# shenweichen/DeepCTR

Hardware: NVIDIA H100
Metric: samples/sec fwd+bwd DeepFM Criteo-synth (higher is better)
Workload: dtype f32

## Files before the change

### deepctr_b200/csrc/common.cuh

```cuda
#pragma once
#include <cuda_runtime.h>
#include <cuda_bf16.h>
#include <stdint.h>
#include <stdio.h>
#include <atomic>
#include "../../include/b2ctr.h"

namespace b2ctr {

void set_error(const char* fmt, ...);
extern std::atomic<long long> g_launches;
inline void count_launch(int n = 1) { g_launches.fetch_add(n, std::memory_order_relaxed); }

#define B2_REQUIRE(cond, ...)                         \
  do {                                                \
    if (!(cond)) {                                    \
      b2ctr::set_error(__VA_ARGS__);                  \
      return B2CTR_ERR_INVALID_ARG;                   \
    }                                                 \
  } while (0)

#define B2_CHECK_LAUNCH(name)                                                         \
  do {                                                                                \
    cudaError_t e__ = cudaGetLastError();                                             \
    if (e__ != cudaSuccess) {                                                         \
      b2ctr::set_error("%s: CUDA launch failed: %s", name, cudaGetErrorString(e__));  \
      return B2CTR_ERR_CUDA;                                                          \
    }                                                                                 \
    b2ctr::count_launch();                                                            \
  } while (0)

constexpr int kNumSMs = 132;

unsigned long long* oob_counter();

static inline int64_t ceil_div(int64_t a, int64_t b) { return (a + b - 1) / b; }

static inline int grid_for(int64_t work_items, int items_per_block, int blocks_per_sm) {
  int64_t need = ceil_div(work_items, items_per_block);
  int64_t cap = (int64_t)kNumSMs * blocks_per_sm;
  if (need < 1) need = 1;
  return (int)(need < cap ? need : cap);
}

static inline int64_t planes_rows_pad(int64_t rows) { return (rows + 255) / 256 * 256; }
static inline int64_t planes_cols_pad(int64_t cols) { return cols <= 64 ? 64 : (cols + 127) / 128 * 128; }

#ifdef __CUDACC__
__device__ __forceinline__ uint32_t pack_bf16(__nv_bfloat16 lo, __nv_bfloat16 hi) {
  return (uint32_t)__bfloat16_as_ushort(lo) | ((uint32_t)__bfloat16_as_ushort(hi) << 16);
}

__device__ __forceinline__ float4 ldg_stream_f4(const float* p) {
  float4 r;
  asm volatile("ld.global.nc.L1::no_allocate.v4.f32 {%0,%1,%2,%3}, [%4];"
               : "=f"(r.x), "=f"(r.y), "=f"(r.z), "=f"(r.w)
               : "l"(p));
  return r;
}
__device__ __forceinline__ float ldg_stream_f1(const float* p) {
  float r;
  asm volatile("ld.global.nc.L1::no_allocate.f32 %0, [%1];" : "=f"(r) : "l"(p));
  return r;
}
__device__ __forceinline__ void stg_stream_f4(float* p, float4 v) {
  asm volatile("st.global.L1::no_allocate.v4.f32 [%0], {%1,%2,%3,%4};" ::"l"(p), "f"(v.x),
               "f"(v.y), "f"(v.z), "f"(v.w)
               : "memory");
}
__device__ __forceinline__ void red_add_f4(float* p, float4 v) {
  asm volatile("red.relaxed.gpu.global.add.v4.f32 [%0], {%1,%2,%3,%4};" ::"l"(p), "f"(v.x),
               "f"(v.y), "f"(v.z), "f"(v.w)
               : "memory");
}
__device__ __forceinline__ void red_add_f1(float* p, float v) {
  asm volatile("red.relaxed.gpu.global.add.f32 [%0], %1;" ::"l"(p), "f"(v) : "memory");
}

__device__ __forceinline__ uint64_t l2_policy_evict_last() {
  uint64_t p;
  asm volatile("createpolicy.fractional.L2::evict_last.b64 %0, 1.0;" : "=l"(p));
  return p;
}
__device__ __forceinline__ uint64_t l2_policy_evict_first() {
  uint64_t p;
  asm volatile("createpolicy.fractional.L2::evict_first.b64 %0, 1.0;" : "=l"(p));
  return p;
}
__device__ __forceinline__ float4 ldg_stream_f4_pol(const float* p, uint64_t pol) {
  float4 r;
  asm volatile("ld.global.nc.L1::no_allocate.L2::cache_hint.v4.f32 {%0,%1,%2,%3}, [%4], %5;"
               : "=f"(r.x), "=f"(r.y), "=f"(r.z), "=f"(r.w)
               : "l"(p), "l"(pol));
  return r;
}
__device__ __forceinline__ float ldg_f1_pol(const float* p, uint64_t pol) {
  float r;
  asm volatile("ld.global.nc.L2::cache_hint.f32 %0, [%1], %2;" : "=f"(r) : "l"(p), "l"(pol));
  return r;
}
__device__ __forceinline__ void stg_stream_f4_pol(float* p, float4 v, uint64_t pol) {
  asm volatile("st.global.L1::no_allocate.L2::cache_hint.v4.f32 [%0], {%1,%2,%3,%4}, %5;" ::"l"(p),
               "f"(v.x), "f"(v.y), "f"(v.z), "f"(v.w), "l"(pol)
               : "memory");
}
__device__ __forceinline__ void red_add_f4_pol(float* p, float4 v, uint64_t pol) {
  asm volatile("red.relaxed.gpu.global.add.L2::cache_hint.v4.f32 [%0], {%1,%2,%3,%4}, %5;" ::"l"(p),
               "f"(v.x), "f"(v.y), "f"(v.z), "f"(v.w), "l"(pol)
               : "memory");
}
__device__ __forceinline__ void red_add_f1_pol(float* p, float v, uint64_t pol) {
  asm volatile("red.relaxed.gpu.global.add.L2::cache_hint.f32 [%0], %1, %2;" ::"l"(p), "f"(v), "l"(pol)
               : "memory");
}

__device__ __forceinline__ bool id_in_range(int64_t id, int64_t vocab) { return (uint64_t)id < (uint64_t)vocab; }
__device__ __forceinline__ void note_oob(unsigned long long* counter) {
  if (counter) atomicAdd(counter, 1ull);
}

__device__ __forceinline__ float warp_sum(float v) {
#pragma unroll
  for (int o = 16; o > 0; o >>= 1) v += __shfl_xor_sync(0xffffffffu, v, o);
  return v;
}

__device__ __forceinline__ uint32_t mix32(uint64_t z) {
  z = (z ^ (z >> 30)) * 0xbf58476d1ce4e5b9ULL;
  z = (z ^ (z >> 27)) * 0x94d049bb133111ebULL;
  return (uint32_t)((z ^ (z >> 31)) >> 32);
}

__device__ __forceinline__ int64_t load_idx(const void* p, int64_t off, int dtype) {
  return dtype == B2CTR_IDX_I64 ? reinterpret_cast<const int64_t*>(p)[off]
                                : (int64_t) reinterpret_cast<const int32_t*>(p)[off];
}

__device__ __forceinline__ float act_apply(float x, int act) {
  switch (act) {
    case B2CTR_ACT_RELU: return x > 0.f ? x : 0.f;
    case B2CTR_ACT_SIGMOID: return 1.f / (1.f + expf(-x));
    case B2CTR_ACT_TANH: return tanhf(x);
    default: return x;
  }
}
__device__ __forceinline__ float act_grad_from_out(float y, int act) {
  switch (act) {
    case B2CTR_ACT_RELU: return y > 0.f ? 1.f : 0.f;
    case B2CTR_ACT_SIGMOID: return y * (1.f - y);
    case B2CTR_ACT_TANH: return 1.f - y * y;
    default: return 1.f;
  }
}

#endif
}
```

### deepctr_b200/csrc/gemm_tc.cu

```cuda
#include <cuda.h>
#include <cuda_bf16.h>
#include "common.cuh"

namespace b2ctr {

constexpr int kTM = 128;
constexpr int kTK = 64;
constexpr int kTcThreads = 256;

struct PlaneArgs {
  const __nv_bfloat16* a_hi; const __nv_bfloat16* a_lo;
  const __nv_bfloat16* b_hi; const __nv_bfloat16* b_lo;
  int64_t a_pitch, b_pitch;
  int a_mn, b_mn;
  float* c; const float* bias; float* ws;
  int64_t m, n, k_pad;
  int64_t ldc;
  int64_t k_per_split;
  float alpha;
  int act, accumulate, splits;
  const float* cin_t0; const float* cin_xk;
  int64_t cin_ld0, cin_ldk, cin_rows;
  int cin_m, cin_h, cin_hp, cin_on;
  float* fold_dt0; float* fold_dxk; int64_t fold_ldx;
};

__device__ __forceinline__ uint32_t smem_u32(const void* p) {
  return (uint32_t)__cvta_generic_to_shared(p);
}
__device__ __forceinline__ void mbar_init(uint64_t* bar, uint32_t count) {
  asm volatile("mbarrier.init.shared::cta.b64 [%0], %1;" ::"r"(smem_u32(bar)), "r"(count));
}
__device__ __forceinline__ void mbar_arrive(uint64_t* bar) {
  asm volatile("mbarrier.arrive.shared::cta.b64 _, [%0];" ::"r"(smem_u32(bar)) : "memory");
}
__device__ __forceinline__ void mbar_wait(uint64_t* bar, uint32_t parity) {
  uint32_t done;
  do {
    asm volatile(
        "{\n\t"
        ".reg .pred p;\n\t"
        "mbarrier.try_wait.parity.shared::cta.b64 p, [%1], %2;\n\t"
        "selp.u32 %0, 1, 0, p;\n\t"
        "}\n"
        : "=r"(done)
        : "r"(smem_u32(bar)), "r"(parity)
        : "memory");
  } while (!done);
}
__device__ __forceinline__ uint64_t wgmma_desc(uint32_t saddr, int mn) {
  return (uint64_t)((saddr & 0x3FFFF) >> 4) | ((uint64_t)(mn ? 512 : 1) << 16) | (64ull << 32) | (1ull << 62);
}
__device__ __forceinline__ uint64_t wgmma_desc_k(uint32_t base, int ks, int mn) {
  return wgmma_desc(mn ? base + ks * 2048 : base + ks * 32, mn);
}
__device__ __forceinline__ void wgmma_fence() { asm volatile("wgmma.fence.sync.aligned;" ::: "memory"); }
__device__ __forceinline__ void wgmma_commit() { asm volatile("wgmma.commit_group.sync.aligned;" ::: "memory"); }
template <int N>
__device__ __forceinline__ void wgmma_wait() { asm volatile("wgmma.wait_group.sync.aligned %0;" ::"n"(N) : "memory"); }
template <int R>
__device__ __forceinline__ void fence_acc(float (&d)[R]) {
#pragma unroll
  for (int i = 0; i < R; ++i) asm volatile("" : "+f"(d[i])::"memory");
}

template <int N> struct Wgmma;
template <> struct Wgmma<32> {
  template <int TA, int TB>
  static __device__ __forceinline__ void mma(float (&d)[16], uint64_t da, uint64_t db) {
    asm volatile(
        "{\n\t.reg .pred p;\n\tsetp.ne.b32 p, %18, 0;\n\t"
        "wgmma.mma_async.sync.aligned.m64n32k16.f32.bf16.bf16 "
        "{%0,%1,%2,%3,%4,%5,%6,%7,%8,%9,%10,%11,%12,%13,%14,%15}, %16, %17, p, 1, 1, %19, %20;\n}\n"
        : "+f"(d[0]), "+f"(d[1]), "+f"(d[2]), "+f"(d[3]), "+f"(d[4]), "+f"(d[5]), "+f"(d[6]), "+f"(d[7]), "+f"(d[8]), "+f"(d[9]), "+f"(d[10]), "+f"(d[11]), "+f"(d[12]), "+f"(d[13]), "+f"(d[14]), "+f"(d[15])
        : "l"(da), "l"(db), "r"(1), "n"(TA), "n"(TB));
  }
};
template <> struct Wgmma<64> {
  template <int TA, int TB>
  static __device__ __forceinline__ void mma(float (&d)[32], uint64_t da, uint64_t db) {
    asm volatile(
        "{\n\t.reg .pred p;\n\tsetp.ne.b32 p, %34, 0;\n\t"
        "wgmma.mma_async.sync.aligned.m64n64k16.f32.bf16.bf16 "
        "{%0,%1,%2,%3,%4,%5,%6,%7,%8,%9,%10,%11,%12,%13,%14,%15,%16,%17,%18,%19,%20,%21,%22,%23,%24,%25,%26,%27,%28,%29,%30,%31}, %32, %33, p, 1, 1, %35, %36;\n}\n"
        : "+f"(d[0]), "+f"(d[1]), "+f"(d[2]), "+f"(d[3]), "+f"(d[4]), "+f"(d[5]), "+f"(d[6]), "+f"(d[7]), "+f"(d[8]), "+f"(d[9]), "+f"(d[10]), "+f"(d[11]), "+f"(d[12]), "+f"(d[13]), "+f"(d[14]), "+f"(d[15]), "+f"(d[16]), "+f"(d[17]), "+f"(d[18]), "+f"(d[19]), "+f"(d[20]), "+f"(d[21]), "+f"(d[22]), "+f"(d[23]), "+f"(d[24]), "+f"(d[25]), "+f"(d[26]), "+f"(d[27]), "+f"(d[28]), "+f"(d[29]), "+f"(d[30]), "+f"(d[31])
        : "l"(da), "l"(db), "r"(1), "n"(TA), "n"(TB));
  }
};
template <> struct Wgmma<128> {
  template <int TA, int TB>
  static __device__ __forceinline__ void mma(float (&d)[64], uint64_t da, uint64_t db) {
    asm volatile(
        "{\n\t.reg .pred p;\n\tsetp.ne.b32 p, %66, 0;\n\t"
        "wgmma.mma_async.sync.aligned.m64n128k16.f32.bf16.bf16 "
        "{%0,%1,%2,%3,%4,%5,%6,%7,%8,%9,%10,%11,%12,%13,%14,%15,%16,%17,%18,%19,%20,%21,%22,%23,%24,%25,%26,%27,%28,%29,%30,%31,%32,%33,%34,%35,%36,%37,%38,%39,%40,%41,%42,%43,%44,%45,%46,%47,%48,%49,%50,%51,%52,%53,%54,%55,%56,%57,%58,%59,%60,%61,%62,%63}, %64, %65, p, 1, 1, %67, %68;\n}\n"
        : "+f"(d[0]), "+f"(d[1]), "+f"(d[2]), "+f"(d[3]), "+f"(d[4]), "+f"(d[5]), "+f"(d[6]), "+f"(d[7]), "+f"(d[8]), "+f"(d[9]), "+f"(d[10]), "+f"(d[11]), "+f"(d[12]), "+f"(d[13]), "+f"(d[14]), "+f"(d[15]), "+f"(d[16]), "+f"(d[17]), "+f"(d[18]), "+f"(d[19]), "+f"(d[20]), "+f"(d[21]), "+f"(d[22]), "+f"(d[23]), "+f"(d[24]), "+f"(d[25]), "+f"(d[26]), "+f"(d[27]), "+f"(d[28]), "+f"(d[29]), "+f"(d[30]), "+f"(d[31]), "+f"(d[32]), "+f"(d[33]), "+f"(d[34]), "+f"(d[35]), "+f"(d[36]), "+f"(d[37]), "+f"(d[38]), "+f"(d[39]), "+f"(d[40]), "+f"(d[41]), "+f"(d[42]), "+f"(d[43]), "+f"(d[44]), "+f"(d[45]), "+f"(d[46]), "+f"(d[47]), "+f"(d[48]), "+f"(d[49]), "+f"(d[50]), "+f"(d[51]), "+f"(d[52]), "+f"(d[53]), "+f"(d[54]), "+f"(d[55]), "+f"(d[56]), "+f"(d[57]), "+f"(d[58]), "+f"(d[59]), "+f"(d[60]), "+f"(d[61]), "+f"(d[62]), "+f"(d[63])
        : "l"(da), "l"(db), "r"(1), "n"(TA), "n"(TB));
  }
};
template <> struct Wgmma<256> {
  template <int TA, int TB>
  static __device__ __forceinline__ void mma(float (&d)[128], uint64_t da, uint64_t db) {
    asm volatile(
        "{\n\t.reg .pred p;\n\tsetp.ne.b32 p, %130, 0;\n\t"
        "wgmma.mma_async.sync.aligned.m64n256k16.f32.bf16.bf16 "
        "{%0,%1,%2,%3,%4,%5,%6,%7,%8,%9,%10,%11,%12,%13,%14,%15,%16,%17,%18,%19,%20,%21,%22,%23,%24,%25,%26,%27,%28,%29,%30,%31,%32,%33,%34,%35,%36,%37,%38,%39,%40,%41,%42,%43,%44,%45,%46,%47,%48,%49,%50,%51,%52,%53,%54,%55,%56,%57,%58,%59,%60,%61,%62,%63,%64,%65,%66,%67,%68,%69,%70,%71,%72,%73,%74,%75,%76,%77,%78,%79,%80,%81,%82,%83,%84,%85,%86,%87,%88,%89,%90,%91,%92,%93,%94,%95,%96,%97,%98,%99,%100,%101,%102,%103,%104,%105,%106,%107,%108,%109,%110,%111,%112,%113,%114,%115,%116,%117,%118,%119,%120,%121,%122,%123,%124,%125,%126,%127}, %128, %129, p, 1, 1, %131, %132;\n}\n"
        : "+f"(d[0]), "+f"(d[1]), "+f"(d[2]), "+f"(d[3]), "+f"(d[4]), "+f"(d[5]), "+f"(d[6]), "+f"(d[7]), "+f"(d[8]), "+f"(d[9]), "+f"(d[10]), "+f"(d[11]), "+f"(d[12]), "+f"(d[13]), "+f"(d[14]), "+f"(d[15]), "+f"(d[16]), "+f"(d[17]), "+f"(d[18]), "+f"(d[19]), "+f"(d[20]), "+f"(d[21]), "+f"(d[22]), "+f"(d[23]), "+f"(d[24]), "+f"(d[25]), "+f"(d[26]), "+f"(d[27]), "+f"(d[28]), "+f"(d[29]), "+f"(d[30]), "+f"(d[31]), "+f"(d[32]), "+f"(d[33]), "+f"(d[34]), "+f"(d[35]), "+f"(d[36]), "+f"(d[37]), "+f"(d[38]), "+f"(d[39]), "+f"(d[40]), "+f"(d[41]), "+f"(d[42]), "+f"(d[43]), "+f"(d[44]), "+f"(d[45]), "+f"(d[46]), "+f"(d[47]), "+f"(d[48]), "+f"(d[49]), "+f"(d[50]), "+f"(d[51]), "+f"(d[52]), "+f"(d[53]), "+f"(d[54]), "+f"(d[55]), "+f"(d[56]), "+f"(d[57]), "+f"(d[58]), "+f"(d[59]), "+f"(d[60]), "+f"(d[61]), "+f"(d[62]), "+f"(d[63]), "+f"(d[64]), "+f"(d[65]), "+f"(d[66]), "+f"(d[67]), "+f"(d[68]), "+f"(d[69]), "+f"(d[70]), "+f"(d[71]), "+f"(d[72]), "+f"(d[73]), "+f"(d[74]), "+f"(d[75]), "+f"(d[76]), "+f"(d[77]), "+f"(d[78]), "+f"(d[79]), "+f"(d[80]), "+f"(d[81]), "+f"(d[82]), "+f"(d[83]), "+f"(d[84]), "+f"(d[85]), "+f"(d[86]), "+f"(d[87]), "+f"(d[88]), "+f"(d[89]), "+f"(d[90]), "+f"(d[91]), "+f"(d[92]), "+f"(d[93]), "+f"(d[94]), "+f"(d[95]), "+f"(d[96]), "+f"(d[97]), "+f"(d[98]), "+f"(d[99]), "+f"(d[100]), "+f"(d[101]), "+f"(d[102]), "+f"(d[103]), "+f"(d[104]), "+f"(d[105]), "+f"(d[106]), "+f"(d[107]), "+f"(d[108]), "+f"(d[109]), "+f"(d[110]), "+f"(d[111]), "+f"(d[112]), "+f"(d[113]), "+f"(d[114]), "+f"(d[115]), "+f"(d[116]), "+f"(d[117]), "+f"(d[118]), "+f"(d[119]), "+f"(d[120]), "+f"(d[121]), "+f"(d[122]), "+f"(d[123]), "+f"(d[124]), "+f"(d[125]), "+f"(d[126]), "+f"(d[127])
        : "l"(da), "l"(db), "r"(1), "n"(TA), "n"(TB));
  }
};
template <int BN, int TA, int TB>
__device__ __forceinline__ void wg_kblock(float (&d)[BN / 2], uint32_t st, int wg) {
  constexpr uint32_t A_PLANE = kTM * 128, B_PLANE = BN * 128;
  const uint32_t a_hi = st + wg * 8192, a_lo = a_hi + A_PLANE, b_hi = st + 2 * A_PLANE, b_lo = b_hi + B_PLANE;
  wgmma_fence();
#pragma unroll
  for (int ks = 0; ks < kTK / 16; ++ks) {
    const uint64_t dah = wgmma_desc_k(a_hi, ks, TA), dal = wgmma_desc_k(a_lo, ks, TA);
    const uint64_t dbh = wgmma_desc_k(b_hi, ks, TB), dbl = wgmma_desc_k(b_lo, ks, TB);
    Wgmma<BN>::template mma<TA, TB>(d, dah, dbh);
    Wgmma<BN>::template mma<TA, TB>(d, dah, dbl);
    Wgmma<BN>::template mma<TA, TB>(d, dal, dbh);
  }
  wgmma_commit();
}
template <int BN, int TA, int TB, int KS0>
__device__ __forceinline__ void tile_kblock_half(float (&d0)[BN / 2], float (&d1)[BN / 2], uint32_t st) {
  constexpr uint32_t A_PLANE = kTM * 128, B_PLANE = BN * 128;
  const uint32_t a_hi = st, a_lo = a_hi + A_PLANE, b_hi = st + 2 * A_PLANE, b_lo = b_hi + B_PLANE;
  wgmma_fence();
#pragma unroll
  for (int ks = KS0; ks < KS0 + 2; ++ks) {
    const uint64_t dah0 = wgmma_desc_k(a_hi, ks, TA), dal0 = wgmma_desc_k(a_lo, ks, TA);
    const uint64_t dah1 = wgmma_desc_k(a_hi + 8192, ks, TA), dal1 = wgmma_desc_k(a_lo + 8192, ks, TA);
    const uint64_t dbh = wgmma_desc_k(b_hi, ks, TB), dbl = wgmma_desc_k(b_lo, ks, TB);
    Wgmma<BN>::template mma<TA, TB>(d0, dah0, dbh);
    Wgmma<BN>::template mma<TA, TB>(d1, dah1, dbh);
    Wgmma<BN>::template mma<TA, TB>(d0, dah0, dbl);
    Wgmma<BN>::template mma<TA, TB>(d1, dah1, dbl);
    Wgmma<BN>::template mma<TA, TB>(d0, dal0, dbh);
    Wgmma<BN>::template mma<TA, TB>(d1, dal1, dbh);
  }
  wgmma_commit();
}
template <int V> struct Major { static constexpr int value = V; };
template <class F>
__device__ __forceinline__ void with_majorness(int a_mn, int b_mn, F&& f) {
  if (a_mn) {
    if (b_mn) f(Major<1>{}, Major<1>{});
    else f(Major<1>{}, Major<0>{});
  } else {
    if (b_mn) f(Major<0>{}, Major<1>{});
    else f(Major<0>{}, Major<0>{});
  }
}

template <int BN>
__device__ __forceinline__ void store_acc(const PlaneArgs& g, const float (&d)[BN / 2], int64_t row0, int64_t n0,
                                          int64_t z) {
  const int lane = threadIdx.x & 31, w = (threadIdx.x >> 5) & 3;
  const bool vec = (g.ldc % 2 == 0) && ((reinterpret_cast<uintptr_t>(g.c) & 7) == 0);
  const bool vec_ws = g.n % 2 == 0;
#pragma unroll
  for (int h = 0; h < 2; ++h) {
    const int64_t gm = row0 + w * 16 + (lane >> 2) + 8 * h;
    if (gm >= g.m) continue;
#pragma unroll
    for (int i = 0; i < BN / 8; ++i) {
      const int64_t gn = n0 + 8 * i + 2 * (lane & 3);
      if (gn >= g.n) continue;
      const bool two = gn + 1 < g.n;
      float v0 = g.alpha * d[4 * i + 2 * h], v1 = g.alpha * d[4 * i + 2 * h + 1];
      if (g.splits > 1) {
        float* wp = g.ws + (z * g.m + gm) * g.n + gn;
        if (two && vec_ws) *reinterpret_cast<float2*>(wp) = make_float2(v0, v1);
        else {
          wp[0] = v0;
          if (two) wp[1] = v1;
        }
        continue;
      }
      float* cp = g.c + gm * g.ldc + gn;
      if (two && vec) {
        if (g.accumulate) {
          const float2 o = *reinterpret_cast<const float2*>(cp);
          v0 += o.x; v1 += o.y;
        }
        if (g.bias) { v0 += __ldg(g.bias + gn); v1 += __ldg(g.bias + gn + 1); }
        *reinterpret_cast<float2*>(cp) = make_float2(act_apply(v0, g.act), act_apply(v1, g.act));
      } else {
        if (g.accumulate) v0 += cp[0];
        if (g.bias) v0 += g.bias[gn];
        cp[0] = act_apply(v0, g.act);
        if (two) {
          if (g.accumulate) v1 += cp[1];
          if (g.bias) v1 += g.bias[gn + 1];
          cp[1] = act_apply(v1, g.act);
        }
      }
    }
  }
}

__device__ __forceinline__ unsigned char* align1024(unsigned char* p) {
  return reinterpret_cast<unsigned char*>((reinterpret_cast<uintptr_t>(p) + 1023) & ~(uintptr_t)1023);
}

__global__ void tc_splitk_reduce_kernel(const PlaneArgs g) {
  const int64_t total = g.m * g.n;
  for (int64_t i = (int64_t)blockIdx.x * blockDim.x + threadIdx.x; i < total;
       i += (int64_t)gridDim.x * blockDim.x) {
    const int64_t gm = i / g.n, gn = i - gm * g.n;
    float v = 0.f;
    for (int z = 0; z < g.splits; ++z) v += g.ws[(int64_t)z * total + i];
    if (g.accumulate) v += g.c[gm * g.ldc + gn];
    if (g.bias) v += g.bias[gn];
    g.c[gm * g.ldc + gn] = act_apply(v, g.act);
  }
}
constexpr int kReduceBatch = 16;
__global__ void __launch_bounds__(128) tc_splitk_reduce4_kernel(const PlaneArgs g) {
  const int64_t total4 = g.m * g.n / 4;
  const float4* ws = reinterpret_cast<const float4*>(g.ws);
  const bool vec_c = g.ldc % 4 == 0 && ((reinterpret_cast<uintptr_t>(g.c) & 15) == 0);
  for (int64_t i = (int64_t)blockIdx.x * blockDim.x + threadIdx.x; i < total4;
       i += (int64_t)gridDim.x * blockDim.x) {
    float v[4] = {0.f, 0.f, 0.f, 0.f};
    for (int z0 = 0; z0 < g.splits; z0 += kReduceBatch) {
      float4 p[kReduceBatch];
#pragma unroll
      for (int j = 0; j < kReduceBatch; ++j)
        if (z0 + j < g.splits) p[j] = __ldcs(ws + (int64_t)(z0 + j) * total4 + i);
#pragma unroll
      for (int j = 0; j < kReduceBatch; ++j)
        if (z0 + j < g.splits) {
          v[0] += p[j].x; v[1] += p[j].y; v[2] += p[j].z; v[3] += p[j].w;
        }
    }
    const int64_t gm = (4 * i) / g.n, gn = 4 * i - gm * g.n;
    float* cp = g.c + gm * g.ldc + gn;
    if (g.accumulate) {
#pragma unroll
      for (int e = 0; e < 4; ++e) v[e] += cp[e];
    }
    if (g.bias) {
#pragma unroll
      for (int e = 0; e < 4; ++e) v[e] += __ldg(g.bias + gn + e);
    }
#pragma unroll
    for (int e = 0; e < 4; ++e) v[e] = act_apply(v[e], g.act);
    if (vec_c) *reinterpret_cast<float4*>(cp) = make_float4(v[0], v[1], v[2], v[3]);
    else {
#pragma unroll
      for (int e = 0; e < 4; ++e) cp[e] = v[e];
    }
  }
}
static void splitk_reduce(const PlaneArgs& pa, cudaStream_t st) {
  if (pa.n % 4 != 0 || ((uintptr_t)pa.ws & 15) != 0) {
    tc_splitk_reduce_kernel<<<grid_for(pa.m * pa.n, 256, 4), 256, 0, st>>>(pa);
    return;
  }
  const int64_t total4 = pa.m * pa.n / 4;
  int tpb = 128;
  while (tpb > 32 && ceil_div(total4, tpb) < kNumSMs) tpb /= 2;
  tc_splitk_reduce4_kernel<<<grid_for(total4, tpb, 2048 / tpb), tpb, 0, st>>>(pa);
}

__global__ void __launch_bounds__(256)
    split_planes_kernel(const float* __restrict__ p, int64_t sr, int64_t rows, int64_t k, int64_t rows_pad,
                        int64_t k_pad, __nv_bfloat16* hi, __nv_bfloat16* lo, int vec_ok) {
  const int64_t chunks = k_pad / 8;
  const int64_t total = rows_pad * chunks;
  for (int64_t t = (int64_t)blockIdx.x * blockDim.x + threadIdx.x; t < total;
       t += (int64_t)gridDim.x * blockDim.x) {
    const int64_t r = t / chunks;
    const int64_t k0 = (t - r * chunks) * 8;
    float v[8];
    if (r < rows && vec_ok && k0 + 8 <= k) {
      const float4 a = __ldg(reinterpret_cast<const float4*>(p + r * sr + k0));
      const float4 b = __ldg(reinterpret_cast<const float4*>(p + r * sr + k0) + 1);
      v[0] = a.x; v[1] = a.y; v[2] = a.z; v[3] = a.w; v[4] = b.x; v[5] = b.y; v[6] = b.z; v[7] = b.w;
    } else {
#pragma unroll
      for (int j = 0; j < 8; ++j) v[j] = (r < rows && k0 + j < k) ? __ldg(p + r * sr + k0 + j) : 0.f;
    }
    uint32_t h[4], l[4];
#pragma unroll
    for (int j = 0; j < 4; ++j) {
      const __nv_bfloat16 h0 = __float2bfloat16_rn(v[2 * j]), h1 = __float2bfloat16_rn(v[2 * j + 1]);
      h[j] = pack_bf16(h0, h1);
      l[j] = pack_bf16(__float2bfloat16_rn(v[2 * j] - __bfloat162float(h0)),
                       __float2bfloat16_rn(v[2 * j + 1] - __bfloat162float(h1)));
    }
    *reinterpret_cast<uint4*>(hi + r * k_pad + k0) = make_uint4(h[0], h[1], h[2], h[3]);
    *reinterpret_cast<uint4*>(lo + r * k_pad + k0) = make_uint4(l[0], l[1], l[2], l[3]);
  }
}
__global__ void __launch_bounds__(256)
    split_planes_t_kernel(const float* __restrict__ p, int64_t sk, int64_t rows, int64_t k, int64_t rows_pad,
                          int64_t k_pad, __nv_bfloat16* hi, __nv_bfloat16* lo) {
  __shared__ float tile[64][65];
  const int64_t r0 = (int64_t)blockIdx.x * 64, k0 = (int64_t)blockIdx.y * 64;
  const int tx = threadIdx.x & 63, ty = threadIdx.x >> 6;
#pragma unroll 4
  for (int kk = ty; kk < 64; kk += 4) {
    const int64_t gr = r0 + tx, gk = k0 + kk;
    tile[kk][tx] = (gr < rows && gk < k) ? __ldg(p + gk * sk + gr) : 0.f;
  }
  __syncthreads();
  for (int t = threadIdx.x; t < 64 * 8; t += 256) {
    const int r = t >> 3, c = t & 7;
    const int64_t gr = r0 + r;
    if (gr >= rows_pad) continue;
    uint32_t h[4], l[4];
#pragma unroll
    for (int j = 0; j < 4; ++j) {
      const float v0 = tile[c * 8 + 2 * j][r], v1 = tile[c * 8 + 2 * j + 1][r];
      const __nv_bfloat16 h0 = __float2bfloat16_rn(v0), h1 = __float2bfloat16_rn(v1);
      h[j] = pack_bf16(h0, h1);
      l[j] = pack_bf16(__float2bfloat16_rn(v0 - __bfloat162float(h0)), __float2bfloat16_rn(v1 - __bfloat162float(h1)));
    }
    *reinterpret_cast<uint4*>(hi + gr * k_pad + k0 + c * 8) = make_uint4(h[0], h[1], h[2], h[3]);
    *reinterpret_cast<uint4*>(lo + gr * k_pad + k0 + c * 8) = make_uint4(l[0], l[1], l[2], l[3]);
  }
}

__device__ __forceinline__ void cp_async16(uint32_t dst, const void* src) {
  asm volatile("cp.async.cg.shared.global [%0], [%1], 16;" ::"r"(dst), "l"(src) : "memory");
}

template <int BN, int STAGES>
__global__ void __launch_bounds__(kTcThreads, (STAGES * (2 * kTM * 128 + 2 * BN * 128) + 1024 <= 113 * 1024) ? 2 : 1)
    gemm_planes_kernel(const PlaneArgs g) {
  constexpr int A_PLANE = kTM * 128;
  constexpr int B_PLANE = BN * 128;
  constexpr int STAGE = 2 * A_PLANE + 2 * B_PLANE;
  extern __shared__ unsigned char smem_raw[];
  unsigned char* tiles = align1024(smem_raw);

  const int tid = threadIdx.x, wg = tid >> 7;
  const int64_t m0 = (int64_t)blockIdx.y * kTM, n0 = (int64_t)blockIdx.x * BN;
  const int64_t kbeg = (int64_t)blockIdx.z * g.k_per_split;
  const int64_t kend = kbeg + g.k_per_split < g.k_pad ? kbeg + g.k_per_split : g.k_pad;
  const int nkb = kend > kbeg ? (int)((kend - kbeg) / kTK) : 0;

  auto load = [&](int kb) {
    const uint32_t st = smem_u32(tiles + (size_t)(kb % STAGES) * STAGE);
    const int64_t k0 = kbeg + (int64_t)kb * kTK;
#pragma unroll
    for (int t = tid; t < kTM * 8; t += kTcThreads) {
      uint32_t off;
      int64_t src;
      if (g.a_mn) {
        const int kk = t / (kTM / 8), c = t % (kTM / 8);
        off = (c >> 3) * 8192 + kk * 128 + (((c & 7) ^ (kk & 7)) << 4);
        src = (k0 + kk) * g.a_pitch + m0 + c * 8;
      } else {
        const int r = t >> 3, c = t & 7;
        off = r * 128 + ((c ^ (r & 7)) << 4);
        src = (m0 + r) * g.a_pitch + k0 + c * 8;
      }
      cp_async16(st + off, g.a_hi + src);
      cp_async16(st + A_PLANE + off, g.a_lo + src);
    }
#pragma unroll
    for (int t = tid; t < BN * 8; t += kTcThreads) {
      uint32_t off;
      int64_t src;
      if (g.b_mn) {
        const int kk = t / (BN / 8), c = t % (BN / 8);
        off = (c >> 3) * 8192 + kk * 128 + (((c & 7) ^ (kk & 7)) << 4);
        src = (k0 + kk) * g.b_pitch + n0 + c * 8;
      } else {
        const int r = t >> 3, c = t & 7;
        off = r * 128 + ((c ^ (r & 7)) << 4);
        src = (n0 + r) * g.b_pitch + k0 + c * 8;
      }
      cp_async16(st + 2 * A_PLANE + off, g.b_hi + src);
      cp_async16(st + 2 * A_PLANE + B_PLANE + off, g.b_lo + src);
    }
  };

  float d[BN / 2];
#pragma unroll
  for (int j = 0; j < BN / 2; ++j) d[j] = 0.f;
#pragma unroll
  for (int s = 0; s < STAGES - 1; ++s) {
    if (s < nkb) load(s);
    asm volatile("cp.async.commit_group;" ::: "memory");
  }
  with_majorness(g.a_mn, g.b_mn, [&](auto ta, auto tb) {
    for (int kb = 0; kb < nkb; ++kb) {
      if (kb + STAGES - 1 < nkb) load(kb + STAGES - 1);
      asm volatile("cp.async.commit_group;" ::: "memory");
      asm volatile("cp.async.wait_group %0;" ::"n"(STAGES - 1) : "memory");
      asm volatile("fence.proxy.async.shared::cta;" ::: "memory");
      __syncthreads();
      wg_kblock<BN, decltype(ta)::value, decltype(tb)::value>(d, smem_u32(tiles + (size_t)(kb % STAGES) * STAGE), wg);
      wgmma_wait<0>();
      __syncthreads();
    }
  });
  asm volatile("cp.async.wait_all;" ::: "memory");
  fence_acc(d);
  store_acc<BN>(g, d, m0 + wg * 64, n0, blockIdx.z);
}

template <int BN, int STAGES>
static cudaError_t launch_planes(const PlaneArgs& pa, cudaStream_t st) {
  constexpr size_t smem = (size_t)STAGES * (2 * kTM * 128 + 2 * BN * 128) + 1024;
  dim3 grid((unsigned)ceil_div(pa.n, BN), (unsigned)ceil_div(pa.m, kTM), (unsigned)pa.splits);
  auto kern = gemm_planes_kernel<BN, STAGES>;
  cudaError_t e = cudaFuncSetAttribute(kern, cudaFuncAttributeMaxDynamicSharedMemorySize, (int)smem);
  if (e != cudaSuccess) return e;
  kern<<<grid, kTcThreads, smem, st>>>(pa);
  return cudaGetLastError();
}


constexpr int kWsConsumerWarps = 8;
constexpr int kWsProducers = 4;

struct WsArgs {
  PlaneArgs p;
  int tiles_m, tiles_n;
  int64_t ntiles;
  int c_tma;
  int coop;
};
template <int BN>
__host__ __device__ constexpr int ws_staging_bytes() { return 64 * (BN < 64 ? BN : 64) * 4; }
__device__ __forceinline__ void mbar_expect_tx(uint64_t* bar, uint32_t bytes) {
  asm volatile("mbarrier.arrive.expect_tx.shared::cta.b64 _, [%0], %1;" ::"r"(smem_u32(bar)), "r"(bytes) : "memory");
}
__device__ __forceinline__ void tma_load_2d(uint32_t dst, const CUtensorMap* map, int32_t c0, int32_t c1, uint64_t* bar) {
  asm volatile(
      "cp.async.bulk.tensor.2d.shared::cluster.global.mbarrier::complete_tx::bytes [%0], [%1, {%2, %3}], [%4];" ::"r"(dst),
      "l"(map), "r"(c0), "r"(c1), "r"(smem_u32(bar))
      : "memory");
}
__device__ __forceinline__ void tma_prefetch_desc(const CUtensorMap* map) {
  asm volatile("prefetch.tensormap [%0];" ::"l"(map) : "memory");
}
__device__ __forceinline__ void tma_store_2d(const CUtensorMap* map, uint32_t src, int32_t c0, int32_t c1) {
  asm volatile("cp.async.bulk.tensor.2d.global.shared::cta.bulk_group [%0, {%2, %3}], [%1];" ::"l"(map), "r"(src),
               "r"(c0), "r"(c1)
               : "memory");
}
__device__ __forceinline__ void tma_store_3d(const CUtensorMap* map, uint32_t src, int32_t c0, int32_t c1, int32_t c2) {
  asm volatile("cp.async.bulk.tensor.3d.global.shared::cta.bulk_group [%0, {%2, %3, %4}], [%1];" ::"l"(map), "r"(src),
               "r"(c0), "r"(c1), "r"(c2)
               : "memory");
}
__device__ __forceinline__ void bulk_commit() { asm volatile("cp.async.bulk.commit_group;" ::: "memory"); }
__device__ __forceinline__ void bulk_wait_read() { asm volatile("cp.async.bulk.wait_group.read 0;" ::: "memory"); }
__device__ __forceinline__ void bulk_wait_all() { asm volatile("cp.async.bulk.wait_group 0;" ::: "memory"); }
__device__ __forceinline__ void warpgroup_sync(int wg) {
  asm volatile("bar.sync %0, 128;" ::"r"(1 + wg) : "memory");
}
__device__ __forceinline__ void mma_order_wait(int wg) { asm volatile("bar.sync %0, 256;" ::"r"(3 + wg) : "memory"); }
__device__ __forceinline__ void mma_order_arrive(int wg) { asm volatile("bar.arrive %0, 256;" ::"r"(3 + wg) : "memory"); }
template <int R>
__device__ __forceinline__ void setmaxnreg_dec() { asm volatile("setmaxnreg.dec.sync.aligned.u32 %0;" ::"n"(R)); }
template <int R>
__device__ __forceinline__ void setmaxnreg_inc() { asm volatile("setmaxnreg.inc.sync.aligned.u32 %0;" ::"n"(R)); }

template <int BN, int ACT>
__device__ __forceinline__ void store_acc_tma_act(const PlaneArgs& g, const float (&d)[BN / 2], const CUtensorMap* map,
                                                  uint32_t stg, int wg, int64_t row0, int64_t n0, int32_t z) {
  constexpr int HALF = BN < 64 ? BN : 64;
  const int t = threadIdx.x & 127, lane = t & 31, w = t >> 5;
  const int64_t n4 = g.n & ~(int64_t)3;
  const bool tail = n0 + BN > n4;
  const float* bias = z < 0 ? g.bias : nullptr;
  const float alpha = g.alpha;
#pragma unroll
  for (int hf = 0; hf < BN / HALF; ++hf) {
    if (t == 0) bulk_wait_read();
    warpgroup_sync(wg);
#pragma unroll
    for (int i = hf * HALF / 8; i < (hf + 1) * HALF / 8; ++i) {
      const int col = 8 * i + 2 * (lane & 3) - hf * HALF;
      const int64_t gn = n0 + 8 * i + 2 * (lane & 3);
      const bool in0 = gn < g.n, in1 = gn + 1 < g.n;
      float b0 = 0.f, b1 = 0.f;
      if (bias) {
        if (in0) b0 = __ldg(bias + gn);
        if (in1) b1 = __ldg(bias + gn + 1);
      }
#pragma unroll
      for (int h = 0; h < 2; ++h) {
        const int r = w * 16 + (lane >> 2) + 8 * h;
        float v0 = __fmul_rn(alpha, d[4 * i + 2 * h]), v1 = __fmul_rn(alpha, d[4 * i + 2 * h + 1]);
        if (bias) {
          if (in0) v0 = __fadd_rn(v0, b0);
          if (in1) v1 = __fadd_rn(v1, b1);
        }
        v0 = act_apply(v0, ACT < 0 ? g.act : ACT);
        v1 = act_apply(v1, ACT < 0 ? g.act : ACT);
        const uint32_t off = (col >> 5) * 8192 + r * 128 + ((((col & 31) >> 2) ^ (r & 7)) << 4) + (col & 3) * 4;
        asm volatile("st.shared.v2.f32 [%0], {%1, %2};" ::"r"(stg + off), "f"(v0), "f"(v1) : "memory");
        if (tail && gn >= n4 && in0 && row0 + r < g.m) {
          float* cp = g.c + (row0 + r) * g.ldc + gn;
          cp[0] = v0;
          if (in1) cp[1] = v1;
        }
      }
    }
    asm volatile("fence.proxy.async.shared::cta;" ::: "memory");
    warpgroup_sync(wg);
    if (t == 0 && row0 < g.m) {
#pragma unroll
      for (int b = 0; b < HALF / 32; ++b) {
        const int64_t c0 = n0 + hf * HALF + 32 * b;
        if (c0 >= n4) continue;
        if (z < 0) tma_store_2d(map, stg + b * 8192, (int32_t)c0, (int32_t)row0);
        else tma_store_3d(map, stg + b * 8192, (int32_t)c0, (int32_t)row0, z);
      }
      bulk_commit();
    }
  }
}
template <int BN>
__device__ __forceinline__ void store_acc_tma(const PlaneArgs& g, const float (&d)[BN / 2], const CUtensorMap* map,
                                              uint32_t stg, int wg, int64_t row0, int64_t n0, int32_t z) {
  if (z >= 0 || g.act == B2CTR_ACT_NONE) store_acc_tma_act<BN, B2CTR_ACT_NONE>(g, d, map, stg, wg, row0, n0, z);
  else if (g.act == B2CTR_ACT_RELU) store_acc_tma_act<BN, B2CTR_ACT_RELU>(g, d, map, stg, wg, row0, n0, z);
  else store_acc_tma_act<BN, -1>(g, d, map, stg, wg, row0, n0, z);
}

__device__ __forceinline__ void split_pair(float v0, float v1, uint32_t& h, uint32_t& l) {
  const __nv_bfloat162 hh = __floats2bfloat162_rn(v0, v1);
  h = *reinterpret_cast<const uint32_t*>(&hh);
  const float h0 = __uint_as_float(h << 16), h1 = __uint_as_float(h & 0xffff0000u);
  const __nv_bfloat162 ll = __floats2bfloat162_rn(v0 - h0, v1 - h1);
  l = *reinterpret_cast<const uint32_t*>(&ll);
}
__device__ __forceinline__ void store_chunk(const float (&v)[8], unsigned char* hi_row, unsigned char* lo_row, int off) {
  uint32_t h[4], l[4];
#pragma unroll
  for (int e = 0; e < 4; ++e) split_pair(v[2 * e], v[2 * e + 1], h[e], l[e]);
  *reinterpret_cast<uint4*>(hi_row + off) = make_uint4(h[0], h[1], h[2], h[3]);
  *reinterpret_cast<uint4*>(lo_row + off) = make_uint4(l[0], l[1], l[2], l[3]);
}

struct GenRegs {
  float4 x[8];
  float a;
};
__device__ __forceinline__ void cin_load_half(const PlaneArgs& g, int64_t r, int q0, GenRegs& o) {
  const bool row_ok = r < g.cin_rows;
  const float* xk = g.cin_xk + r * g.cin_ldk;
  const int hp = g.cin_hp, h = g.cin_h;
  const int i = q0 / hp, j = q0 - i * hp;
  o.a = (row_ok && i < g.cin_m) ? __ldg(g.cin_t0 + r * g.cin_ld0 + i) : 0.f;
#pragma unroll
  for (int c = 0; c < 4; ++c) {
    const int jj = j + 8 * c;
    o.x[2 * c] = (row_ok && jj < h) ? __ldg(reinterpret_cast<const float4*>(xk + jj)) : make_float4(0.f, 0.f, 0.f, 0.f);
    o.x[2 * c + 1] = (row_ok && jj + 4 < h) ? __ldg(reinterpret_cast<const float4*>(xk + jj) + 1)
                                            : make_float4(0.f, 0.f, 0.f, 0.f);
  }
}
__device__ __forceinline__ void cin_emit_half(const PlaneArgs& g, GenRegs& io, int q0, unsigned char* hi_row,
                                              unsigned char* lo_row, int rr, int c0, bool has_next, int64_t r_next,
                                              int q0_next, bool reload_x) {
  const int hp = g.cin_hp, h = g.cin_h;
  const int j = q0 - (q0 / hp) * hp;
  const float a = io.a;
  const bool row_ok = has_next && r_next < g.cin_rows;
  const float* xk = g.cin_xk + r_next * g.cin_ldk;
  const int in_ = q0_next / hp, jn = q0_next - in_ * hp;
  if (has_next) io.a = (row_ok && in_ < g.cin_m) ? __ldg(g.cin_t0 + r_next * g.cin_ld0 + in_) : 0.f;
#pragma unroll
  for (int c = 0; c < 4; ++c) {
    float v[8] = {a * io.x[2 * c].x, a * io.x[2 * c].y, a * io.x[2 * c].z, a * io.x[2 * c].w,
                  a * io.x[2 * c + 1].x, a * io.x[2 * c + 1].y, a * io.x[2 * c + 1].z, a * io.x[2 * c + 1].w};
    if (reload_x) {
      const int jj = jn + 8 * c;
      io.x[2 * c] = (row_ok && jj < h) ? __ldg(reinterpret_cast<const float4*>(xk + jj)) : make_float4(0.f, 0.f, 0.f, 0.f);
      io.x[2 * c + 1] = (row_ok && jj + 4 < h) ? __ldg(reinterpret_cast<const float4*>(xk + jj) + 1)
                                               : make_float4(0.f, 0.f, 0.f, 0.f);
    }
    if (h & 7) {
#pragma unroll
      for (int e = 0; e < 8; ++e)
        if (j + 8 * c + e >= h) v[e] = 0.f;
    }
    store_chunk(v, hi_row, lo_row, ((c0 + c) ^ (rr & 7)) << 4);
  }
}

__device__ __noinline__ void att_generate_half(const PlaneArgs& g, int64_t r, int col0, unsigned char* hi_row,
                                                  unsigned char* lo_row, int rr, int c0) {
  const int T = g.cin_m, E = g.cin_h;
  const bool row_ok = r < g.cin_rows;
  const uint32_t bu = row_ok ? (uint32_t)r / (uint32_t)T : 0u;
  const int64_t b = bu;
  const int t = row_ok ? (int)((uint32_t)r - bu * (uint32_t)T) : 0;
  const float* q = g.cin_t0 + b * g.cin_ld0;
  const float* k = g.cin_xk + b * g.cin_ldk + (int64_t)t * E;
#pragma unroll
  for (int c = 0; c < 4; ++c) {
    const int col = col0 + 8 * c;
    const int seg = col / E, e = col - seg * E;
    float v[8];
    if (row_ok && seg < 4) {
      float4 a0 = make_float4(0.f, 0.f, 0.f, 0.f), a1 = a0, b0 = a0, b1 = a0;
      if (seg != 1) { a0 = __ldg(reinterpret_cast<const float4*>(q + e)); a1 = __ldg(reinterpret_cast<const float4*>(q + e) + 1); }
      if (seg != 0) { b0 = __ldg(reinterpret_cast<const float4*>(k + e)); b1 = __ldg(reinterpret_cast<const float4*>(k + e) + 1); }
      const float qa[8] = {a0.x, a0.y, a0.z, a0.w, a1.x, a1.y, a1.z, a1.w};
      const float ka[8] = {b0.x, b0.y, b0.z, b0.w, b1.x, b1.y, b1.z, b1.w};
#pragma unroll
      for (int jx = 0; jx < 8; ++jx)
        v[jx] = seg == 0 ? qa[jx] : seg == 1 ? ka[jx] : seg == 2 ? __fsub_rn(qa[jx], ka[jx]) : __fmul_rn(qa[jx], ka[jx]);
    } else {
#pragma unroll
      for (int jx = 0; jx < 8; ++jx) v[jx] = 0.f;
    }
    store_chunk(v, hi_row, lo_row, ((c0 + c) ^ (rr & 7)) << 4);
  }
}

template <bool GENERATED>
struct WsLayout {
  static constexpr int kProducers = GENERATED ? 8 : kWsProducers;
  static constexpr int kThreads = (kWsConsumerWarps + kProducers) * 32;
};

template <int BN, int STAGES, int GEN = 0, bool FOLD = false>
__global__ void __launch_bounds__(WsLayout<GEN != 0>::kThreads, 1)
    gemm_planes_ws_kernel(const __grid_constant__ WsArgs w, const __grid_constant__ CUtensorMap tm_ah,
                          const __grid_constant__ CUtensorMap tm_al, const __grid_constant__ CUtensorMap tm_bh,
                          const __grid_constant__ CUtensorMap tm_bl, const __grid_constant__ CUtensorMap tm_c) {
  static_assert(BN <= 128, "the consumer accumulator is BN / 2 registers per thread");
  constexpr bool PINGPONG = GEN == 0 && !FOLD;
  const PlaneArgs& g = w.p;
  constexpr int A_PLANE = kTM * 128;
  constexpr int B_PLANE = BN * 128;
  constexpr int STAGE = 2 * A_PLANE + 2 * B_PLANE;
  extern __shared__ unsigned char smem_raw[];
  unsigned char* tiles = align1024(smem_raw);
  __shared__ __align__(8) uint64_t full_bar[STAGES], empty_bar[STAGES];

  const int warp = threadIdx.x >> 5, lane = threadIdx.x & 31;
  const int64_t cta0 = blockIdx.x, nctas = gridDim.x;

  if (threadIdx.x == 0) {
    for (int s = 0; s < STAGES; ++s) {
      mbar_init(&full_bar[s], GEN == 1 ? 1 + 256 : GEN == 2 ? 1 + 128 : 1);
      mbar_init(&empty_bar[s], PINGPONG && !w.coop ? kWsConsumerWarps / 2 : kWsConsumerWarps);
    }
    asm volatile("fence.mbarrier_init.release.cluster;" ::: "memory");
  }
  __syncthreads();

  auto decode = [&](int64_t tile, int64_t& mt, int64_t& nt, int64_t& kbeg, int& nkb) {
    if constexpr (FOLD) {
      const int64_t j = tile / nctas;
      nt = j % w.tiles_n;
      mt = tile % nctas + (j / w.tiles_n) * nctas;
      kbeg = 0;
      nkb = mt < w.tiles_m ? (int)(g.k_pad / kTK) : 0;
      return;
    }
    nt = tile % w.tiles_n;
    const int64_t rest = tile / w.tiles_n;
    mt = rest % w.tiles_m;
    const int64_t z = rest / w.tiles_m;
    kbeg = z * g.k_per_split;
    const int64_t kend = kbeg + g.k_per_split < g.k_pad ? kbeg + g.k_per_split : g.k_pad;
    nkb = kend > kbeg ? (int)((kend - kbeg) / kTK) : 0;
  };

  if (GEN != 0 && warp >= kWsConsumerWarps) {
    const int tid = threadIdx.x - kWsConsumerWarps * 32;
    const int grp = tid >> 7, t128 = tid & 127;
    if (t128 == 0) { tma_prefetch_desc(&tm_bh); tma_prefetch_desc(&tm_bl); }
    uint32_t it = 0;
    if constexpr (GEN == 1) {
      const int half = tid & 1;
      const int atom = tid >> 7, rr = g.a_mn ? (tid & 127) >> 1 : tid >> 1;
      const int soff = (g.a_mn ? atom * 8192 : 0) + rr * 128;
      const int ntiles = (int)w.ntiles, stride = (int)nctas;
      auto dec = [&](int tile, int& m0, int& n0, int& kbeg, int& nkb) {
        int64_t mt, nt, kb64;
        decode(tile, mt, nt, kb64, nkb);
        m0 = (int)(mt * kTM);
        n0 = (int)(nt * BN);
        kbeg = (int)kb64;
      };
      int tile = (int)cta0, m0 = 0, n0 = 0, kbeg = 0, nkb = 0, kb = 0;
      for (; tile < ntiles; tile += stride) {
        dec(tile, m0, n0, kbeg, nkb);
        if (nkb > 0) break;
      }
      auto row_of = [&](int m0_, int k0_) { return g.a_mn ? k0_ + rr : m0_ + rr; };
      auto col_of = [&](int m0_, int k0_) { return g.a_mn ? m0_ + atom * 64 + half * 32 : k0_ + half * 32; };
      GenRegs gr;
      if (tile < ntiles) cin_load_half(g, row_of(m0, kbeg), col_of(m0, kbeg), gr);
      const int nj = (!g.a_mn && g.splits == 1 && g.cin_hp >= 128) ? g.cin_hp / kTK : 1;
      auto k_of = [&](int kbeg_, int kb_, int nkb_) {
        if (nj == 1) return kbeg_ + kb_ * kTK;
        const int ni = nkb_ / nj;
        const int jb = kb_ / ni, i = kb_ - jb * ni;
        return (i * nj + jb) * kTK;
      };
      while (tile < ntiles) {
        const int k0 = k_of(kbeg, kb, nkb);
        int tile_n = tile, m0_n = m0, n0_n = n0, kbeg_n = kbeg, nkb_n = nkb, kb_n = kb + 1;
        if (kb_n >= nkb) {
          kb_n = 0;
          for (tile_n = tile + stride; tile_n < ntiles; tile_n += stride) {
            dec(tile_n, m0_n, n0_n, kbeg_n, nkb_n);
            if (nkb_n > 0) break;
          }
        }
        const bool has_next = tile_n < ntiles;
        const int k0_n = k_of(kbeg_n, kb_n, nkb_n);
        const int s = it % STAGES;
        mbar_wait(&empty_bar[s], ((it / STAGES) & 1) ^ 1);
        unsigned char* stp = tiles + (size_t)s * STAGE;
        if (tid == 0) {
          uint64_t* bar = &full_bar[s];
          mbar_expect_tx(bar, (uint32_t)(2 * B_PLANE));
          const uint32_t st = smem_u32(stp);
          if (g.b_mn) {
#pragma unroll
            for (int j = 0; j < (BN >= 64 ? BN / 64 : 1); ++j) {
              tma_load_2d(st + 2 * A_PLANE + j * 8192, &tm_bh, n0 + 64 * j, k0, bar);
              tma_load_2d(st + 2 * A_PLANE + B_PLANE + j * 8192, &tm_bl, n0 + 64 * j, k0, bar);
            }
          } else {
            tma_load_2d(st + 2 * A_PLANE, &tm_bh, k0, n0, bar);
            tma_load_2d(st + 2 * A_PLANE + B_PLANE, &tm_bl, k0, n0, bar);
          }
        }
        const int r = row_of(m0, k0), r_n = row_of(m0_n, k0_n), q = col_of(m0, k0), q_n = col_of(m0_n, k0_n);
        cin_emit_half(g, gr, q, stp + soff, stp + A_PLANE + soff, rr, half * 4, has_next, r_n, q_n,
                      has_next && (r_n != r || q_n % g.cin_hp != q % g.cin_hp));
        asm volatile("fence.proxy.async.shared::cta;" ::: "memory");
        mbar_arrive(&full_bar[s]);
        ++it;
        tile = tile_n; m0 = m0_n; n0 = n0_n; kbeg = kbeg_n; nkb = nkb_n; kb = kb_n;
      }
    } else
    for (int64_t tile = cta0; tile < w.ntiles; tile += nctas) {
      int64_t mt, nt, kbeg;
      int nkb;
      decode(tile, mt, nt, kbeg, nkb);
      const int64_t m0 = mt * kTM;
      const int32_t n0 = (int32_t)(nt * BN);
      for (int kb = 0; kb < nkb; ++kb, ++it) {
        if ((int)(it & 1) != grp) continue;
        const int s = it % STAGES;
        mbar_wait(&empty_bar[s], ((it / STAGES) & 1) ^ 1);
        unsigned char* stp = tiles + (size_t)s * STAGE;
        const int64_t k0 = kbeg + (int64_t)kb * kTK;
        if (t128 == 0) {
          uint64_t* bar = &full_bar[s];
          mbar_expect_tx(bar, (uint32_t)(2 * B_PLANE));
          const uint32_t st = smem_u32(stp);
          if (g.b_mn) {
#pragma unroll
            for (int j = 0; j < (BN >= 64 ? BN / 64 : 1); ++j) {
              tma_load_2d(st + 2 * A_PLANE + j * 8192, &tm_bh, n0 + 64 * j, (int32_t)k0, bar);
              tma_load_2d(st + 2 * A_PLANE + B_PLANE + j * 8192, &tm_bl, n0 + 64 * j, (int32_t)k0, bar);
            }
          } else {
            tma_load_2d(st + 2 * A_PLANE, &tm_bh, (int32_t)k0, n0, bar);
            tma_load_2d(st + 2 * A_PLANE + B_PLANE, &tm_bl, (int32_t)k0, n0, bar);
          }
        }
        if (g.a_mn) {
          const int atom = t128 >> 6, rr = t128 & 63;
          unsigned char* row = stp + atom * 8192 + rr * 128;
          att_generate_half(g, k0 + rr, (int)(m0 + atom * 64), row, row + A_PLANE, rr, 0);
          att_generate_half(g, k0 + rr, (int)(m0 + atom * 64 + 32), row, row + A_PLANE, rr, 4);
        } else {
          unsigned char* row = stp + t128 * 128;
          att_generate_half(g, m0 + t128, (int)k0, row, row + A_PLANE, t128, 0);
          att_generate_half(g, m0 + t128, (int)(k0 + 32), row, row + A_PLANE, t128, 4);
        }
        asm volatile("fence.proxy.async.shared::cta;" ::: "memory");
        mbar_arrive(&full_bar[s]);
      }
    }
  } else if (warp >= kWsConsumerWarps) {
    if constexpr (PINGPONG) setmaxnreg_dec<56>();
    if (warp == kWsConsumerWarps && lane == 0) {
      tma_prefetch_desc(&tm_ah); tma_prefetch_desc(&tm_al); tma_prefetch_desc(&tm_bh); tma_prefetch_desc(&tm_bl);
      uint32_t it = 0;
      for (int64_t tile = cta0; tile < w.ntiles; tile += nctas) {
        int64_t mt, nt, kbeg;
        int nkb;
        decode(tile, mt, nt, kbeg, nkb);
        const int32_t m0 = (int32_t)(mt * kTM);
        const int32_t n0 = (int32_t)(nt * BN);
        for (int kb = 0; kb < nkb; ++kb, ++it) {
          const int s = it % STAGES;
          mbar_wait(&empty_bar[s], ((it / STAGES) & 1) ^ 1);
          uint64_t* bar = &full_bar[s];
          mbar_expect_tx(bar, (uint32_t)STAGE);
          const uint32_t st = smem_u32(tiles + (size_t)s * STAGE);
          const int32_t k0 = (int32_t)(kbeg + (int64_t)kb * kTK);
          if (g.a_mn) {
#pragma unroll
            for (int j = 0; j < kTM / 64; ++j) {
              tma_load_2d(st + j * 8192, &tm_ah, m0 + 64 * j, k0, bar);
              tma_load_2d(st + A_PLANE + j * 8192, &tm_al, m0 + 64 * j, k0, bar);
            }
          } else {
            tma_load_2d(st, &tm_ah, k0, m0, bar);
            tma_load_2d(st + A_PLANE, &tm_al, k0, m0, bar);
          }
          if (g.b_mn) {
#pragma unroll
            for (int j = 0; j < (BN >= 64 ? BN / 64 : 1); ++j) {
              tma_load_2d(st + 2 * A_PLANE + j * 8192, &tm_bh, n0 + 64 * j, k0, bar);
              tma_load_2d(st + 2 * A_PLANE + B_PLANE + j * 8192, &tm_bl, n0 + 64 * j, k0, bar);
            }
          } else {
            tma_load_2d(st + 2 * A_PLANE, &tm_bh, k0, n0, bar);
            tma_load_2d(st + 2 * A_PLANE + B_PLANE, &tm_bl, k0, n0, bar);
          }
        }
      }
    }
  } else {
    const int wg = warp >> 2;
    auto pingpong = [&](auto ta, auto tb) {
      constexpr int TA = decltype(ta)::value, TB = decltype(tb)::value;
      const uint32_t stg = smem_u32(tiles + STAGES * STAGE + wg * ws_staging_bytes<BN>());
      uint32_t it = 0;
      float d0[BN / 2], d1[BN / 2];
      int64_t j = 0;
      for (int64_t tile = cta0; tile < w.ntiles; tile += nctas, ++j) {
        int64_t mt, nt, kbeg;
        int nkb;
        decode(tile, mt, nt, kbeg, nkb);
        if ((j & 1) != wg) {
          it += nkb;
          continue;
        }
        if (j > 0) mma_order_wait(wg);
#pragma unroll
        for (int i = 0; i < BN / 2; ++i) d0[i] = d1[i] = 0.f;
        int prev = -1;
        for (int kb = 0; kb < nkb; ++kb, ++it) {
          const int s = it % STAGES;
          mbar_wait(&full_bar[s], (it / STAGES) & 1);
          const uint32_t st = smem_u32(tiles + (size_t)s * STAGE);
          tile_kblock_half<BN, TA, TB, 0>(d0, d1, st);
          wgmma_wait<1>();
          if (prev >= 0) {
            __syncwarp();
            if (lane == 0) mbar_arrive(&empty_bar[prev]);
          }
          tile_kblock_half<BN, TA, TB, 2>(d0, d1, st);
          wgmma_wait<1>();
          prev = s;
        }
        if (tile + nctas < w.ntiles) mma_order_arrive(wg ^ 1);
        wgmma_wait<0>();
        fence_acc(d0);
        fence_acc(d1);
        if (prev >= 0) {
          __syncwarp();
          if (lane == 0) mbar_arrive(&empty_bar[prev]);
        }
        const int64_t row0 = mt * kTM;
        if (w.c_tma == 2) {
          const int32_t z = (int32_t)(tile / ((int64_t)w.tiles_n * w.tiles_m));
          store_acc_tma<BN>(g, d0, &tm_c, stg, wg, row0, nt * BN, z);
          store_acc_tma<BN>(g, d1, &tm_c, stg, wg, row0 + 64, nt * BN, z);
        } else if (w.c_tma) {
          store_acc_tma<BN>(g, d0, &tm_c, stg, wg, row0, nt * BN, -1);
          store_acc_tma<BN>(g, d1, &tm_c, stg, wg, row0 + 64, nt * BN, -1);
        } else {
          const int64_t z = tile / ((int64_t)w.tiles_n * w.tiles_m);
          store_acc<BN>(g, d0, row0, nt * BN, z);
          store_acc<BN>(g, d1, row0 + 64, nt * BN, z);
        }
      }
      if (w.c_tma && (threadIdx.x & 127) == 0) bulk_wait_all();
    };
    auto consume = [&](auto ta, auto tb) {
      uint32_t it = 0;
      float d[BN / 2];
      [[maybe_unused]] float dxk[FOLD ? BN / 2 : 1];
      for (int64_t tile = cta0; tile < w.ntiles; tile += nctas) {
        int64_t mt, nt, kbeg;
        int nkb;
        decode(tile, mt, nt, kbeg, nkb);
        if (FOLD && nkb == 0) continue;
#pragma unroll
        for (int j = 0; j < BN / 2; ++j) d[j] = 0.f;
        int prev = -1;
        for (int kb = 0; kb < nkb; ++kb, ++it) {
          const int s = it % STAGES;
          mbar_wait(&full_bar[s], (it / STAGES) & 1);
          wg_kblock<BN, decltype(ta)::value, decltype(tb)::value>(d, smem_u32(tiles + (size_t)s * STAGE), wg);
          wgmma_wait<1>();
          if (prev >= 0) {
            __syncwarp();
            if (lane == 0) mbar_arrive(&empty_bar[prev]);
          }
          prev = s;
        }
        wgmma_wait<0>();
        fence_acc(d);
        if (prev >= 0) {
          __syncwarp();
          if (lane == 0) mbar_arrive(&empty_bar[prev]);
        }
        const int64_t row0 = mt * kTM + wg * 64;
        if constexpr (FOLD) {
          if (nt == 0) {
#pragma unroll
            for (int j = 0; j < BN / 2; ++j) dxk[j] = 0.f;
          }
#pragma unroll
          for (int h = 0; h < 2; ++h) {
            const int64_t gm = row0 + (warp & 3) * 16 + (lane >> 2) + 8 * h;
            const bool row_ok = gm < g.m;
            const float* t0 = g.cin_t0 + (row_ok ? gm : 0) * g.cin_ld0;
            const float* xk = g.cin_xk + (row_ok ? gm : 0) * g.cin_ldk;
            float p = 0.f;
#pragma unroll
            for (int i = 0; i < BN / 8; ++i) {
              const int c = 8 * i + 2 * (lane & 3);
              const int64_t q = nt * BN + c;
              const int ic = (int)(q / g.cin_hp), j = (int)(q - (int64_t)ic * g.cin_hp);
              const bool ok = row_ok && ic < g.cin_m;
              const float a = ok ? __ldg(t0 + ic) : 0.f;
              const float x0 = ok && j < g.cin_h ? __ldg(xk + j) : 0.f;
              const float x1 = ok && j + 1 < g.cin_h ? __ldg(xk + j + 1) : 0.f;
              const float d0 = d[4 * i + 2 * h], d1 = d[4 * i + 2 * h + 1];
              p += d0 * x0 + d1 * x1;
              dxk[4 * i + 2 * h] += d0 * a;
              dxk[4 * i + 2 * h + 1] += d1 * a;
              if ((8 * (i + 1)) % g.cin_hp == 0) {
                p += __shfl_xor_sync(0xffffffffu, p, 1);
                p += __shfl_xor_sync(0xffffffffu, p, 2);
                if ((lane & 3) == 0 && ok) red_add_f1(g.fold_dt0 + gm * g.cin_ld0 + ic, p);
                p = 0.f;
              }
            }
            if (nt == w.tiles_n - 1 && row_ok) {
              float* dst = g.fold_dxk + gm * g.fold_ldx;
#pragma unroll
              for (int i = 0; i < BN / 8; ++i) {
                const int j = (8 * i + 2 * (lane & 3)) % g.cin_hp;
                if (j < g.cin_h) red_add_f1(dst + j, dxk[4 * i + 2 * h]);
                if (j + 1 < g.cin_h) red_add_f1(dst + j + 1, dxk[4 * i + 2 * h + 1]);
              }
            }
          }
        } else if (w.c_tma) {
          const uint32_t stg = smem_u32(tiles + STAGES * STAGE + wg * ws_staging_bytes<BN>());
          if (w.c_tma == 2)
            store_acc_tma<BN>(g, d, &tm_c, stg, wg, row0, nt * BN, (int32_t)(tile / ((int64_t)w.tiles_n * w.tiles_m)));
          else
            store_acc_tma<BN>(g, d, &tm_c, stg, wg, row0, nt * BN, -1);
        } else {
          const int64_t z = tile / ((int64_t)w.tiles_n * w.tiles_m);
          store_acc<BN>(g, d, row0, nt * BN, z);
        }
      }
      if (!FOLD && w.c_tma && (threadIdx.x & 127) == 0) bulk_wait_all();
    };
    if constexpr (FOLD) consume(Major<0>{}, Major<0>{});
    else if constexpr (GEN != 0) {
      if (g.a_mn) consume(Major<1>{}, Major<1>{});
      else consume(Major<0>{}, Major<1>{});
    } else {
      setmaxnreg_inc<224>();
      auto run = [&](auto ta, auto tb) {
        if (w.coop) consume(ta, tb);
        else pingpong(ta, tb);
      };
      if constexpr (BN < 64) {
        if (g.a_mn) run(Major<1>{}, Major<0>{});
        else run(Major<0>{}, Major<0>{});
      } else {
        with_majorness(g.a_mn, g.b_mn, run);
      }
    }
  }
}

struct TmaMaps {
  CUtensorMap ah, al, bh, bl, c;
};

template <int BN, int STAGES, int GEN = 0, bool FOLD = false>
static cudaError_t launch_ws_impl(const WsArgs& wa, const TmaMaps& tm, cudaStream_t st) {
  constexpr size_t smem = (size_t)STAGES * (2 * kTM * 128 + 2 * BN * 128) + 2 * ws_staging_bytes<BN>() + 1024;
  static_assert(smem + 256 <= 227 * 1024, "stage ring + epilogue staging exceed shared memory");
  auto kern = gemm_planes_ws_kernel<BN, STAGES, GEN, FOLD>;
  cudaError_t e = cudaFuncSetAttribute(kern, cudaFuncAttributeMaxDynamicSharedMemorySize, (int)smem);
  if (e != cudaSuccess) return e;
  int64_t nctas = wa.ntiles < kNumSMs ? wa.ntiles : kNumSMs;
  WsArgs wcopy = wa;
  if (FOLD) {
    nctas = wa.tiles_m < kNumSMs ? wa.tiles_m : kNumSMs;
    wcopy.ntiles = ceil_div(wa.tiles_m, nctas) * wa.tiles_n * nctas;
  }
  kern<<<(unsigned)nctas, WsLayout<GEN != 0>::kThreads, smem, st>>>(wcopy, tm.ah, tm.al, tm.bh, tm.bl, tm.c);
  return cudaGetLastError();
}

typedef CUresult (*EncodeTiledFn)(CUtensorMap*, CUtensorMapDataType, cuuint32_t, void*, const cuuint64_t*,
                                  const cuuint64_t*, const cuuint32_t*, const cuuint32_t*, CUtensorMapInterleave,
                                  CUtensorMapSwizzle, CUtensorMapL2promotion, CUtensorMapFloatOOBfill);
static EncodeTiledFn tma_encoder() {
  static EncodeTiledFn fn = nullptr;
  static bool tried = false;
  if (!tried) {
    tried = true;
    void* p = nullptr;
    cudaDriverEntryPointQueryResult q;
    if (cudaGetDriverEntryPoint("cuTensorMapEncodeTiled", &p, cudaEnableDefault, &q) == cudaSuccess &&
        q == cudaDriverEntryPointSuccess)
      fn = (EncodeTiledFn)p;
    else
      cudaGetLastError();
  }
  return fn;
}
static bool tma_map_2d(CUtensorMap* m, const void* base, int64_t inner, int64_t outer, int64_t pitch,
                       int box_inner, int box_outer) {
  EncodeTiledFn enc = tma_encoder();
  if (!enc || ((uintptr_t)base & 15) || (pitch * 2) % 16 || box_inner * 2 > 128 || box_outer > 256) return false;
  cuuint64_t dims[2] = {(cuuint64_t)inner, (cuuint64_t)outer};
  cuuint64_t strides[1] = {(cuuint64_t)pitch * 2};
  cuuint32_t box[2] = {(cuuint32_t)box_inner, (cuuint32_t)box_outer};
  cuuint32_t estr[2] = {1, 1};
  return enc(m, CU_TENSOR_MAP_DATA_TYPE_BFLOAT16, 2, const_cast<void*>(base), dims, strides, box, estr,
             CU_TENSOR_MAP_INTERLEAVE_NONE, CU_TENSOR_MAP_SWIZZLE_128B, CU_TENSOR_MAP_L2_PROMOTION_L2_256B,
             CU_TENSOR_MAP_FLOAT_OOB_FILL_NONE) == CUDA_SUCCESS;
}

static bool tma_map_c(CUtensorMap* m, const PlaneArgs& p) {
  EncodeTiledFn enc = tma_encoder();
  if (!enc || p.splits > 1 || p.accumulate || !p.c || ((uintptr_t)p.c & 15) || p.ldc % 4 || p.ldc < p.n ||
      p.n < 4 || p.m >= (1ll << 31) || p.n >= (1ll << 31))
    return false;
  cuuint64_t dims[2] = {(cuuint64_t)(p.n & ~(int64_t)3), (cuuint64_t)p.m};
  cuuint64_t strides[1] = {(cuuint64_t)p.ldc * 4};
  cuuint32_t box[2] = {32, 64};
  cuuint32_t estr[2] = {1, 1};
  return enc(m, CU_TENSOR_MAP_DATA_TYPE_FLOAT32, 2, p.c, dims, strides, box, estr, CU_TENSOR_MAP_INTERLEAVE_NONE,
             CU_TENSOR_MAP_SWIZZLE_128B, CU_TENSOR_MAP_L2_PROMOTION_NONE, CU_TENSOR_MAP_FLOAT_OOB_FILL_NONE) ==
         CUDA_SUCCESS;
}
static bool tma_map_ws(CUtensorMap* m, const PlaneArgs& p) {
  EncodeTiledFn enc = tma_encoder();
  if (!enc || p.splits < 2 || !p.ws || ((uintptr_t)p.ws & 15) || p.n % 4 || p.m >= (1ll << 31) ||
      p.n >= (1ll << 31))
    return false;
  cuuint64_t dims[3] = {(cuuint64_t)p.n, (cuuint64_t)p.m, (cuuint64_t)p.splits};
  cuuint64_t strides[2] = {(cuuint64_t)p.n * 4, (cuuint64_t)(p.m * p.n) * 4};
  cuuint32_t box[3] = {32, 64, 1};
  cuuint32_t estr[3] = {1, 1, 1};
  return enc(m, CU_TENSOR_MAP_DATA_TYPE_FLOAT32, 3, p.ws, dims, strides, box, estr, CU_TENSOR_MAP_INTERLEAVE_NONE,
             CU_TENSOR_MAP_SWIZZLE_128B, CU_TENSOR_MAP_L2_PROMOTION_NONE, CU_TENSOR_MAP_FLOAT_OOB_FILL_NONE) ==
         CUDA_SUCCESS;
}

static inline int64_t round_up(int64_t v, int64_t q) { return (v + q - 1) / q * q; }
static inline int planes_bn(int64_t n, int64_t k) {
  if (n <= 32) return 32;
  if (n <= 64) return 64;
  if (n <= 128 || k <= 4 * kTK) return 128;
  return 256;
}

size_t gemm_bf16x3_workspace_bytes(const b2ctr_gemm_t* g) {
  size_t splitk = g->split_k > 1 ? (size_t)g->split_k * g->m * g->n * sizeof(float) : 0;
  const int64_t kp = round_up(g->k > 0 ? g->k : 1, kTK), mp = round_up(g->m, 2 * kTM), np = round_up(g->n, 256);
  return splitk + (size_t)(mp + np) * kp * 2 * sizeof(__nv_bfloat16) + 512;
}

b2ctr_status_t gemm_bf16x3(const b2ctr_gemm_t* g, void* workspace, size_t workspace_bytes, cudaStream_t st) {
  B2_REQUIRE(g->variant == 0 || g->variant == 3 || g->variant == 4, "gemm: variant must be 0, 3 or 4, got %d",
             g->variant);
  B2_REQUIRE(((uintptr_t)g->a_planes & 15) == 0 && ((uintptr_t)g->b_planes & 15) == 0,
             "gemm: a_planes / b_planes must be 16-byte aligned");
  const size_t need = gemm_bf16x3_workspace_bytes(g);
  if (!workspace || workspace_bytes < need) {
    set_error("gemm(bf16x3): needs %zu workspace bytes, got %zu", need, workspace_bytes);
    return B2CTR_ERR_WORKSPACE;
  }
  const int splits = g->split_k > 1 ? g->split_k : 1;
  const bool ws_kernel = g->variant != 3;
  int bn = ws_kernel ? (g->n <= 32 ? 32 : g->n <= 64 ? 64 : 128)
                     : planes_bn(g->n, g->k / (g->split_k > 1 ? g->split_k : 1));
  const int64_t kp = round_up(g->k > 0 ? g->k : 1, kTK), mp = round_up(g->m, 2 * kTM);
  unsigned char* w = (unsigned char*)workspace;
  float* ws = (float*)w;
  w += splits > 1 ? (size_t)splits * g->m * g->n * sizeof(float) : 0;
  w = (unsigned char*)(((uintptr_t)w + 255) & ~(uintptr_t)255);
  const bool a_kc = !g->trans_a, b_kc = g->trans_b != 0;
  const int64_t a_sr = g->trans_a ? g->k : g->m, a_sc = g->trans_a ? g->m : g->k;
  const int64_t b_sr = g->trans_b ? g->n : g->k, b_sc = g->trans_b ? g->k : g->n;
  const bool a_given = g->a_planes != nullptr;
  const bool b_given = g->b_planes && (b_kc || bn >= 64);
  B2_REQUIRE(a_given || g->a, "gemm: NULL A without its planes");
  B2_REQUIRE(b_given || g->b, "gemm: NULL B, and its planes are missing or unusable at N = %lld", (long long)g->n);
  if (b_given && !b_kc && planes_cols_pad(b_sc) % bn != 0) bn = planes_cols_pad(b_sc) == 64 ? 64 : 128;
  const int64_t np = round_up(g->n, bn);
  const int a_mn = !a_kc;
  const int b_mn = !b_kc && bn >= 64;
  __nv_bfloat16 *a_hi, *a_lo, *b_hi, *b_lo;
  int64_t a_pitch, b_pitch;
  int64_t a_prows, b_prows;
  auto split_k = [&](const float* p, int64_t ld, int64_t rows, int64_t cols, int64_t rows_pad, int64_t cols_pad,
                     __nv_bfloat16* hi, __nv_bfloat16* lo) {
    const int vec = (ld % 4 == 0) && (((uintptr_t)p & 15) == 0);
    split_planes_kernel<<<grid_for(rows_pad * (cols_pad / 8), 256, 8), 256, 0, st>>>(p, ld, rows, cols, rows_pad,
                                                                                   cols_pad, hi, lo, vec);
  };
  auto split_t = [&](const float* p, int64_t ld, int64_t rows, int64_t rows_pad, __nv_bfloat16* hi,
                     __nv_bfloat16* lo) {
    dim3 grid((unsigned)ceil_div(rows_pad, 64), (unsigned)(kp / 64));
    split_planes_t_kernel<<<grid, 256, 0, st>>>(p, ld, rows, g->k, rows_pad, kp, hi, lo);
  };
  if (a_given) {
    const int64_t rp = round_up(a_sr, 256), cp = planes_cols_pad(a_sc);
    a_hi = (__nv_bfloat16*)g->a_planes; a_lo = a_hi + rp * cp; a_pitch = cp; a_prows = rp;
  } else {
    a_hi = (__nv_bfloat16*)w; a_lo = a_hi + mp * kp; w = (unsigned char*)(a_lo + mp * kp);
    a_pitch = a_mn ? mp : kp; a_prows = a_mn ? kp : mp;
    if (a_kc) split_k(g->a, g->lda, g->m, g->k, mp, kp, a_hi, a_lo);
    else split_k(g->a, g->lda, g->k, g->m, kp, mp, a_hi, a_lo);
    B2_CHECK_LAUNCH("b2ctr_gemm(bf16x3 split A)");
  }
  if (b_given) {
    const int64_t rp = round_up(b_sr, 256), cp = planes_cols_pad(b_sc);
    b_hi = (__nv_bfloat16*)g->b_planes; b_lo = b_hi + rp * cp; b_pitch = cp; b_prows = rp;
  } else {
    b_hi = (__nv_bfloat16*)w; b_lo = b_hi + np * kp;
    b_pitch = b_mn ? np : kp; b_prows = b_mn ? kp : np;
    if (b_kc) split_k(g->b, g->ldb, g->n, g->k, np, kp, b_hi, b_lo);
    else if (b_mn) split_k(g->b, g->ldb, g->k, g->n, kp, np, b_hi, b_lo);
    else split_t(g->b, g->ldb, g->n, np, b_hi, b_lo);
    B2_CHECK_LAUNCH("b2ctr_gemm(bf16x3 split B)");
  }
  PlaneArgs pa;
  pa.a_hi = a_hi; pa.a_lo = a_lo; pa.b_hi = b_hi; pa.b_lo = b_lo;
  pa.a_mn = a_mn; pa.b_mn = b_mn;
  pa.a_pitch = a_pitch; pa.b_pitch = b_pitch;
  pa.c = g->c; pa.bias = g->bias; pa.ws = ws;
  pa.m = g->m; pa.n = g->n; pa.k_pad = kp; pa.ldc = g->ldc;
  pa.k_per_split = ceil_div(ceil_div(kp, splits), kTK) * kTK;
  pa.alpha = g->alpha; pa.act = g->act; pa.accumulate = g->accumulate; pa.splits = splits;
  pa.cin_on = 0; pa.cin_t0 = pa.cin_xk = nullptr; pa.cin_ld0 = pa.cin_ldk = pa.cin_rows = 0; pa.cin_m = pa.cin_h = pa.cin_hp = 0;
  pa.fold_dt0 = pa.fold_dxk = nullptr; pa.fold_ldx = 0;
  cudaError_t e;
  const bool short_k = pa.k_per_split <= 4 * kTK;
  if (ws_kernel) {
    WsArgs wa;
    wa.p = pa;
    wa.tiles_m = (int)ceil_div(g->m, (int64_t)kTM);
    wa.tiles_n = (int)ceil_div(g->n, bn);
    wa.ntiles = (int64_t)wa.tiles_m * wa.tiles_n * splits;
    TmaMaps tm{};
    if (!(tma_map_2d(&tm.ah, a_hi, a_pitch, a_prows, a_pitch, 64, a_mn ? 64 : kTM) &&
          tma_map_2d(&tm.al, a_lo, a_pitch, a_prows, a_pitch, 64, a_mn ? 64 : kTM) &&
          tma_map_2d(&tm.bh, b_hi, b_pitch, b_prows, b_pitch, 64, b_mn ? 64 : bn) &&
          tma_map_2d(&tm.bl, b_lo, b_pitch, b_prows, b_pitch, 64, b_mn ? 64 : bn))) {
      set_error("b2ctr_gemm(bf16x3): cuTensorMapEncodeTiled unavailable (the kernel loads its operands by TMA)");
      return B2CTR_ERR_UNSUPPORTED;
    }
    wa.c_tma = tma_map_c(&tm.c, pa) ? 1 : tma_map_ws(&tm.c, pa) ? 2 : 0;
    wa.coop = splits > 1 && wa.ntiles <= kNumSMs;
    if (bn == 32) e = launch_ws_impl<32, 5>(wa, tm, st);
    else if (bn == 64) e = launch_ws_impl<64, 4>(wa, tm, st);
    else e = launch_ws_impl<128, 3>(wa, tm, st);
  } else if (bn == 32) e = short_k ? launch_planes<32, 1>(pa, st) : launch_planes<32, 4>(pa, st);
  else if (bn == 64) e = short_k ? launch_planes<64, 1>(pa, st) : launch_planes<64, 4>(pa, st);
  else if (bn == 128) e = short_k ? launch_planes<128, 1>(pa, st) : launch_planes<128, 3>(pa, st);
  else e = launch_planes<256, 2>(pa, st);
  if (e != cudaSuccess) {
    set_error("b2ctr_gemm(bf16x3 planes): CUDA launch failed: %s", cudaGetErrorString(e));
    return B2CTR_ERR_CUDA;
  }
  count_launch();
  if (splits > 1) {
    if (ws_kernel) splitk_reduce(pa, st);
    else tc_splitk_reduce_kernel<<<grid_for(g->m * g->n, 256, 4), 256, 0, st>>>(pa);
    B2_CHECK_LAUNCH("b2ctr_gemm(bf16x3 splitk_reduce)");
  }
  return B2CTR_OK;
}

__global__ void __launch_bounds__(256)
    cin_filter_planes_kernel(const float* __restrict__ w, int m, int h, int hp, int64_t n, int64_t rows_pad,
                             int64_t cols_pad, __nv_bfloat16* hi, __nv_bfloat16* lo) {
  const int64_t chunks = cols_pad / 8;
  const int64_t total = rows_pad * chunks;
  for (int64_t t = (int64_t)blockIdx.x * blockDim.x + threadIdx.x; t < total; t += (int64_t)gridDim.x * blockDim.x) {
    const int64_t r = t / chunks;
    const int64_t c0 = (t - r * chunks) * 8;
    const int i = (int)(r / hp), j = (int)(r - (int64_t)i * hp);
    const bool ok = i < m && j < h;
    uint32_t hh[4], ll[4];
#pragma unroll
    for (int e = 0; e < 4; ++e) {
      const float v0 = (ok && c0 + 2 * e < n) ? __ldg(w + ((int64_t)i * h + j) * n + c0 + 2 * e) : 0.f;
      const float v1 = (ok && c0 + 2 * e + 1 < n) ? __ldg(w + ((int64_t)i * h + j) * n + c0 + 2 * e + 1) : 0.f;
      const __nv_bfloat16 h0 = __float2bfloat16_rn(v0), h1 = __float2bfloat16_rn(v1);
      hh[e] = pack_bf16(h0, h1);
      ll[e] = pack_bf16(__float2bfloat16_rn(v0 - __bfloat162float(h0)), __float2bfloat16_rn(v1 - __bfloat162float(h1)));
    }
    *reinterpret_cast<uint4*>(hi + r * cols_pad + c0) = make_uint4(hh[0], hh[1], hh[2], hh[3]);
    *reinterpret_cast<uint4*>(lo + r * cols_pad + c0) = make_uint4(ll[0], ll[1], ll[2], ll[3]);
  }
}

b2ctr_status_t cin_filter_planes(const float* w, int m, int h, int hp, int64_t n, void* planes, cudaStream_t st) {
  const int64_t rp = round_up((int64_t)m * hp, 256), cp = planes_cols_pad(n);
  __nv_bfloat16* hi = (__nv_bfloat16*)planes;
  cin_filter_planes_kernel<<<grid_for(rp * (cp / 8), 256, 8), 256, 0, st>>>(w, m, h, hp, n, rp, cp, hi, hi + rp * cp);
  B2_CHECK_LAUNCH("b2ctr_cin_filter_planes");
  return B2CTR_OK;
}

struct GenSpec {
  int kind;
  const float* p0; int64_t ld0;
  const float* p1; int64_t ld1;
  int64_t rows;
  int m, h, hp;
  int64_t kq;
};

static size_t gen_gemm_workspace_bytes(const GenSpec& sp, int mode, int64_t n, int split_k) {
  const int64_t M = mode == 0 ? sp.rows : sp.kq;
  return split_k > 1 ? (size_t)split_k * M * n * sizeof(float) + 256 : 0;
}

template <int GEN>
static cudaError_t launch_gen(const WsArgs& wa, const TmaMaps& tm, int bn, cudaStream_t st) {
  if (bn == 64) return launch_ws_impl<64, 4, GEN>(wa, tm, st);
  return launch_ws_impl<128, 3, GEN>(wa, tm, st);
}

static b2ctr_status_t gen_gemm(const GenSpec& sp, int mode, int64_t n, const void* planes, float* c, int64_t ldc,
                               const float* bias, int act, int split_k, void* workspace, size_t workspace_bytes,
                               cudaStream_t st, const char* what) {
  B2_REQUIRE(sp.rows < (1ll << 31) && sp.kq < (1ll << 31), "%s: rows and generated width must fit 31 bits", what);
  const size_t need = gen_gemm_workspace_bytes(sp, mode, n, split_k);
  if (need && (!workspace || workspace_bytes < need)) {
    set_error("%s: needs %zu workspace bytes, got %zu", what, need, workspace_bytes);
    return B2CTR_ERR_WORKSPACE;
  }
  const int splits = split_k > 1 ? split_k : 1;
  PlaneArgs pa;
  pa.a_hi = pa.a_lo = nullptr; pa.a_pitch = 0;
  pa.cin_on = sp.kind; pa.cin_t0 = sp.p0; pa.cin_xk = sp.p1; pa.cin_ld0 = sp.ld0; pa.cin_ldk = sp.ld1;
  pa.cin_rows = sp.rows; pa.cin_m = sp.m; pa.cin_h = sp.h; pa.cin_hp = sp.hp;
  pa.fold_dt0 = pa.fold_dxk = nullptr; pa.fold_ldx = 0;
  pa.b_mn = 1;
  pa.c = c; pa.bias = bias; pa.ws = (float*)workspace; pa.ldc = ldc;
  pa.alpha = 1.f; pa.act = act; pa.accumulate = 0; pa.splits = splits;
  pa.n = n;
  const int64_t cp = planes_cols_pad(n);
  int64_t b_prows;
  if (mode == 0) {
    pa.a_mn = 0; pa.m = sp.rows; pa.k_pad = round_up(sp.kq, kTK);
    b_prows = round_up(sp.kq, 256);
  } else {
    pa.a_mn = 1; pa.m = sp.kq; pa.k_pad = round_up(sp.rows, kTK);
    b_prows = round_up(sp.rows, 256);
  }
  const __nv_bfloat16* bp = (const __nv_bfloat16*)planes;
  pa.b_hi = bp; pa.b_lo = bp + b_prows * cp; pa.b_pitch = cp;
  pa.k_per_split = ceil_div(ceil_div(pa.k_pad, splits), kTK) * kTK;
  const int bn = n <= 64 ? 64 : 128;
  WsArgs wa;
  wa.p = pa;
  wa.tiles_m = (int)ceil_div(pa.m, (int64_t)kTM);
  wa.tiles_n = (int)ceil_div(n, bn);
  wa.ntiles = (int64_t)wa.tiles_m * wa.tiles_n * splits;
  TmaMaps tm{};
  if (!tma_map_2d(&tm.bh, pa.b_hi, cp, b_prows, cp, 64, 64) || !tma_map_2d(&tm.bl, pa.b_lo, cp, b_prows, cp, 64, 64)) {
    set_error("%s: cuTensorMapEncodeTiled unavailable (the kernel loads its B operand by TMA)", what);
    return B2CTR_ERR_UNSUPPORTED;
  }
  tm.ah = tm.bh; tm.al = tm.bl;
  wa.c_tma = tma_map_c(&tm.c, pa);
  wa.coop = 0;
  const cudaError_t e = sp.kind == 1 ? launch_gen<1>(wa, tm, bn, st) : launch_gen<2>(wa, tm, bn, st);
  if (e != cudaSuccess) {
    set_error("%s: CUDA launch failed: %s", what, cudaGetErrorString(e));
    return B2CTR_ERR_CUDA;
  }
  count_launch();
  if (splits > 1) {
    tc_splitk_reduce_kernel<<<grid_for(pa.m * n, 256, 4), 256, 0, st>>>(pa);
    B2_CHECK_LAUNCH("generated-operand gemm (splitk_reduce)");
  }
  return B2CTR_OK;
}

static GenSpec cin_spec(const b2ctr_cin_gemm_t* g) {
  GenSpec sp;
  sp.kind = 1; sp.p0 = g->t0; sp.ld0 = g->ld0; sp.p1 = g->xk; sp.ld1 = g->ldk; sp.rows = g->rows;
  sp.m = g->m; sp.h = g->h; sp.hp = g->hp; sp.kq = (int64_t)g->m * g->hp;
  return sp;
}
size_t cin_gemm_workspace_bytes(const b2ctr_cin_gemm_t* g) {
  return gen_gemm_workspace_bytes(cin_spec(g), g->mode, g->n, g->split_k);
}
b2ctr_status_t cin_gemm(const b2ctr_cin_gemm_t* g, void* workspace, size_t workspace_bytes, cudaStream_t st) {
  B2_REQUIRE(g && g->t0 && g->xk && g->c && g->rows > 0 && g->m > 0 && g->h > 0 && g->n > 0, "cin_gemm: bad arguments");
  B2_REQUIRE(g->hp >= g->h && (g->hp == 32 || g->hp % 64 == 0), "cin_gemm: hp must be 32 or a multiple of 64 and >= h");
// ... 106 lines not shown
```

### deepctr_b200/csrc/tower.cu

```cuda
#include <cuda_bf16.h>
#include "common.cuh"

namespace b2ctr {
namespace {

typedef __nv_bfloat16 bf16;
constexpr int kTowerWarps = 8;
constexpr int kTowerThreads = kTowerWarps * 32;

__host__ __device__ constexpr int cols_pad(int w) { return w <= 64 ? 64 : (w + 127) / 128 * 128; }

struct TowerFwd {
  const float* y0;
  const float* w1; const float* b1;
  const float* w2; const float* b2;
  bf16* p0; bf16* p1;
  float* ylast;
  int64_t batch, rows_pad;
};
struct TowerBwd {
  const float* dy;
  const float* ylast;
  const float* y0;
  const bf16* p1;
  const float* w1; const float* w2;
  bf16* dz0; bf16* dz1; bf16* dz2;
  float* partial;
  int64_t batch, rows_pad;
};

__device__ __forceinline__ void mma_bf16(float (&c)[4], const uint32_t (&a)[4], uint32_t b0, uint32_t b1) {
  asm("mma.sync.aligned.m16n8k16.row.col.f32.bf16.bf16.f32 {%0,%1,%2,%3}, {%4,%5,%6,%7}, {%8,%9}, {%0,%1,%2,%3};"
      : "+f"(c[0]), "+f"(c[1]), "+f"(c[2]), "+f"(c[3])
      : "r"(a[0]), "r"(a[1]), "r"(a[2]), "r"(a[3]), "r"(b0), "r"(b1));
}

struct Split2 { uint32_t hi, lo; };
__device__ __forceinline__ Split2 split2(float x, float y) {
  const bf16 hx = __float2bfloat16_rn(x), hy = __float2bfloat16_rn(y);
  return {pack_bf16(hx, hy), pack_bf16(__float2bfloat16_rn(x - __bfloat162float(hx)),
                                       __float2bfloat16_rn(y - __bfloat162float(hy)))};
}

__device__ __forceinline__ float relu_bias(float acc, float b) {
  float v;
  asm("add.ftz.f32 %0, %1, %2;" : "=f"(v) : "f"(acc), "f"(b));
  return v > 0.f ? v : 0.f;
}

__device__ __forceinline__ float2 ld2(const float* p, bool ok) {
  return ok ? __ldg(reinterpret_cast<const float2*>(p)) : make_float2(0.f, 0.f);
}

__device__ __forceinline__ void st_chunk(bf16* plane, int64_t cp, int64_t ra, int c0, uint32_t a, uint32_t b,
                                         uint32_t c, uint32_t d, int t) {
  const int quad = threadIdx.x & 28;
  uint32_t o0 = 0, o1 = 0, o2 = 0, o3 = 0;
#pragma unroll
  for (int r = 0; r < 4; ++r) {
    const int i = (t - r) & 3, src = (t + r) & 3;
    const uint32_t send = i == 0 ? a : i == 1 ? c : i == 2 ? b : d;
    const uint32_t v = __shfl_sync(0xffffffffu, send, quad | src);
    o0 = src == 0 ? v : o0;
    o1 = src == 1 ? v : o1;
    o2 = src == 2 ? v : o2;
    o3 = src == 3 ? v : o3;
  }
  *reinterpret_cast<uint4*>(plane + (ra + (t >> 1) * 8) * cp + c0 + (t & 1) * 8) = make_uint4(o0, o1, o2, o3);
}

template <int NT, int P>
__device__ __forceinline__ void mma_k16(float (&acc)[NT][4], const uint32_t (&ah)[4], const uint32_t (&al)[4],
                                        const bf16* sh, const bf16* sl, int k0, int g, int t) {
#pragma unroll
  for (int j = 0; j < NT; ++j) {
    const int o = (j * 8 + g) * P + k0 + 2 * t;
    const uint32_t bh0 = *reinterpret_cast<const uint32_t*>(sh + o), bh1 = *reinterpret_cast<const uint32_t*>(sh + o + 8);
    const uint32_t bl0 = *reinterpret_cast<const uint32_t*>(sl + o), bl1 = *reinterpret_cast<const uint32_t*>(sl + o + 8);
    mma_bf16(acc[j], ah, bh0, bh1);
    mma_bf16(acc[j], ah, bl0, bl1);
    mma_bf16(acc[j], al, bh0, bh1);
  }
}

template <int K, int N, bool kTrans>
__device__ __forceinline__ void stage_weight(const float* __restrict__ w, bf16* sh, bf16* sl) {
  for (int i = threadIdx.x; i < K * N; i += kTowerThreads) {
    const int k = i / N, n = i - k * N;
    const float v = __ldg(w + i);
    const bf16 h = __float2bfloat16_rn(v);
    const int o = kTrans ? n * (K + 8) + k : k * (N + 8) + n;
    sh[o] = h;
    sl[o] = __float2bfloat16_rn(v - __bfloat162float(h));
  }
}

template <int W>
__device__ __forceinline__ void zero_pad_cols(bf16* hi, bf16* lo, int64_t r0, int lane) {
  constexpr int CP = cols_pad(W), V = (CP - W) / 8;
  if constexpr (V > 0) {
    for (int i = lane; i < 16 * V; i += 32) {
      const int64_t o = (r0 + i / V) * CP + W + (i % V) * 8;
      *reinterpret_cast<uint4*>(hi + o) = make_uint4(0, 0, 0, 0);
      *reinterpret_cast<uint4*>(lo + o) = make_uint4(0, 0, 0, 0);
    }
  }
}

__device__ __forceinline__ void colsum_add(float* red, int c, float v0, float v1, int g) {
#pragma unroll
  for (int o = 4; o < 32; o <<= 1) {
    v0 += __shfl_xor_sync(0xffffffffu, v0, o);
    v1 += __shfl_xor_sync(0xffffffffu, v1, o);
  }
  if (g == 0) {
    red[c] += v0;
    red[c + 1] += v1;
  }
}

template <int N0, int N1, int N2>
constexpr size_t tower_smem_bytes(bool bwd) {
  return bwd ? ((size_t)N0 * (N1 + 8) + (size_t)N1 * (N2 + 8)) * 2 * sizeof(bf16) +
                   (size_t)kTowerWarps * (N0 + N1 + N2) * sizeof(float)
             : ((size_t)N1 * (N0 + 8) + (size_t)N2 * (N1 + 8)) * 2 * sizeof(bf16);
}

template <int N0, int N1, int N2>
__global__ void __launch_bounds__(kTowerThreads, 1) mlp_relu_fwd_kernel(const TowerFwd p) {
  extern __shared__ __align__(16) unsigned char smem[];
  constexpr int P1 = N0 + 8, P2 = N1 + 8, CP0 = cols_pad(N0), CP1 = cols_pad(N1);
  bf16* w1h = reinterpret_cast<bf16*>(smem);
  bf16* w1l = w1h + N1 * P1;
  bf16* w2h = w1l + N1 * P1;
  bf16* w2l = w2h + N2 * P2;
  stage_weight<N0, N1, true>(p.w1, w1h, w1l);
  if constexpr (N2 > 0) stage_weight<N1, N2, true>(p.w2, w2h, w2l);
  __syncthreads();

  const int lane = threadIdx.x & 31, g = lane >> 2, t = lane & 3;
  bf16* p0l = p.p0 + p.rows_pad * CP0;
  const int64_t tiles = p.rows_pad / 16;
  for (int64_t tile = (int64_t)blockIdx.x * kTowerWarps + (threadIdx.x >> 5); tile < tiles;
       tile += (int64_t)gridDim.x * kTowerWarps) {
    const int64_t r0 = tile * 16, ra = r0 + g, rb = ra + 8;
    const bool va = ra < p.batch, vb = rb < p.batch;
    float acc1[N1 / 8][4];
#pragma unroll
    for (int j = 0; j < N1 / 8; ++j) acc1[j][0] = acc1[j][1] = acc1[j][2] = acc1[j][3] = 0.f;
#pragma unroll 4
    for (int kc = 0; kc < N0 / 16; ++kc) {
      const int c = kc * 16 + 2 * t;
      const float2 x0 = ld2(p.y0 + ra * N0 + c, va), x1 = ld2(p.y0 + rb * N0 + c, vb);
      const float2 x2 = ld2(p.y0 + ra * N0 + c + 8, va), x3 = ld2(p.y0 + rb * N0 + c + 8, vb);
      const Split2 s0 = split2(x0.x, x0.y), s1 = split2(x1.x, x1.y), s2 = split2(x2.x, x2.y), s3 = split2(x3.x, x3.y);
      const uint32_t ah[4] = {s0.hi, s1.hi, s2.hi, s3.hi}, al[4] = {s0.lo, s1.lo, s2.lo, s3.lo};
      st_chunk(p.p0, CP0, ra, kc * 16, s0.hi, s1.hi, s2.hi, s3.hi, t);
      st_chunk(p0l, CP0, ra, kc * 16, s0.lo, s1.lo, s2.lo, s3.lo, t);
      mma_k16<N1 / 8, P1>(acc1, ah, al, w1h, w1l, kc * 16, g, t);
    }
    zero_pad_cols<N0>(p.p0, p0l, r0, lane);

    if constexpr (N2 == 0) {
#pragma unroll
      for (int j = 0; j < N1 / 8; ++j) {
        const int c = j * 8 + 2 * t;
        const float2 b = __ldg(reinterpret_cast<const float2*>(p.b1 + c));
        if (va) *reinterpret_cast<float2*>(p.ylast + ra * N1 + c) =
                    make_float2(relu_bias(acc1[j][0], b.x), relu_bias(acc1[j][1], b.y));
        if (vb) *reinterpret_cast<float2*>(p.ylast + rb * N1 + c) =
                    make_float2(relu_bias(acc1[j][2], b.x), relu_bias(acc1[j][3], b.y));
      }
    } else {
      bf16* p1l = p.p1 + p.rows_pad * CP1;
      uint32_t a2h[N1 / 16][4], a2l[N1 / 16][4];
      Split2 pa, pb;
#pragma unroll
      for (int j = 0; j < N1 / 8; ++j) {
        const int c = j * 8 + 2 * t;
        const float2 b = __ldg(reinterpret_cast<const float2*>(p.b1 + c));
        const Split2 sa = va ? split2(relu_bias(acc1[j][0], b.x), relu_bias(acc1[j][1], b.y)) : Split2{0u, 0u};
        const Split2 sb = vb ? split2(relu_bias(acc1[j][2], b.x), relu_bias(acc1[j][3], b.y)) : Split2{0u, 0u};
        a2h[j / 2][(j & 1) * 2] = sa.hi; a2h[j / 2][(j & 1) * 2 + 1] = sb.hi;
        a2l[j / 2][(j & 1) * 2] = sa.lo; a2l[j / 2][(j & 1) * 2 + 1] = sb.lo;
        if (j & 1) {
          st_chunk(p.p1, CP1, ra, (j / 2) * 16, pa.hi, pb.hi, sa.hi, sb.hi, t);
          st_chunk(p1l, CP1, ra, (j / 2) * 16, pa.lo, pb.lo, sa.lo, sb.lo, t);
        } else {
          pa = sa, pb = sb;
        }
      }
      zero_pad_cols<N1>(p.p1, p1l, r0, lane);
      float acc2[N2 / 8][4];
#pragma unroll
      for (int j = 0; j < N2 / 8; ++j) acc2[j][0] = acc2[j][1] = acc2[j][2] = acc2[j][3] = 0.f;
#pragma unroll
      for (int kc = 0; kc < N1 / 16; ++kc) mma_k16<N2 / 8, P2>(acc2, a2h[kc], a2l[kc], w2h, w2l, kc * 16, g, t);
#pragma unroll
      for (int j = 0; j < N2 / 8; ++j) {
        const int c = j * 8 + 2 * t;
        const float2 b = __ldg(reinterpret_cast<const float2*>(p.b2 + c));
        if (va) *reinterpret_cast<float2*>(p.ylast + ra * N2 + c) =
                    make_float2(relu_bias(acc2[j][0], b.x), relu_bias(acc2[j][1], b.y));
        if (vb) *reinterpret_cast<float2*>(p.ylast + rb * N2 + c) =
                    make_float2(relu_bias(acc2[j][2], b.x), relu_bias(acc2[j][3], b.y));
      }
    }
  }
}

template <int N0, int N1, int N2>
__global__ void __launch_bounds__(kTowerThreads, 1) mlp_relu_bwd_kernel(const TowerBwd p) {
  extern __shared__ __align__(16) unsigned char smem[];
  constexpr int NL = N2 ? N2 : N1, NT = N0 + N1 + N2;
  constexpr int P1 = N1 + 8, P2 = N2 + 8, CP0 = cols_pad(N0), CP1 = cols_pad(N1), CPL = cols_pad(NL);
  constexpr int NC = 32;
  bf16* w1h = reinterpret_cast<bf16*>(smem);
  bf16* w1l = w1h + N0 * P1;
  bf16* w2h = w1l + N0 * P1;
  bf16* w2l = w2h + N1 * P2;
  float* red_all = reinterpret_cast<float*>(w2l + N1 * P2);
  stage_weight<N0, N1, false>(p.w1, w1h, w1l);
  if constexpr (N2 > 0) stage_weight<N1, N2, false>(p.w2, w2h, w2l);
  for (int i = threadIdx.x; i < kTowerWarps * NT; i += kTowerThreads) red_all[i] = 0.f;
  __syncthreads();

  const int lane = threadIdx.x & 31, warp = threadIdx.x >> 5, g = lane >> 2, t = lane & 3;
  float* red = red_all + warp * NT;
  bf16* dzl = N2 ? p.dz2 : p.dz1;
  bf16* dzl_lo = dzl + p.rows_pad * CPL;
  bf16* dz0l = p.dz0 + p.rows_pad * CP0;
  const int64_t tiles = p.rows_pad / 16;
  for (int64_t tile = (int64_t)blockIdx.x * kTowerWarps + warp; tile < tiles; tile += (int64_t)gridDim.x * kTowerWarps) {
    const int64_t r0 = tile * 16, ra = r0 + g, rb = ra + 8;
    const bool va = ra < p.batch, vb = rb < p.batch;

    uint32_t alh[NL / 16][4], all[NL / 16][4];
    Split2 pa, pb;
#pragma unroll
    for (int j = 0; j < NL / 8; ++j) {
      const int c = j * 8 + 2 * t;
      const float2 da = ld2(p.dy + ra * NL + c, va), db = ld2(p.dy + rb * NL + c, vb);
      const float2 ya = ld2(p.ylast + ra * NL + c, va), yb = ld2(p.ylast + rb * NL + c, vb);
      const float z0 = da.x * (ya.x > 0.f ? 1.f : 0.f), z1 = da.y * (ya.y > 0.f ? 1.f : 0.f);
      const float z2 = db.x * (yb.x > 0.f ? 1.f : 0.f), z3 = db.y * (yb.y > 0.f ? 1.f : 0.f);
      const Split2 sa = split2(z0, z1), sb = split2(z2, z3);
      alh[j / 2][(j & 1) * 2] = sa.hi; alh[j / 2][(j & 1) * 2 + 1] = sb.hi;
      all[j / 2][(j & 1) * 2] = sa.lo; all[j / 2][(j & 1) * 2 + 1] = sb.lo;
      if (j & 1) {
        st_chunk(dzl, CPL, ra, (j / 2) * 16, pa.hi, pb.hi, sa.hi, sb.hi, t);
        st_chunk(dzl_lo, CPL, ra, (j / 2) * 16, pa.lo, pb.lo, sa.lo, sb.lo, t);
      } else {
        pa = sa, pb = sb;
      }
      colsum_add(red, N0 + (N2 ? N1 : 0) + c, z0 + z2, z1 + z3, g);
    }
    zero_pad_cols<NL>(dzl, dzl_lo, r0, lane);

    uint32_t a1h[N1 / 16][4], a1l[N1 / 16][4];
    if constexpr (N2 == 0) {
#pragma unroll
      for (int kc = 0; kc < N1 / 16; ++kc)
#pragma unroll
        for (int q = 0; q < 4; ++q) a1h[kc][q] = alh[kc][q], a1l[kc][q] = all[kc][q];
    } else {
      float acc[N1 / 8][4];
#pragma unroll
      for (int j = 0; j < N1 / 8; ++j) acc[j][0] = acc[j][1] = acc[j][2] = acc[j][3] = 0.f;
#pragma unroll
      for (int kc = 0; kc < N2 / 16; ++kc) mma_k16<N1 / 8, P2>(acc, alh[kc], all[kc], w2h, w2l, kc * 16, g, t);
      const bf16* y1h = p.p1;
      bf16* dz1l = p.dz1 + p.rows_pad * CP1;
#pragma unroll
      for (int j = 0; j < N1 / 8; ++j) {
        const int c = j * 8 + 2 * t;
        uint32_t ma, mb;
        asm volatile("ld.global.nc.u32 %0, [%1];" : "=r"(ma) : "l"(y1h + ra * CP1 + c));
        asm volatile("ld.global.nc.u32 %0, [%1];" : "=r"(mb) : "l"(y1h + rb * CP1 + c));
        const float z0 = acc[j][0] * ((ma & 0xffffu) ? 1.f : 0.f), z1 = acc[j][1] * ((ma >> 16) ? 1.f : 0.f);
        const float z2 = acc[j][2] * ((mb & 0xffffu) ? 1.f : 0.f), z3 = acc[j][3] * ((mb >> 16) ? 1.f : 0.f);
        const Split2 sa = split2(z0, z1), sb = split2(z2, z3);
        a1h[j / 2][(j & 1) * 2] = sa.hi; a1h[j / 2][(j & 1) * 2 + 1] = sb.hi;
        a1l[j / 2][(j & 1) * 2] = sa.lo; a1l[j / 2][(j & 1) * 2 + 1] = sb.lo;
        if (j & 1) {
          st_chunk(p.dz1, CP1, ra, (j / 2) * 16, pa.hi, pb.hi, sa.hi, sb.hi, t);
          st_chunk(dz1l, CP1, ra, (j / 2) * 16, pa.lo, pb.lo, sa.lo, sb.lo, t);
        } else {
          pa = sa, pb = sb;
        }
        colsum_add(red, N0 + c, z0 + z2, z1 + z3, g);
      }
      zero_pad_cols<N1>(p.dz1, dz1l, r0, lane);
    }

#pragma unroll 1
    for (int n0 = 0; n0 < N0; n0 += NC) {
      float acc[NC / 8][4];
#pragma unroll
      for (int j = 0; j < NC / 8; ++j) acc[j][0] = acc[j][1] = acc[j][2] = acc[j][3] = 0.f;
#pragma unroll
      for (int kc = 0; kc < N1 / 16; ++kc)
        mma_k16<NC / 8, P1>(acc, a1h[kc], a1l[kc], w1h + n0 * P1, w1l + n0 * P1, kc * 16, g, t);
#pragma unroll
      for (int j = 0; j < NC / 8; ++j) {
        const int c = n0 + j * 8 + 2 * t;
        const float2 ya = ld2(p.y0 + ra * N0 + c, va), yb = ld2(p.y0 + rb * N0 + c, vb);
        const float z0 = acc[j][0] * (ya.x > 0.f ? 1.f : 0.f), z1 = acc[j][1] * (ya.y > 0.f ? 1.f : 0.f);
        const float z2 = acc[j][2] * (yb.x > 0.f ? 1.f : 0.f), z3 = acc[j][3] * (yb.y > 0.f ? 1.f : 0.f);
        const Split2 sa = split2(z0, z1), sb = split2(z2, z3);
        if (j & 1) {
          st_chunk(p.dz0, CP0, ra, n0 + (j / 2) * 16, pa.hi, pb.hi, sa.hi, sb.hi, t);
          st_chunk(dz0l, CP0, ra, n0 + (j / 2) * 16, pa.lo, pb.lo, sa.lo, sb.lo, t);
        } else {
          pa = sa, pb = sb;
        }
        colsum_add(red, c, z0 + z2, z1 + z3, g);
      }
    }
    zero_pad_cols<N0>(p.dz0, dz0l, r0, lane);
  }

  __syncthreads();
  for (int c = threadIdx.x; c < NT; c += kTowerThreads) {
    float s = 0.f;
#pragma unroll
    for (int w = 0; w < kTowerWarps; ++w) s += red_all[w * NT + c];
    p.partial[(int64_t)blockIdx.x * NT + c] = s;
  }
}

__global__ void __launch_bounds__(128)
    tower_bias_reduce_kernel(const float* __restrict__ partial, int nblocks, int n0, int n1, int n2, float* db0,
                             float* db1, float* db2) {
  const int nt = n0 + n1 + n2, c = blockIdx.x * blockDim.x + threadIdx.x;
  if (c >= nt) return;
  float s = 0.f;
  for (int b = 0; b < nblocks; ++b) s += partial[(int64_t)b * nt + c];
  if (c < n0) db0[c] = s;
  else if (c < n0 + n1) db1[c - n0] = s;
  else db2[c - n0 - n1] = s;
}

int tower_grid(int64_t rows_pad) {
  const int64_t need = ceil_div(rows_pad / 16, kTowerWarps);
  return (int)(need < kNumSMs ? need : kNumSMs);
}

template <typename Kern>
b2ctr_status_t launch_tower(Kern kern, size_t smem, int grid, cudaStream_t st, const void* args, const char* name) {
  cudaError_t e = cudaFuncSetAttribute(kern, cudaFuncAttributeMaxDynamicSharedMemorySize, (int)smem);
  if (e != cudaSuccess) {
    set_error("%s: cannot reserve %zu bytes of shared memory: %s", name, smem, cudaGetErrorString(e));
    return B2CTR_ERR_CUDA;
  }
  void* argv[] = {const_cast<void*>(args)};
  e = cudaLaunchKernel((const void*)kern, dim3(grid), dim3(kTowerThreads), argv, smem, st);
  if (e != cudaSuccess) {
    set_error("%s: CUDA launch failed: %s", name, cudaGetErrorString(e));
    return B2CTR_ERR_CUDA;
  }
  count_launch();
  return B2CTR_OK;
}

#define B2_TOWERS(X) X(256, 128, 64) X(128, 128, 64) X(256, 128, 0) X(128, 64, 0)

bool tower_widths(const int32_t* widths, int32_t nlayers, int* n) {
  if (!widths || nlayers < 2 || nlayers > 3) return false;
  n[0] = widths[0];
  n[1] = widths[1];
  n[2] = nlayers == 3 ? widths[2] : 0;
#define B2_MATCH(a, b, c) if (n[0] == a && n[1] == b && n[2] == c) return true;
  B2_TOWERS(B2_MATCH)
#undef B2_MATCH
  return false;
}

}
}

using namespace b2ctr;

extern "C" {

int32_t b2ctr_mlp_relu_supported(const int32_t* widths, int32_t nlayers) {
  int n[3];
  return tower_widths(widths, nlayers, n) ? 1 : 0;
}

b2ctr_status_t b2ctr_mlp_relu_fwd(const float* y0, const float* const* w, const float* const* b, void* const* planes,
                                  float* y_last, const int32_t* widths, int32_t nlayers, int64_t batch, void* stream) {
  int n[3];
  B2_REQUIRE(tower_widths(widths, nlayers, n), "mlp_relu_fwd: unsupported tower widths");
  B2_REQUIRE(y0 && w && b && planes && y_last && batch > 0, "mlp_relu_fwd: bad arguments");
  B2_REQUIRE(w[0] && b[0] && planes[0] && (n[2] == 0 || (w[1] && b[1] && planes[1])), "mlp_relu_fwd: NULL operand");
  TowerFwd p{y0, w[0], b[0], n[2] ? w[1] : nullptr, n[2] ? b[1] : nullptr, (bf16*)planes[0],
             n[2] ? (bf16*)planes[1] : nullptr, y_last, batch, planes_rows_pad(batch)};
  const int grid = tower_grid(p.rows_pad);
#define B2_FWD(a, b_, c)                                                                                     \
  if (n[0] == a && n[1] == b_ && n[2] == c)                                                                  \
    return launch_tower(mlp_relu_fwd_kernel<a, b_, c>, tower_smem_bytes<a, b_, c>(false), grid, (cudaStream_t)stream, \
                        &p, "b2ctr_mlp_relu_fwd");
  B2_TOWERS(B2_FWD)
#undef B2_FWD
  return B2CTR_ERR_INVALID_ARG;
}

size_t b2ctr_mlp_relu_bwd_workspace_bytes(const int32_t* widths, int32_t nlayers) {
  int n[3];
  if (!tower_widths(widths, nlayers, n)) return 0;
  return (size_t)kNumSMs * (n[0] + n[1] + n[2]) * sizeof(float);
}

b2ctr_status_t b2ctr_mlp_relu_bwd(const float* dy_last, const float* y_last, const float* y0, void* const* planes,
                                  const float* const* w, void* const* dz_planes, float* const* dbias,
                                  const int32_t* widths, int32_t nlayers, int64_t batch, void* workspace,
                                  size_t workspace_bytes, void* stream) {
  int n[3];
  B2_REQUIRE(tower_widths(widths, nlayers, n), "mlp_relu_bwd: unsupported tower widths");
  B2_REQUIRE(dy_last && y_last && y0 && w && dz_planes && dbias && batch > 0, "mlp_relu_bwd: bad arguments");
  const int L = nlayers;
  for (int i = 0; i < L; ++i) B2_REQUIRE(dz_planes[i] && dbias[i], "mlp_relu_bwd: NULL output");
  B2_REQUIRE(w[0] && (n[2] == 0 || (w[1] && planes && planes[1])), "mlp_relu_bwd: NULL operand");
  const size_t need = b2ctr_mlp_relu_bwd_workspace_bytes(widths, nlayers);
  if (!workspace || workspace_bytes < need) {
    set_error("mlp_relu_bwd: needs %zu workspace bytes, got %zu", need, workspace_bytes);
    return B2CTR_ERR_WORKSPACE;
  }
  TowerBwd p{dy_last, y_last, y0, n[2] ? (const bf16*)planes[1] : nullptr, w[0], n[2] ? w[1] : nullptr,
             (bf16*)dz_planes[0], (bf16*)dz_planes[1], n[2] ? (bf16*)dz_planes[2] : nullptr, (float*)workspace,
             batch, planes_rows_pad(batch)};
  const int grid = tower_grid(p.rows_pad);
  b2ctr_status_t s = B2CTR_ERR_INVALID_ARG;
#define B2_BWD(a, b_, c)                                                                                     \
  if (n[0] == a && n[1] == b_ && n[2] == c)                                                                  \
    s = launch_tower(mlp_relu_bwd_kernel<a, b_, c>, tower_smem_bytes<a, b_, c>(true), grid, (cudaStream_t)stream, \
                     &p, "b2ctr_mlp_relu_bwd");
  B2_TOWERS(B2_BWD)
#undef B2_BWD
  if (s != B2CTR_OK) return s;
  const int nt = n[0] + n[1] + n[2];
  tower_bias_reduce_kernel<<<(unsigned)ceil_div(nt, 128), 128, 0, (cudaStream_t)stream>>>(
      (const float*)workspace, grid, n[0], n[1], n[2], dbias[0], dbias[1], n[2] ? dbias[2] : nullptr);
  B2_CHECK_LAUNCH("b2ctr_mlp_relu_bwd(reduce)");
  return B2CTR_OK;
}

}
```

### deepctr_b200/kernels.py

```python
import contextlib
import ctypes as C
import functools

import torch

from . import _lib as L

_workspace = {}
_retired = []


def _require_cuda(*tensors):
    for t in tensors:
        if t is not None and not t.is_cuda:
            raise L.B2ctrError("b2ctr kernels need CUDA tensors: there is no CPU fallback")


def stream():
    return C.c_void_p(torch.cuda.current_stream().cuda_stream)


def ptr(t):
    return C.c_void_p(t.data_ptr()) if t is not None else C.c_void_p(0)

# ... 3 lines not shown
        return None
    key = (device.index if device.index is not None else torch.cuda.current_device())
    buf = _workspace.get(key)
    if buf is None or buf.numel() < nbytes:
        if buf is not None:
            _retired.append(buf)
        size = max(nbytes, 1 << 20, 2 * buf.numel() if buf is not None else 0)
        if torch.cuda.is_current_stream_capturing():
            raise RuntimeError("workspace growth during CUDA-graph capture (run the step eagerly first)")
        buf = torch.empty(size, dtype=torch.uint8, device=device)
        _workspace[key] = buf
    return buf


def idx_dtype(t):
    if t.dtype == torch.int32:
        return L.IDX_I32
    if t.dtype == torch.int64:
        return L.IDX_I64
    raise ValueError("ids must be int32 or int64, got %s" % t.dtype)


PROFILE = None
PROFILE_TAG = None


@contextlib.contextmanager
def profiled():
    global PROFILE
    PROFILE = {}
    try:
        yield PROFILE
    finally:
        PROFILE = None


class profile_tag(object):

    def __init__(self, tag):
        self.tag = tag

    def __enter__(self):
        global PROFILE_TAG
        self.prev, PROFILE_TAG = PROFILE_TAG, (self.tag if PROFILE_TAG is None else PROFILE_TAG)

    def __exit__(self, *a):
        global PROFILE_TAG
        PROFILE_TAG = self.prev


def _timed(fn):
    name = fn.__name__

    @functools.wraps(fn)
    def wrap(*a, **k):
        prof = PROFILE
        if prof is None:
            return fn(*a, **k)
        e0, e1 = torch.cuda.Event(enable_timing=True), torch.cuda.Event(enable_timing=True)
        e0.record()
        r = fn(*a, **k)
        e1.record()
        prof.setdefault(name if PROFILE_TAG is None else "%s:%s" % (PROFILE_TAG, name), []).append((e0, e1))
        return r

    return wrap


def profile_summary():
    torch.cuda.synchronize()
    out = {}
    for name, evs in (PROFILE or {}).items():
        out[name] = (len(evs), float(sum(a.elapsed_time(b) for a, b in evs)))
    return out


def make_feature(table, idx, out, out_col=0, out_ld=None, maxlen=1, pool=L.POOL_NONE,
                 mask_mode=L.MASK_NONE, length=None, weight=None, weight_mode=L.WEIGHT_NONE,
                 hash_mode=L.HASH_NONE, idx_stride=None, src_table=None, vocab=None):
    _require_cuda(table, idx, out)
    f = L.Feature()
    f.table = table.data_ptr()
    f.idx = idx.data_ptr()
    f.len = length.data_ptr() if length is not None else None
    f.weight = weight.data_ptr() if weight is not None else None
    f.len_stride = length.stride(0) if (length is not None and length.dim() >= 1 and length.shape[0] > 1) else 0
    f.weight_ld = weight.stride(0) if (weight is not None and weight.dim() >= 2 and weight.shape[0] > 1) else 0
    f.out = out.data_ptr()
    f.vocab = table.shape[0] if vocab is None else int(vocab)
    f.dim = table.shape[1] if table.dim() > 1 else 1
    f.idx_stride = idx_stride if idx_stride is not None else (idx.stride(0) if idx.dim() >= 1 else 1)
    f.out_ld = out_ld if out_ld is not None else out.stride(0)
    f.out_col = out_col
    f.maxlen = maxlen
    f.idx_dtype = idx_dtype(idx)
    f.pool = pool
    f.mask_mode = mask_mode
    f.hash_mode = hash_mode
    f.weight_mode = weight_mode
    f.src_table = src_table.data_ptr() if src_table is not None else None
    return f


def _feat_array(feats):
    arr = (L.Feature * len(feats))(*feats)
    return arr


@_timed
def embed_gather_fwd(feats, batch):
    arr = _feat_array(feats)
    L.check(L.lib().b2ctr_embed_gather_fwd(arr, len(feats), batch, stream()), "embed_gather_fwd")


def embed_oob_count(reset=True):
    n = C.c_int64(0)
    L.check(L.lib().b2ctr_embed_oob_count(C.byref(n), 1 if reset else 0, stream()), "embed_oob_count")
    return int(n.value)


@_timed
def embed_scatter_add(feats, batch, scale):
    arr = _feat_array(feats)
    L.check(L.lib().b2ctr_embed_scatter_add(arr, len(feats), batch, scale, stream()),
            "embed_scatter_add")


@_timed
def embed_max_pool_shares(feats, batch, shares):
    _require_cuda(shares)
    arr = _feat_array(feats)
    L.check(L.lib().b2ctr_embed_max_pool_shares(arr, len(feats), batch, ptr(shares), shares.stride(0), stream()),
            "embed_max_pool_shares")


class UniformPlan(object):

    def __init__(self, feats, lin_tables, dense, x, linear, fm, fm_mask):
        self.feat_arr = _feat_array(feats)
        self.g = L.UniformGather()
        self.g.feats = self.feat_arr
        if lin_tables is not None:
            self.lin_arr = (C.c_void_p * len(feats))(*[t.data_ptr() for t in lin_tables])
            self.g.lin_tables = self.lin_arr
        self.g.dense = dense.data_ptr() if dense is not None else None
        self.g.x = x.data_ptr()
        self.g.linear = linear.data_ptr() if linear is not None else None
        self.g.fm = fm.data_ptr() if fm is not None else None
        self.g.ldx = x.stride(0)
        self.g.dense_ld = dense.stride(0) if dense is not None else 0
        self.g.nfeat = len(feats)
        self.g.ndense = dense.shape[1] if dense is not None else 0
        self.g.fm_mask[0] = fm_mask & 0xFFFFFFFFFFFFFFFF
        self.g.fm_mask[1] = 0
        self.fm_sum = (torch.empty((x.shape[0], feats[0].dim), dtype=torch.float32, device=x.device)
                       if fm is not None else None)
        self.x_rows, self.x_device = x.shape[0], x.device
        self.x_planes, self.x_planes_cols = None, 0

    def set_planes(self, cols):
        nbytes = L.lib().b2ctr_planes_bytes(self.x_rows, cols)
        self.x_planes = torch.empty((nbytes,), dtype=torch.uint8, device=self.x_device)
        self.x_planes_cols = cols
        return self.x_planes

    def set_peers(self, world, peer_tables, peer_lin_tables):
        self.peer_refs = (peer_tables, peer_lin_tables)
        self.g.world = world
        self.g.peer_tables = peer_tables.data_ptr()
        self.g.peer_lin_tables = peer_lin_tables.data_ptr() if peer_lin_tables is not None else None


@_timed
def embed_gather_uniform_fwd(plan, batch):
    L.check(L.lib().b2ctr_embed_gather_uniform_fwd_ex(C.byref(plan.g), ptr(plan.fm_sum), ptr(plan.x_planes),
                                                      plan.x_planes_cols, batch, stream()),
            "embed_gather_uniform_fwd")


@_timed
def embed_scatter_uniform_bwd(plan, dx, dfm, dlinear, scale, lin_scale, batch, fm_sum=None):
    L.check(L.lib().b2ctr_embed_scatter_uniform_bwd_ex(C.byref(plan.g), ptr(dx), ptr(dfm), ptr(fm_sum),
                                                       ptr(dlinear), scale, lin_scale, batch, stream()),
            "embed_scatter_uniform_bwd")


@_timed
def embed_update_sorted(plan, dx, dfm, dlinear, optimizer, lr, lin_lr, eps, acc_tables, lin_acc_tables, batch):
    nf = plan.g.nfeat
    dim = plan.feat_arr[0].dim
    nbytes = L.lib().b2ctr_embed_update_sorted_workspace_bytes(nf, dim, batch)
    dev = dx.device if dx is not None else (dfm.device if dfm is not None else dlinear.device)
    ws = workspace(nbytes, dev)
    acc = (C.c_void_p * nf)(*[t.data_ptr() for t in acc_tables]) if acc_tables is not None else None
    lacc = (C.c_void_p * nf)(*[t.data_ptr() for t in lin_acc_tables]) if lin_acc_tables is not None else None
    L.check(L.lib().b2ctr_embed_update_sorted(C.byref(plan.g), ptr(dx), ptr(dfm), ptr(dlinear), optimizer, lr, lin_lr,
                                              eps, acc, lacc, batch, ptr(ws), nbytes, stream()),
            "embed_update_sorted")


@_timed
def hash64(ids, num_buckets, mask_zero):
    _require_cuda(ids)
    ids = ids.contiguous()
    out = torch.empty(ids.shape, dtype=torch.int64, device=ids.device)
    L.check(L.lib().b2ctr_hash64(ptr(ids), idx_dtype(ids), ids.numel(), num_buckets,
                                 1 if mask_zero else 0, ptr(out), stream()), "hash64")
    return out


@_timed
def init_normal(dst, mean, std, seed):
    _require_cuda(dst)
    L.check(L.lib().b2ctr_init_normal(ptr(dst), dst.numel(), mean, std, seed, stream()), "init_normal")
    return dst


@_timed
def gemm(a, b, c=None, bias=None, trans_a=False, trans_b=False, act=L.ACT_NONE, accumulate=False,
         precision=L.GEMM_FP32, split_k=1, alpha=1.0, m=None, n=None, k=None, variant=0, a_planes=None,
         b_planes=None):
    _require_cuda(a, b, c, bias, a_planes, b_planes)
    if (a is None and a_planes is None) or (b is None and b_planes is None):
        raise ValueError("gemm: an fp32 operand may be None only when its planes are given")
    if (a is None or b is None) and None in (m, n, k):
        raise ValueError("gemm: m, n and k are required when an fp32 operand is None")
    if m is None:
        m = a.shape[1] if trans_a else a.shape[0]
    if k is None:
        k = a.shape[0] if trans_a else a.shape[1]
    if n is None:
        n = b.shape[0] if trans_b else b.shape[1]
    dev = next(t.device for t in (a, b, a_planes, b_planes) if t is not None)
    if c is None:
        c = torch.empty((m, n), dtype=torch.float32, device=dev)
    g = L.Gemm()
    g.a = a.data_ptr() if a is not None else None
    g.b = b.data_ptr() if b is not None else None
    g.c = c.data_ptr()
    g.bias = bias.data_ptr() if bias is not None else None
    g.m, g.n, g.k = m, n, k
    g.lda = a.stride(0) if a is not None else (m if trans_a else k)
    g.ldb = b.stride(0) if b is not None else (k if trans_b else n)
    g.ldc = c.stride(0)
    g.trans_a, g.trans_b = int(trans_a), int(trans_b)
    g.act, g.accumulate, g.precision, g.split_k, g.alpha = act, int(accumulate), precision, split_k, alpha
    g.variant = variant
    g.a_planes = a_planes.data_ptr() if a_planes is not None else None
    g.b_planes = b_planes.data_ptr() if b_planes is not None else None
    nbytes = L.lib().b2ctr_gemm_workspace_bytes(C.byref(g))
    ws = workspace(nbytes, dev)
    L.check(L.lib().b2ctr_gemm(C.byref(g), ptr(ws), nbytes if ws is not None else 0, stream()), "gemm")
    return c


@_timed
def split_planes(x2d):
    _require_cuda(x2d)
    rows, cols = x2d.shape
    nbytes = L.lib().b2ctr_planes_bytes(rows, cols)
    buf = torch.empty((nbytes,), dtype=torch.uint8, device=x2d.device)
    L.check(L.lib().b2ctr_split_planes(ptr(x2d), x2d.stride(0), rows, cols, ptr(buf), stream()), "split_planes")
    return buf


def planes_fusable(m, n):
    return m % 256 == 0 and (n == 64 or n % 128 == 0) and n % 4 == 0 and n // 4 <= 256 and 256 % (n // 4) == 0


@_timed
def bias_act_bwd(dy, y, act, want_dz=True, want_dbias=True, m=None, n=None, want_planes=False):
    _require_cuda(dy, y)
    if m is None:
        m, n = dy.shape[0], dy.shape[1]
    ld = dy.stride(0)
    if y is not None and y.dim() == 2 and y.stride(0) != ld:
        raise ValueError("bias_act_bwd: dy and y must have the same row pitch (%d != %d)" % (ld, y.stride(0)))
    dz = torch.empty((m, ld), dtype=torch.float32, device=dy.device)[:, :n] if want_dz else None
    dbias = torch.empty((n,), dtype=torch.float32, device=dy.device) if want_dbias else None
    nbytes = L.lib().b2ctr_bias_act_bwd_workspace_bytes(m, n) if want_dbias else 0
    ws = workspace(nbytes, dy.device)
    if want_planes:
        planes = torch.empty((L.lib().b2ctr_planes_bytes(m, n),), dtype=torch.uint8, device=dy.device)
        L.check(L.lib().b2ctr_bias_act_bwd_planes(ptr(dy), ptr(y), ptr(dz), ptr(dbias), ptr(planes), m, n, ld, act,
                                                  ptr(ws), nbytes, stream()), "bias_act_bwd_planes")
        return dz, dbias, planes
    L.check(L.lib().b2ctr_bias_act_bwd(ptr(dy), ptr(y), ptr(dz), ptr(dbias), m, n, ld, act, ptr(ws),
                                       nbytes, stream()), "bias_act_bwd")
    return dz, dbias


def _widths(widths):
    return (C.c_int32 * len(widths))(*widths), len(widths)


def _ptrs(ts):
    return (C.c_void_p * len(ts))(*[t.data_ptr() if t is not None else None for t in ts])


def _planes(rows, cols, device):
    return torch.empty((L.lib().b2ctr_planes_bytes(rows, cols),), dtype=torch.uint8, device=device)


@_timed
def mlp_relu_fwd(y0, ws, bs):
    _require_cuda(y0, *ws, *bs)
    widths = [y0.shape[1]] + [w.shape[1] for w in ws]
    m = y0.shape[0]
    planes = [_planes(m, n, y0.device) for n in widths[:-1]]
    y = torch.empty((m, widths[-1]), dtype=torch.float32, device=y0.device)
    L.check(L.lib().b2ctr_mlp_relu_fwd(ptr(y0.contiguous()), _ptrs(ws), _ptrs(bs), _ptrs(planes), ptr(y),
                                       *_widths(widths), m, stream()), "mlp_relu_fwd")
    return planes, y


@_timed
def mlp_relu_bwd(dy, y, y0, planes, ws):
    _require_cuda(dy, y, y0, *ws)
    widths = [y0.shape[1]] + [w.shape[1] for w in ws]
    m = y0.shape[0]
    dzp = [_planes(m, n, y0.device) for n in widths]
    db = [torch.empty((n,), dtype=torch.float32, device=y0.device) for n in widths]
    wid = _widths(widths)
    nbytes = L.lib().b2ctr_mlp_relu_bwd_workspace_bytes(*wid)
    wsp = workspace(nbytes, y0.device)
    L.check(L.lib().b2ctr_mlp_relu_bwd(ptr(dy.contiguous()), ptr(y), ptr(y0), _ptrs(planes), _ptrs(ws), _ptrs(dzp),
                                       _ptrs(db), *wid, m, ptr(wsp), nbytes, stream()), "mlp_relu_bwd")
    return dzp, db


@_timed
def act_fwd(x, act, out=None):
    _require_cuda(x)
    out = torch.empty_like(x) if out is None else out
    L.check(L.lib().b2ctr_act_fwd(ptr(x), ptr(out), x.numel(), act, stream()), "act_fwd")
    return out


@_timed
def add_n(ins, scales=None, out=None):
    _require_cuda(*ins)
    out = torch.empty_like(ins[0]) if out is None else out
    arr = (C.c_void_p * len(ins))(*[t.data_ptr() for t in ins])
    sc = (C.c_float * len(ins))(*(scales if scales is not None else [1.0] * len(ins)))
    L.check(L.lib().b2ctr_add_n(arr, sc, len(ins), ptr(out), out.numel(), stream()), "add_n")
    return out


@_timed
def axpy(x, y, alpha=1.0):
    _require_cuda(x, y)
    L.check(L.lib().b2ctr_axpy(ptr(x), ptr(y), alpha, x.numel(), stream()), "axpy")
    return y


@_timed
def fill(dst, value):
    _require_cuda(dst)
    L.check(L.lib().b2ctr_fill(ptr(dst), value, dst.numel(), stream()), "fill")
    return dst


@_timed
def mask_nonzero_and(ids, inout=None):
    _require_cuda(ids, inout)
    first = inout is None
    if first:
        inout = torch.empty(ids.shape, dtype=torch.uint8, device=ids.device)
    L.check(L.lib().b2ctr_mask_nonzero_and(ptr(ids), idx_dtype(ids), ids.numel(), ptr(inout), int(first),
                                           stream()), "mask_nonzero_and")
    return inout


@_timed
def mask_from_len(lengths, maxlen):
    _require_cuda(lengths)
    lengths = lengths.reshape(-1)
    out = torch.empty((lengths.shape[0], maxlen), dtype=torch.uint8, device=lengths.device)
    L.check(L.lib().b2ctr_mask_from_len(ptr(lengths), lengths.shape[0], maxlen, ptr(out), stream()),
            "mask_from_len")
    return out


@_timed
def copy2d(src, ld_src, dst, ld_dst, rows, cols, accumulate=False, src_off=0, dst_off=0):
    _require_cuda(src, dst)
    sp = C.c_void_p(src.data_ptr() + 4 * src_off)
    dp = C.c_void_p(dst.data_ptr() + 4 * dst_off)
    L.check(L.lib().b2ctr_copy2d(sp, ld_src, dp, ld_dst, rows, cols, int(accumulate), stream()), "copy2d")
    return dst


@_timed
def pack_rows(src_flat, widths, batch, out=None):
    _require_cuda(src_flat)
    total = int(sum(widths))
    if out is None:
        out = torch.empty((batch, total), dtype=torch.float32, device=src_flat.device)
    arr = (C.c_int32 * len(widths))(*[int(w) for w in widths])
    L.check(L.lib().b2ctr_pack_rows(ptr(src_flat), arr, len(widths), batch, ptr(out), total, stream()), "pack_rows")
    return out


@_timed
def rowsum(x, rows, cols, ld=None):
    _require_cuda(x)
    out = torch.empty((rows,), dtype=torch.float32, device=x.device)
    L.check(L.lib().b2ctr_rowsum(ptr(x), ld if ld is not None else x.stride(0), ptr(out), rows, cols,
                                 stream()), "rowsum")
    return out


@_timed
def fm_fwd(x, nfield, dim, ldx=None):
    _require_cuda(x)
    batch = x.shape[0]
    out = torch.empty((batch,), dtype=torch.float32, device=x.device)
    L.check(L.lib().b2ctr_fm_fwd(ptr(x), ldx if ldx is not None else x.stride(0), nfield, dim, ptr(out),
                                 batch, stream()), "fm_fwd")
    return out


@_timed
def fm_bwd(x, nfield, dim, dout, dx=None, accumulate=False, ldx=None):
    _require_cuda(x, dout)
    batch = x.shape[0]
    ldx = ldx if ldx is not None else x.stride(0)
    if dx is None:
        dx = torch.empty_like(x)
        accumulate = False
    L.check(L.lib().b2ctr_fm_bwd(ptr(x), ldx, nfield, dim, ptr(dout), ptr(dx), dx.stride(0),
                                 int(accumulate), batch, stream()), "fm_bwd")
    return dx


@_timed
def fm_weighted_fwd(x, ldx, m, nfield, dim, batch):
    _require_cuda(x, m)
    out = torch.empty((batch,), dtype=torch.float32, device=x.device)
    L.check(L.lib().b2ctr_fm_weighted_fwd(ptr(x), ldx, ptr(m), m.stride(0), nfield, dim, ptr(out), batch, stream()),
            "fm_weighted_fwd")
    return out


@_timed
def fm_weighted_bwd(x, ldx, m, nfield, dim, dout, batch, dx=None, accumulate=False, want_dx=True, want_dm=True):
    _require_cuda(x, m, dout, dx)
    if dx is None and want_dx:
        dx = torch.empty((batch, nfield * dim), dtype=torch.float32, device=x.device)
        accumulate = False
    dm = torch.empty((batch, nfield), dtype=torch.float32, device=x.device) if want_dm else None
    L.check(L.lib().b2ctr_fm_weighted_bwd(ptr(x), ldx, ptr(m), m.stride(0), nfield, dim, ptr(dout), ptr(dx),
                                          dx.stride(0) if dx is not None else nfield * dim, int(accumulate), ptr(dm),
                                          nfield, batch, stream()), "fm_weighted_bwd")
    return dx, dm


@_timed
def field_scale_fwd(x, ldx, m, nfield, dim, batch, out=None):
    _require_cuda(x, m, out)
    if out is None:
        out = torch.empty((batch, nfield * dim), dtype=torch.float32, device=x.device)
    L.check(L.lib().b2ctr_field_scale_fwd(ptr(x), ldx, ptr(m), m.stride(0), nfield, dim, ptr(out), out.stride(0),
                                          batch, stream()), "field_scale_fwd")
    return out


@_timed
def field_scale_bwd(dy, x, ldx, m, nfield, dim, batch, dx=None, accumulate=False, want_dx=True, want_dm=True):
    _require_cuda(dy, x, m, dx)
    if dx is None and want_dx:
        dx = torch.empty((batch, nfield * dim), dtype=torch.float32, device=x.device)
        accumulate = False
    dm = torch.empty((batch, nfield), dtype=torch.float32, device=x.device) if want_dm else None
    L.check(L.lib().b2ctr_field_scale_bwd(ptr(dy), dy.stride(0), ptr(x), ldx, ptr(m), m.stride(0), nfield, dim,
                                          ptr(dx), dx.stride(0) if dx is not None else nfield * dim, int(accumulate),
                                          ptr(dm), nfield, batch, stream()), "field_scale_bwd")
    return dx, dm


@_timed
def softmax_rows_fwd(x, scale=1.0):
    _require_cuda(x)
    rows, cols = x.shape
    y = torch.empty((rows, cols), dtype=torch.float32, device=x.device)
    L.check(L.lib().b2ctr_softmax_rows_fwd(ptr(x), x.stride(0), ptr(y), cols, rows, cols, scale, stream()),
            "softmax_rows_fwd")
    return y


@_timed
def softmax_rows_bwd(y, dy, scale=1.0):
    _require_cuda(y, dy)
    rows, cols = y.shape
    dx = torch.empty((rows, cols), dtype=torch.float32, device=y.device)
    L.check(L.lib().b2ctr_softmax_rows_bwd(ptr(y), y.stride(0), ptr(dy), dy.stride(0), ptr(dx), cols, rows, cols,
                                           scale, stream()), "softmax_rows_bwd")
    return dx


@_timed
def predict_loss(logit, bias=None, labels=None, task=L.TASK_BINARY, want_grad=False):
    _require_cuda(logit, bias, labels)
    batch = logit.numel()
    pred = torch.empty((batch,), dtype=torch.float32, device=logit.device)
    dlogit = torch.empty((batch,), dtype=torch.float32, device=logit.device) if want_grad else None
    acc = None
    if labels is not None:
        acc = torch.empty((2,), dtype=torch.float32, device=logit.device)
        fill(acc, 0.0)
    loss_sum = acc[0:1] if acc is not None else None
    dbias = acc[1:2] if (acc is not None and want_grad and bias is not None) else None
    L.check(L.lib().b2ctr_predict_loss(ptr(logit), ptr(bias), ptr(labels), ptr(pred), ptr(dlogit),
                                       ptr(dbias), ptr(loss_sum), batch, task, stream()), "predict_loss")
    return pred, dlogit, dbias, loss_sum


@_timed
def sgd_step(w, g, lr, l2=0.0):
    _require_cuda(w, g)
    L.check(L.lib().b2ctr_sgd_step(ptr(w), ptr(g), lr, l2, w.numel(), stream()), "sgd_step")


@_timed
def sgd_step_multi(ws, gs, lr, l2s):
    n = len(ws)
    if n == 0:
        return
    _require_cuda(*ws)
    _require_cuda(*gs)
    wp, gp = (C.c_void_p * n)(*[ptr(t) for t in ws]), (C.c_void_p * n)(*[ptr(t) for t in gs])
    nn = (C.c_int64 * n)(*[t.numel() for t in ws])
    ll = (C.c_float * n)(*[float(v) for v in l2s])
    L.check(L.lib().b2ctr_sgd_step_multi(wp, gp, nn, ll, n, lr, stream()), "sgd_step_multi")


@_timed
def adam_step(w, g, m, v, lr, step, beta1=0.9, beta2=0.999, eps=1e-7, l2=0.0):
    _require_cuda(w, g, m, v)
    L.check(L.lib().b2ctr_adam_step(ptr(w), ptr(g), ptr(m), ptr(v), lr, beta1, beta2, eps, l2, step,
                                    w.numel(), stream()), "adam_step")


@_timed
def adam_step_dev(w, g, m, v, lr, step_dev, beta1=0.9, beta2=0.999, eps=1e-7, l2=0.0):
    _require_cuda(w, g, m, v, step_dev)
    L.check(L.lib().b2ctr_adam_step_dev(ptr(w), ptr(g), ptr(m), ptr(v), lr, beta1, beta2, eps, l2, ptr(step_dev),
                                        w.numel(), stream()), "adam_step_dev")


@_timed
def counter_add(counter, delta=1):
    _require_cuda(counter)
    L.check(L.lib().b2ctr_counter_add(ptr(counter), delta, stream()), "counter_add")


@_timed
def adagrad_step(w, g, acc, lr, eps=1e-7, l2=0.0):
    _require_cuda(w, g, acc)
    L.check(L.lib().b2ctr_adagrad_step(ptr(w), ptr(g), ptr(acc), lr, eps, l2, w.numel(), stream()),
            "adagrad_step")


def ffm_field(idx=None, vocab=1, hash_mode=L.HASH_NONE, pooled=None, grad=None):
    _require_cuda(idx, pooled, grad)
    f = L.FfmField()
    if idx is not None:
        f.idx, f.idx_stride, f.idx_dtype = idx.data_ptr(), idx.stride(0), idx_dtype(idx)
        f.vocab, f.hash_mode = int(vocab), hash_mode
    if pooled is not None:
        f.pooled, f.pooled_ld = pooled.data_ptr(), pooled.stride(0)
    if grad is not None:
        f.grad, f.grad_ld = grad.data_ptr(), grad.stride(0)
    return f


@_timed
def ffm_product_fwd(fields, tables, dim, reduce_sum, out, out_col, batch):
    arr = (L.FfmField * len(fields))(*fields)
    _lib_call("ffm_product_fwd", arr, len(fields), ptr(tables), dim, int(reduce_sum), ptr(out), out.stride(0),
              out_col, batch, stream())


@_timed
def ffm_product_bwd(fields, tables, dim, reduce_sum, g, g_col, batch):
    arr = (L.FfmField * len(fields))(*fields)
    _lib_call("ffm_product_bwd", arr, len(fields), ptr(tables), dim, int(reduce_sum), ptr(g), g.stride(0), g_col,
              batch, stream())


def _lib_call(name, *args):
    L.check(getattr(L.lib(), "b2ctr_" + name)(*args), name)


@_timed
def ewise(op, a, b, c=None, out=None, accumulate=False):
    _require_cuda(a, b, c, out)
    out = torch.empty_like(a) if out is None else out
    _lib_call("ewise", op, ptr(a), ptr(b), ptr(c), ptr(out), a.numel(), int(accumulate), stream())
    return out


@_timed
def cross_vector_fwd(x0, ld0, xl, ldl, w, bias, batch, dim):
    out = torch.empty((batch, dim), dtype=torch.float32, device=x0.device)
    s = torch.empty((batch,), dtype=torch.float32, device=x0.device)
    _lib_call("cross_vector_fwd", ptr(x0), ld0, ptr(xl), ldl, ptr(w), ptr(bias), ptr(out), ptr(s), batch, dim,
              stream())
    return out, s


@_timed
def cross_vector_bwd(x0, ld0, w, dout, s, batch, dim):
    dx0 = torch.empty((batch, dim), dtype=torch.float32, device=x0.device)
    dxl = torch.empty((batch, dim), dtype=torch.float32, device=x0.device)
    ds = torch.empty((batch,), dtype=torch.float32, device=x0.device)
    _lib_call("cross_vector_bwd", ptr(x0), ld0, ptr(w), ptr(dout), ptr(s), ptr(dx0), ptr(dxl), ptr(ds), batch,
              dim, stream())
    return dx0, dxl, ds


def _off(t, elems):
    return C.c_void_p(t.data_ptr() + 4 * elems)


@_timed
def cin_outer_fwd(x0, v0, xk, vk, z, b0, nb, m, h, d):
    _lib_call("cin_outer_fwd", _off(x0, b0 * v0[0]), v0[0], v0[1], v0[2], _off(xk, b0 * vk[0]), vk[0], vk[1],
              vk[2], ptr(z), nb, m, h, d, stream())
# ... 755 lines not shown
```

Measured before the change: 36.54 million.

## Feed fused MLP tower kernels with a TMA producer warp and mbarrier ring

Restructures the fused ReLU MLP tower forward and backward kernels around a dedicated producer warp. It streams activation tiles through a multi-stage shared-memory ring with TMA loads and mbarriers. Output planes are staged in swizzled shared memory and written back with TMA bulk stores instead of per-thread shuffled global stores, and weight staging is vectorised with float4 loads. The aim is to overlap global memory traffic with the tensor-core math and cut store instruction overhead. In exchange it needs 16-byte aligned operands (the Python side may clone to satisfy this), tensor map encoding on the host per call, and more shared memory and synchronisation complexity.

```diff
diff --git a/deepctr_b200/csrc/common.cuh b/deepctr_b200/csrc/common.cuh
--- a/deepctr_b200/csrc/common.cuh
+++ b/deepctr_b200/csrc/common.cuh
@@ -1,4 +1,5 @@
 #pragma once
+#include <cuda.h>
 #include <cuda_runtime.h>
 #include <cuda_bf16.h>
 #include <stdint.h>
@@ -46,6 +47,11 @@
 static inline int64_t planes_rows_pad(int64_t rows) { return (rows + 255) / 256 * 256; }
 static inline int64_t planes_cols_pad(int64_t cols) { return cols <= 64 ? 64 : (cols + 127) / 128 * 128; }
 
+typedef CUresult (*EncodeTiledFn)(CUtensorMap*, CUtensorMapDataType, cuuint32_t, void*, const cuuint64_t*,
+                                  const cuuint64_t*, const cuuint32_t*, const cuuint32_t*, CUtensorMapInterleave,
+                                  CUtensorMapSwizzle, CUtensorMapL2promotion, CUtensorMapFloatOOBfill);
+EncodeTiledFn tma_encoder();
+
 #ifdef __CUDACC__
 __device__ __forceinline__ uint32_t pack_bf16(__nv_bfloat16 lo, __nv_bfloat16 hi) {
   return (uint32_t)__bfloat16_as_ushort(lo) | ((uint32_t)__bfloat16_as_ushort(hi) << 16);
@@ -76,6 +82,50 @@
 __device__ __forceinline__ void red_add_f1(float* p, float v) {
   asm volatile("red.relaxed.gpu.global.add.f32 [%0], %1;" ::"l"(p), "f"(v) : "memory");
 }
+
+__device__ __forceinline__ uint32_t smem_u32(const void* p) {
+  return (uint32_t)__cvta_generic_to_shared(p);
+}
+__device__ __forceinline__ void mbar_init(uint64_t* bar, uint32_t count) {
+  asm volatile("mbarrier.init.shared::cta.b64 [%0], %1;" ::"r"(smem_u32(bar)), "r"(count));
+}
+__device__ __forceinline__ void mbar_arrive(uint64_t* bar) {
+  asm volatile("mbarrier.arrive.shared::cta.b64 _, [%0];" ::"r"(smem_u32(bar)) : "memory");
+}
+__device__ __forceinline__ void mbar_wait(uint64_t* bar, uint32_t parity) {
+  uint32_t done;
+  do {
+    asm volatile(
+        "{\n\t"
+        ".reg .pred p;\n\t"
+        "mbarrier.try_wait.parity.shared::cta.b64 p, [%1], %2;\n\t"
+        "selp.u32 %0, 1, 0, p;\n\t"
+        "}\n"
+        : "=r"(done)
+        : "r"(smem_u32(bar)), "r"(parity)
+        : "memory");
+  } while (!done);
+}
+__device__ __forceinline__ void mbar_expect_tx(uint64_t* bar, uint32_t bytes) {
+  asm volatile("mbarrier.arrive.expect_tx.shared::cta.b64 _, [%0], %1;" ::"r"(smem_u32(bar)), "r"(bytes) : "memory");
+}
+__device__ __forceinline__ void tma_load_2d(uint32_t dst, const CUtensorMap* map, int32_t c0, int32_t c1, uint64_t* bar) {
+  asm volatile(
+      "cp.async.bulk.tensor.2d.shared::cluster.global.mbarrier::complete_tx::bytes [%0], [%1, {%2, %3}], [%4];" ::"r"(dst),
+      "l"(map), "r"(c0), "r"(c1), "r"(smem_u32(bar))
+      : "memory");
+}
+__device__ __forceinline__ void tma_prefetch_desc(const CUtensorMap* map) {
+  asm volatile("prefetch.tensormap [%0];" ::"l"(map) : "memory");
+}
+__device__ __forceinline__ void tma_store_2d(const CUtensorMap* map, uint32_t src, int32_t c0, int32_t c1) {
+  asm volatile("cp.async.bulk.tensor.2d.global.shared::cta.bulk_group [%0, {%2, %3}], [%1];" ::"l"(map), "r"(src),
+               "r"(c0), "r"(c1)
+               : "memory");
+}
+__device__ __forceinline__ void bulk_commit() { asm volatile("cp.async.bulk.commit_group;" ::: "memory"); }
+__device__ __forceinline__ void bulk_wait_read() { asm volatile("cp.async.bulk.wait_group.read 0;" ::: "memory"); }
+__device__ __forceinline__ void bulk_wait_all() { asm volatile("cp.async.bulk.wait_group 0;" ::: "memory"); }
 
 __device__ __forceinline__ uint64_t l2_policy_evict_last() {
   uint64_t p;
diff --git a/deepctr_b200/csrc/gemm_tc.cu b/deepctr_b200/csrc/gemm_tc.cu
--- a/deepctr_b200/csrc/gemm_tc.cu
+++ b/deepctr_b200/csrc/gemm_tc.cu
@@ -1,4 +1,3 @@
-#include <cuda.h>
 #include <cuda_bf16.h>
 #include "common.cuh"
 
@@ -25,29 +24,6 @@
   float* fold_dt0; float* fold_dxk; int64_t fold_ldx;
 };
 
-__device__ __forceinline__ uint32_t smem_u32(const void* p) {
-  return (uint32_t)__cvta_generic_to_shared(p);
-}
-__device__ __forceinline__ void mbar_init(uint64_t* bar, uint32_t count) {
-  asm volatile("mbarrier.init.shared::cta.b64 [%0], %1;" ::"r"(smem_u32(bar)), "r"(count));
-}
-__device__ __forceinline__ void mbar_arrive(uint64_t* bar) {
-  asm volatile("mbarrier.arrive.shared::cta.b64 _, [%0];" ::"r"(smem_u32(bar)) : "memory");
-}
-__device__ __forceinline__ void mbar_wait(uint64_t* bar, uint32_t parity) {
-  uint32_t done;
-  do {
-    asm volatile(
-        "{\n\t"
-        ".reg .pred p;\n\t"
-        "mbarrier.try_wait.parity.shared::cta.b64 p, [%1], %2;\n\t"
-        "selp.u32 %0, 1, 0, p;\n\t"
-        "}\n"
-        : "=r"(done)
-        : "r"(smem_u32(bar)), "r"(parity)
-        : "memory");
-  } while (!done);
-}
 __device__ __forceinline__ uint64_t wgmma_desc(uint32_t saddr, int mn) {
   return (uint64_t)((saddr & 0x3FFFF) >> 4) | ((uint64_t)(mn ? 512 : 1) << 16) | (64ull << 32) | (1ull << 62);
 }
@@ -431,31 +407,11 @@
 };
 template <int BN>
 __host__ __device__ constexpr int ws_staging_bytes() { return 64 * (BN < 64 ? BN : 64) * 4; }
-__device__ __forceinline__ void mbar_expect_tx(uint64_t* bar, uint32_t bytes) {
-  asm volatile("mbarrier.arrive.expect_tx.shared::cta.b64 _, [%0], %1;" ::"r"(smem_u32(bar)), "r"(bytes) : "memory");
-}
-__device__ __forceinline__ void tma_load_2d(uint32_t dst, const CUtensorMap* map, int32_t c0, int32_t c1, uint64_t* bar) {
-  asm volatile(
-      "cp.async.bulk.tensor.2d.shared::cluster.global.mbarrier::complete_tx::bytes [%0], [%1, {%2, %3}], [%4];" ::"r"(dst),
-      "l"(map), "r"(c0), "r"(c1), "r"(smem_u32(bar))
-      : "memory");
-}
-__device__ __forceinline__ void tma_prefetch_desc(const CUtensorMap* map) {
-  asm volatile("prefetch.tensormap [%0];" ::"l"(map) : "memory");
-}
-__device__ __forceinline__ void tma_store_2d(const CUtensorMap* map, uint32_t src, int32_t c0, int32_t c1) {
-  asm volatile("cp.async.bulk.tensor.2d.global.shared::cta.bulk_group [%0, {%2, %3}], [%1];" ::"l"(map), "r"(src),
-               "r"(c0), "r"(c1)
-               : "memory");
-}
 __device__ __forceinline__ void tma_store_3d(const CUtensorMap* map, uint32_t src, int32_t c0, int32_t c1, int32_t c2) {
   asm volatile("cp.async.bulk.tensor.3d.global.shared::cta.bulk_group [%0, {%2, %3, %4}], [%1];" ::"l"(map), "r"(src),
                "r"(c0), "r"(c1), "r"(c2)
                : "memory");
 }
-__device__ __forceinline__ void bulk_commit() { asm volatile("cp.async.bulk.commit_group;" ::: "memory"); }
-__device__ __forceinline__ void bulk_wait_read() { asm volatile("cp.async.bulk.wait_group.read 0;" ::: "memory"); }
-__device__ __forceinline__ void bulk_wait_all() { asm volatile("cp.async.bulk.wait_group 0;" ::: "memory"); }
 __device__ __forceinline__ void warpgroup_sync(int wg) {
   asm volatile("bar.sync %0, 128;" ::"r"(1 + wg) : "memory");
 }
@@ -1012,10 +968,7 @@
   return cudaGetLastError();
 }
 
-typedef CUresult (*EncodeTiledFn)(CUtensorMap*, CUtensorMapDataType, cuuint32_t, void*, const cuuint64_t*,
-                                  const cuuint64_t*, const cuuint32_t*, const cuuint32_t*, CUtensorMapInterleave,
-                                  CUtensorMapSwizzle, CUtensorMapL2promotion, CUtensorMapFloatOOBfill);
-static EncodeTiledFn tma_encoder() {
+EncodeTiledFn tma_encoder() {
   static EncodeTiledFn fn = nullptr;
   static bool tried = false;
   if (!tried) {
diff --git a/deepctr_b200/csrc/tower.cu b/deepctr_b200/csrc/tower.cu
--- a/deepctr_b200/csrc/tower.cu
+++ b/deepctr_b200/csrc/tower.cu
@@ -6,25 +6,31 @@
 
 typedef __nv_bfloat16 bf16;
 constexpr int kTowerWarps = 8;
-constexpr int kTowerThreads = kTowerWarps * 32;
+constexpr int kConsumerThreads = kTowerWarps * 32;
+constexpr int kTowerThreads = kConsumerThreads + 32;
+constexpr int kBlockRows = 16 * kTowerWarps;
+constexpr int kStageBytes = kBlockRows * 64;
+constexpr int kStageMax = 8;
+constexpr int kStgBytes = 2048;
+constexpr size_t kSmemOptin = 232448;
+constexpr size_t kSmemAlignSlack = 512;
 
 __host__ __device__ constexpr int cols_pad(int w) { return w <= 64 ? 64 : (w + 127) / 128 * 128; }
 
 struct TowerFwd {
-  const float* y0;
+  CUtensorMap y0;
+  CUtensorMap p0, p1;
   const float* w1; const float* b1;
   const float* w2; const float* b2;
-  bf16* p0; bf16* p1;
   float* ylast;
   int64_t batch, rows_pad;
 };
 struct TowerBwd {
-  const float* dy;
-  const float* ylast;
-  const float* y0;
-  const bf16* p1;
+  CUtensorMap dy, ylast;
+  CUtensorMap y1h;
+  CUtensorMap y0;
+  CUtensorMap dz0, dz1, dz2;
   const float* w1; const float* w2;
-  bf16* dz0; bf16* dz1; bf16* dz2;
   float* partial;
   int64_t batch, rows_pad;
 };
@@ -48,25 +54,69 @@
   return v > 0.f ? v : 0.f;
 }
 
-__device__ __forceinline__ float2 ld2(const float* p, bool ok) {
-  return ok ? __ldg(reinterpret_cast<const float2*>(p)) : make_float2(0.f, 0.f);
-}
-
-__device__ __forceinline__ void st_chunk(bf16* plane, int64_t cp, int64_t ra, int c0, uint32_t a, uint32_t b,
-                                         uint32_t c, uint32_t d, int t) {
-  const int quad = threadIdx.x & 28;
-  uint32_t o0 = 0, o1 = 0, o2 = 0, o3 = 0;
-#pragma unroll
-  for (int r = 0; r < 4; ++r) {
-    const int i = (t - r) & 3, src = (t + r) & 3;
-    const uint32_t send = i == 0 ? a : i == 1 ? c : i == 2 ? b : d;
-    const uint32_t v = __shfl_sync(0xffffffffu, send, quad | src);
-    o0 = src == 0 ? v : o0;
-    o1 = src == 1 ? v : o1;
-    o2 = src == 2 ? v : o2;
-    o3 = src == 3 ? v : o3;
-  }
-  *reinterpret_cast<uint4*>(plane + (ra + (t >> 1) * 8) * cp + c0 + (t & 1) * 8) = make_uint4(o0, o1, o2, o3);
+__device__ __forceinline__ int sw64(int r, int b) { return r * 64 + ((((b >> 4) ^ (r >> 1)) & 3) << 4) + (b & 15); }
+__device__ __forceinline__ float2 lds2(const unsigned char* stage, int r, int b) {
+  return *reinterpret_cast<const float2*>(stage + sw64(r, b));
+}
+
+template <int S>
+struct RingPos {
+  int s = 0;
+  uint32_t phase = 0;
+  __device__ __forceinline__ void next() {
+    if (++s == S) s = 0, phase ^= 1;
+  }
+};
+struct Ring {
+  unsigned char* buf;
+  uint64_t* full;
+  uint64_t* empty;
+};
+template <int S>
+__device__ __forceinline__ void ring_load(const Ring& q, RingPos<S>& pos, const CUtensorMap* map, int c, int r) {
+  mbar_wait(&q.empty[pos.s], pos.phase ^ 1);
+  mbar_expect_tx(&q.full[pos.s], kStageBytes);
+  tma_load_2d(smem_u32(q.buf + pos.s * kStageBytes), map, c, r, &q.full[pos.s]);
+  pos.next();
+}
+template <int S>
+__device__ __forceinline__ const unsigned char* ring_wait(const Ring& q, const RingPos<S>& pos) {
+  mbar_wait(&q.full[pos.s], pos.phase);
+  return q.buf + pos.s * kStageBytes;
+}
+template <int S>
+__device__ __forceinline__ void ring_release(const Ring& q, RingPos<S>& pos, int lane) {
+  __syncwarp();
+  if (lane == 0) mbar_arrive(&q.empty[pos.s]);
+  pos.next();
+}
+
+__device__ __forceinline__ void stage16(unsigned char* stg, int h, uint32_t a, uint32_t b, uint32_t c, uint32_t d,
+                                        int g, int t) {
+  const int b0 = h * 32 + 4 * t;
+  *reinterpret_cast<uint32_t*>(stg + sw64(g, b0)) = a;
+  *reinterpret_cast<uint32_t*>(stg + sw64(g + 8, b0)) = b;
+  *reinterpret_cast<uint32_t*>(stg + sw64(g, b0 + 16)) = c;
+  *reinterpret_cast<uint32_t*>(stg + sw64(g + 8, b0 + 16)) = d;
+}
+__device__ __forceinline__ void stage_split(unsigned char* stg, int h, Split2 a, Split2 b, Split2 c, Split2 d, int g,
+                                            int t) {
+  stage16(stg, h, a.hi, b.hi, c.hi, d.hi, g, t);
+  stage16(stg + 1024, h, a.lo, b.lo, c.lo, d.lo, g, t);
+}
+__device__ __forceinline__ void staging_reclaim(int lane) {
+  if (lane == 0) bulk_wait_read();
+  __syncwarp();
+}
+__device__ __forceinline__ void staging_store(const CUtensorMap* map, unsigned char* stg, int c0, int64_t r0,
+                                              int64_t rows_pad, int lane) {
+  asm volatile("fence.proxy.async.shared::cta;" ::: "memory");
+  __syncwarp();
+  if (lane == 0) {
+    tma_store_2d(map, smem_u32(stg), c0, (int32_t)r0);
+    tma_store_2d(map, smem_u32(stg + 1024), c0, (int32_t)(rows_pad + r0));
+    bulk_commit();
+  }
 }
 
 template <int NT, int P>
@@ -85,24 +135,41 @@
 
 template <int K, int N, bool kTrans>
 __device__ __forceinline__ void stage_weight(const float* __restrict__ w, bf16* sh, bf16* sl) {
-  for (int i = threadIdx.x; i < K * N; i += kTowerThreads) {
-    const int k = i / N, n = i - k * N;
-    const float v = __ldg(w + i);
-    const bf16 h = __float2bfloat16_rn(v);
-    const int o = kTrans ? n * (K + 8) + k : k * (N + 8) + n;
-    sh[o] = h;
-    sl[o] = __float2bfloat16_rn(v - __bfloat162float(h));
-  }
-}
-
-template <int W>
-__device__ __forceinline__ void zero_pad_cols(bf16* hi, bf16* lo, int64_t r0, int lane) {
-  constexpr int CP = cols_pad(W), V = (CP - W) / 8;
-  if constexpr (V > 0) {
-    for (int i = lane; i < 16 * V; i += 32) {
-      const int64_t o = (r0 + i / V) * CP + W + (i % V) * 8;
-      *reinterpret_cast<uint4*>(hi + o) = make_uint4(0, 0, 0, 0);
-      *reinterpret_cast<uint4*>(lo + o) = make_uint4(0, 0, 0, 0);
+  constexpr int kItems = kTrans ? (K / 2) * (N / 4) : K * (N / 4), kBatch = 4;
+  static_assert(kItems % (kConsumerThreads * kBatch) == 0, "weight staging batches");
+  for (int i0 = threadIdx.x; i0 < kItems; i0 += kConsumerThreads * kBatch) {
+    float4 v[kBatch][kTrans ? 2 : 1];
+#pragma unroll
+    for (int u = 0; u < kBatch; ++u) {
+      const int i = i0 + u * kConsumerThreads;
+      if constexpr (kTrans) {
+        const int kp = i % (K / 2), nq = i / (K / 2);
+        v[u][0] = __ldg(reinterpret_cast<const float4*>(w + (2 * kp) * N + 4 * nq));
+        v[u][1] = __ldg(reinterpret_cast<const float4*>(w + (2 * kp + 1) * N + 4 * nq));
+      } else {
+        v[u][0] = __ldg(reinterpret_cast<const float4*>(w + i * 4));
+      }
+    }
+#pragma unroll
+    for (int u = 0; u < kBatch; ++u) {
+      const int i = i0 + u * kConsumerThreads;
+      if constexpr (kTrans) {
+        const int kp = i % (K / 2), nq = i / (K / 2);
+        const float a[4] = {v[u][0].x, v[u][0].y, v[u][0].z, v[u][0].w}, b[4] = {v[u][1].x, v[u][1].y, v[u][1].z, v[u][1].w};
+#pragma unroll
+        for (int e = 0; e < 4; ++e) {
+          const Split2 s = split2(a[e], b[e]);
+          const int o = (4 * nq + e) * (K + 8) + 2 * kp;
+          *reinterpret_cast<uint32_t*>(sh + o) = s.hi;
+          *reinterpret_cast<uint32_t*>(sl + o) = s.lo;
+        }
+      } else {
+        const int k = i / (N / 4), nq = i % (N / 4);
+        const Split2 s0 = split2(v[u][0].x, v[u][0].y), s1 = split2(v[u][0].z, v[u][0].w);
+        const int o = k * (N + 8) + 4 * nq;
+        *reinterpret_cast<uint2*>(sh + o) = make_uint2(s0.hi, s1.hi);
+        *reinterpret_cast<uint2*>(sl + o) = make_uint2(s0.lo, s1.lo);
+      }
     }
   }
 }
@@ -119,47 +186,110 @@
   }
 }
 
+__device__ __forceinline__ void consumers_sync() { asm volatile("bar.sync 1, %0;" ::"n"(kConsumerThreads) : "memory"); }
+
 template <int N0, int N1, int N2>
-constexpr size_t tower_smem_bytes(bool bwd) {
+__host__ __device__ constexpr size_t tower_weight_bytes(bool bwd) {
   return bwd ? ((size_t)N0 * (N1 + 8) + (size_t)N1 * (N2 + 8)) * 2 * sizeof(bf16) +
                    (size_t)kTowerWarps * (N0 + N1 + N2) * sizeof(float)
              : ((size_t)N1 * (N0 + 8) + (size_t)N2 * (N1 + 8)) * 2 * sizeof(bf16);
 }
-
 template <int N0, int N1, int N2>
-__global__ void __launch_bounds__(kTowerThreads, 1) mlp_relu_fwd_kernel(const TowerFwd p) {
+__host__ __device__ constexpr int tower_stages(bool bwd) {
+  constexpr size_t kStatic = 2 * kStageMax * sizeof(uint64_t);
+  const size_t room = kSmemOptin - kStatic - kSmemAlignSlack - (size_t)kTowerWarps * kStgBytes - tower_weight_bytes<N0, N1, N2>(bwd);
+  return room / kStageBytes < kStageMax ? (int)(room / kStageBytes) : kStageMax;
+}
+template <int N0, int N1, int N2>
+__host__ __device__ constexpr size_t tower_smem_bytes(bool bwd) {
+  return kSmemAlignSlack + (size_t)tower_stages<N0, N1, N2>(bwd) * kStageBytes + (size_t)kTowerWarps * kStgBytes +
+         tower_weight_bytes<N0, N1, N2>(bwd);
+}
+
+template <int N0, int N1, int N2>
+__device__ constexpr bool tower_shape_ok() {
+  return cols_pad(N0) == N0 && cols_pad(N1) == N1 && (N2 == 0 || cols_pad(N2) == N2) && N0 % 32 == 0 && N1 % 32 == 0 &&
+         N2 % 32 == 0;
+}
+
+struct TowerSmem {
+  Ring ring;
+  unsigned char* stg;
+  unsigned char* weights;
+};
+template <int S>
+__device__ __forceinline__ TowerSmem tower_smem(unsigned char* smem, uint64_t* full, uint64_t* empty) {
+  const uint32_t a = smem_u32(smem);
+  unsigned char* base = smem + (((a + (uint32_t)kSmemAlignSlack - 1) & ~(uint32_t)(kSmemAlignSlack - 1)) - a);
+  if (threadIdx.x == 0) {
+    for (int s = 0; s < S; ++s) {
+      mbar_init(&full[s], 1);
+      mbar_init(&empty[s], kTowerWarps);
+    }
+    asm volatile("fence.mbarrier_init.release.cluster;" ::: "memory");
+  }
+  __syncthreads();
+  return {{base, full, empty}, base + S * kStageBytes, base + S * kStageBytes + kTowerWarps * kStgBytes};
+}
+
+template <int N0, int N1, int N2>
+__global__ void __launch_bounds__(kTowerThreads, 1) mlp_relu_fwd_kernel(const __grid_constant__ TowerFwd p) {
+  static_assert(tower_shape_ok<N0, N1, N2>(), "tower widths");
+  constexpr int S = tower_stages<N0, N1, N2>(false);
+  static_assert(S >= 2, "ring");
   extern __shared__ __align__(16) unsigned char smem[];
-  constexpr int P1 = N0 + 8, P2 = N1 + 8, CP0 = cols_pad(N0), CP1 = cols_pad(N1);
-  bf16* w1h = reinterpret_cast<bf16*>(smem);
+  __shared__ __align__(8) uint64_t full[kStageMax], empty[kStageMax];
+  constexpr int P1 = N0 + 8, P2 = N1 + 8;
+  const TowerSmem sm = tower_smem<S>(smem, full, empty);
+  const int lane = threadIdx.x & 31, warp = threadIdx.x >> 5;
+  const int64_t blocks = p.rows_pad / kBlockRows;
+
+  if (warp == kTowerWarps) {
+    if (lane == 0) {
+      tma_prefetch_desc(&p.y0);
+      RingPos<S> pos;
+      for (int64_t blk = blockIdx.x; blk < blocks; blk += gridDim.x)
+        for (int kc = 0; kc < N0 / 16; ++kc) ring_load(sm.ring, pos, &p.y0, kc * 16, (int)(blk * kBlockRows));
+    }
+    return;
+  }
+
+  bf16* w1h = reinterpret_cast<bf16*>(sm.weights);
   bf16* w1l = w1h + N1 * P1;
   bf16* w2h = w1l + N1 * P1;
   bf16* w2l = w2h + N2 * P2;
   stage_weight<N0, N1, true>(p.w1, w1h, w1l);
   if constexpr (N2 > 0) stage_weight<N1, N2, true>(p.w2, w2h, w2l);
-  __syncthreads();
-
-  const int lane = threadIdx.x & 31, g = lane >> 2, t = lane & 3;
-  bf16* p0l = p.p0 + p.rows_pad * CP0;
-  const int64_t tiles = p.rows_pad / 16;
-  for (int64_t tile = (int64_t)blockIdx.x * kTowerWarps + (threadIdx.x >> 5); tile < tiles;
-       tile += (int64_t)gridDim.x * kTowerWarps) {
-    const int64_t r0 = tile * 16, ra = r0 + g, rb = ra + 8;
+  consumers_sync();
+
+  const int g = lane >> 2, t = lane & 3, ra_s = warp * 16 + g, rb_s = ra_s + 8;
+  unsigned char* stg = sm.stg + warp * kStgBytes;
+  RingPos<S> pos;
+  for (int64_t blk = blockIdx.x; blk < blocks; blk += gridDim.x) {
+    const int64_t r0 = blk * kBlockRows + warp * 16, ra = r0 + g, rb = ra + 8;
     const bool va = ra < p.batch, vb = rb < p.batch;
     float acc1[N1 / 8][4];
 #pragma unroll
     for (int j = 0; j < N1 / 8; ++j) acc1[j][0] = acc1[j][1] = acc1[j][2] = acc1[j][3] = 0.f;
-#pragma unroll 4
+    float2 x[4];
+    auto read_y0 = [&](float2 (&v)[4]) {
+      const unsigned char* st = ring_wait(sm.ring, pos);
+#pragma unroll
+      for (int i = 0; i < 4; ++i) v[i] = lds2(st, i & 1 ? rb_s : ra_s, (i >> 1) * 32 + 8 * t);
+      ring_release(sm.ring, pos, lane);
+    };
+    read_y0(x);
+#pragma unroll 2
     for (int kc = 0; kc < N0 / 16; ++kc) {
-      const int c = kc * 16 + 2 * t;
-      const float2 x0 = ld2(p.y0 + ra * N0 + c, va), x1 = ld2(p.y0 + rb * N0 + c, vb);
-      const float2 x2 = ld2(p.y0 + ra * N0 + c + 8, va), x3 = ld2(p.y0 + rb * N0 + c + 8, vb);
-      const Split2 s0 = split2(x0.x, x0.y), s1 = split2(x1.x, x1.y), s2 = split2(x2.x, x2.y), s3 = split2(x3.x, x3.y);
+      const Split2 s0 = split2(x[0].x, x[0].y), s1 = split2(x[1].x, x[1].y), s2 = split2(x[2].x, x[2].y),
+                   s3 = split2(x[3].x, x[3].y);
       const uint32_t ah[4] = {s0.hi, s1.hi, s2.hi, s3.hi}, al[4] = {s0.lo, s1.lo, s2.lo, s3.lo};
-      st_chunk(p.p0, CP0, ra, kc * 16, s0.hi, s1.hi, s2.hi, s3.hi, t);
-      st_chunk(p0l, CP0, ra, kc * 16, s0.lo, s1.lo, s2.lo, s3.lo, t);
+      if ((kc & 1) == 0) staging_reclaim(lane);
+      stage_split(stg, kc & 1, s0, s1, s2, s3, g, t);
+      if (kc & 1) staging_store(&p.p0, stg, (kc / 2) * 32, r0, p.rows_pad, lane);
+      if (kc + 1 < N0 / 16) read_y0(x);
       mma_k16<N1 / 8, P1>(acc1, ah, al, w1h, w1l, kc * 16, g, t);
     }
-    zero_pad_cols<N0>(p.p0, p0l, r0, lane);
 
     if constexpr (N2 == 0) {
 #pragma unroll
@@ -172,7 +302,6 @@
                     make_float2(relu_bias(acc1[j][2], b.x), relu_bias(acc1[j][3], b.y));
       }
     } else {
-      bf16* p1l = p.p1 + p.rows_pad * CP1;
       uint32_t a2h[N1 / 16][4], a2l[N1 / 16][4];
       Split2 pa, pb;
 #pragma unroll
@@ -184,13 +313,14 @@
         a2h[j / 2][(j & 1) * 2] = sa.hi; a2h[j / 2][(j & 1) * 2 + 1] = sb.hi;
         a2l[j / 2][(j & 1) * 2] = sa.lo; a2l[j / 2][(j & 1) * 2 + 1] = sb.lo;
         if (j & 1) {
-          st_chunk(p.p1, CP1, ra, (j / 2) * 16, pa.hi, pb.hi, sa.hi, sb.hi, t);
-          st_chunk(p1l, CP1, ra, (j / 2) * 16, pa.lo, pb.lo, sa.lo, sb.lo, t);
+          const int h = (j / 2) & 1;
+          if (h == 0) staging_reclaim(lane);
+          stage_split(stg, h, pa, pb, sa, sb, g, t);
+          if (h == 1) staging_store(&p.p1, stg, (j / 4) * 32, r0, p.rows_pad, lane);
         } else {
           pa = sa, pb = sb;
         }
       }
-      zero_pad_cols<N1>(p.p1, p1l, r0, lane);
       float acc2[N2 / 8][4];
 #pragma unroll
       for (int j = 0; j < N2 / 8; ++j) acc2[j][0] = acc2[j][1] = acc2[j][2] = acc2[j][3] = 0.f;
@@ -207,55 +337,96 @@
       }
     }
   }
+  if (lane == 0) bulk_wait_read();
 }
 
 template <int N0, int N1, int N2>
-__global__ void __launch_bounds__(kTowerThreads, 1) mlp_relu_bwd_kernel(const TowerBwd p) {
+__global__ void __launch_bounds__(kTowerThreads, 1) mlp_relu_bwd_kernel(const __grid_constant__ TowerBwd p) {
+  static_assert(tower_shape_ok<N0, N1, N2>(), "tower widths");
+  constexpr int S = tower_stages<N0, N1, N2>(true);
+  static_assert(S >= 2, "ring: dy and y_last are read together");
   extern __shared__ __align__(16) unsigned char smem[];
+  __shared__ __align__(8) uint64_t full[kStageMax], empty[kStageMax];
   constexpr int NL = N2 ? N2 : N1, NT = N0 + N1 + N2;
-  constexpr int P1 = N1 + 8, P2 = N2 + 8, CP0 = cols_pad(N0), CP1 = cols_pad(N1), CPL = cols_pad(NL);
+  constexpr int P1 = N1 + 8, P2 = N2 + 8;
   constexpr int NC = 32;
-  bf16* w1h = reinterpret_cast<bf16*>(smem);
+  const TowerSmem sm = tower_smem<S>(smem, full, empty);
+  const int lane = threadIdx.x & 31, warp = threadIdx.x >> 5;
+  const int64_t blocks = p.rows_pad / kBlockRows;
+
+  if (warp == kTowerWarps) {
+    if (lane == 0) {
+      tma_prefetch_desc(&p.dy);
+      tma_prefetch_desc(&p.ylast);
+      tma_prefetch_desc(&p.y0);
+      if constexpr (N2 > 0) tma_prefetch_desc(&p.y1h);
+      RingPos<S> pos;
+      for (int64_t blk = blockIdx.x; blk < blocks; blk += gridDim.x) {
+        const int r = (int)(blk * kBlockRows);
+        for (int c = 0; c < NL; c += 16) {
+          ring_load(sm.ring, pos, &p.dy, c, r);
+          ring_load(sm.ring, pos, &p.ylast, c, r);
+        }
+        if constexpr (N2 > 0)
+          for (int c = 0; c < N1; c += 32) ring_load(sm.ring, pos, &p.y1h, c, r);
+        for (int c = 0; c < N0; c += 16) ring_load(sm.ring, pos, &p.y0, c, r);
+      }
+    }
+    return;
+  }
+
+  bf16* w1h = reinterpret_cast<bf16*>(sm.weights);
   bf16* w1l = w1h + N0 * P1;
   bf16* w2h = w1l + N0 * P1;
   bf16* w2l = w2h + N1 * P2;
   float* red_all = reinterpret_cast<float*>(w2l + N1 * P2);
   stage_weight<N0, N1, false>(p.w1, w1h, w1l);
   if constexpr (N2 > 0) stage_weight<N1, N2, false>(p.w2, w2h, w2l);
-  for (int i = threadIdx.x; i < kTowerWarps * NT; i += kTowerThreads) red_all[i] = 0.f;
-  __syncthreads();
-
-  const int lane = threadIdx.x & 31, warp = threadIdx.x >> 5, g = lane >> 2, t = lane & 3;
+  for (int i = threadIdx.x; i < kTowerWarps * NT; i += kConsumerThreads) red_all[i] = 0.f;
+  consumers_sync();
+
+  const int g = lane >> 2, t = lane & 3, ra_s = warp * 16 + g, rb_s = ra_s + 8;
   float* red = red_all + warp * NT;
-  bf16* dzl = N2 ? p.dz2 : p.dz1;
-  bf16* dzl_lo = dzl + p.rows_pad * CPL;
-  bf16* dz0l = p.dz0 + p.rows_pad * CP0;
-  const int64_t tiles = p.rows_pad / 16;
-  for (int64_t tile = (int64_t)blockIdx.x * kTowerWarps + warp; tile < tiles; tile += (int64_t)gridDim.x * kTowerWarps) {
-    const int64_t r0 = tile * 16, ra = r0 + g, rb = ra + 8;
-    const bool va = ra < p.batch, vb = rb < p.batch;
+  const CUtensorMap* dzl = N2 ? &p.dz2 : &p.dz1;
+  unsigned char* stg = sm.stg + warp * kStgBytes;
+  RingPos<S> pos;
+  for (int64_t blk = blockIdx.x; blk < blocks; blk += gridDim.x) {
+    const int64_t r0 = blk * kBlockRows + warp * 16;
 
     uint32_t alh[NL / 16][4], all[NL / 16][4];
-    Split2 pa, pb;
-#pragma unroll
-    for (int j = 0; j < NL / 8; ++j) {
-      const int c = j * 8 + 2 * t;
-      const float2 da = ld2(p.dy + ra * NL + c, va), db = ld2(p.dy + rb * NL + c, vb);
-      const float2 ya = ld2(p.ylast + ra * NL + c, va), yb = ld2(p.ylast + rb * NL + c, vb);
-      const float z0 = da.x * (ya.x > 0.f ? 1.f : 0.f), z1 = da.y * (ya.y > 0.f ? 1.f : 0.f);
-      const float z2 = db.x * (yb.x > 0.f ? 1.f : 0.f), z3 = db.y * (yb.y > 0.f ? 1.f : 0.f);
-      const Split2 sa = split2(z0, z1), sb = split2(z2, z3);
-      alh[j / 2][(j & 1) * 2] = sa.hi; alh[j / 2][(j & 1) * 2 + 1] = sb.hi;
-      all[j / 2][(j & 1) * 2] = sa.lo; all[j / 2][(j & 1) * 2 + 1] = sb.lo;
-      if (j & 1) {
-        st_chunk(dzl, CPL, ra, (j / 2) * 16, pa.hi, pb.hi, sa.hi, sb.hi, t);
-        st_chunk(dzl_lo, CPL, ra, (j / 2) * 16, pa.lo, pb.lo, sa.lo, sb.lo, t);
-      } else {
-        pa = sa, pb = sb;
-      }
-      colsum_add(red, N0 + (N2 ? N1 : 0) + c, z0 + z2, z1 + z3, g);
-    }
-    zero_pad_cols<NL>(dzl, dzl_lo, r0, lane);
+#pragma unroll
+    for (int kc = 0; kc < NL / 16; ++kc) {
+      const unsigned char* sdy = ring_wait(sm.ring, pos);
+      RingPos<S> pos_y = pos;
+      pos_y.next();
+      const unsigned char* sy = ring_wait(sm.ring, pos_y);
+      float2 d[4], y[4];
+#pragma unroll
+      for (int i = 0; i < 4; ++i) {
+        d[i] = lds2(sdy, i & 1 ? rb_s : ra_s, (i >> 1) * 32 + 8 * t);
+        y[i] = lds2(sy, i & 1 ? rb_s : ra_s, (i >> 1) * 32 + 8 * t);
+      }
+      ring_release(sm.ring, pos, lane);
+      ring_release(sm.ring, pos, lane);
+      Split2 sp[4];
+#pragma unroll
+      for (int h = 0; h < 2; ++h) {
+        const int c = kc * 16 + h * 8 + 2 * t;
+        const float2 da = d[2 * h], db = d[2 * h + 1], ya = y[2 * h], yb = y[2 * h + 1];
+        const float z0 = da.x * (ya.x > 0.f ? 1.f : 0.f), z1 = da.y * (ya.y > 0.f ? 1.f : 0.f);
+        const float z2 = db.x * (yb.x > 0.f ? 1.f : 0.f), z3 = db.y * (yb.y > 0.f ? 1.f : 0.f);
+        sp[2 * h] = split2(z0, z1);
+        sp[2 * h + 1] = split2(z2, z3);
+        alh[kc][h * 2] = sp[2 * h].hi; alh[kc][h * 2 + 1] = sp[2 * h + 1].hi;
+        all[kc][h * 2] = sp[2 * h].lo; all[kc][h * 2 + 1] = sp[2 * h + 1].lo;
+        if (h == 1) {
+          if ((kc & 1) == 0) staging_reclaim(lane);
+          stage_split(stg, kc & 1, sp[0], sp[1], sp[2], sp[3], g, t);
+          if (kc & 1) staging_store(dzl, stg, (kc / 2) * 32, r0, p.rows_pad, lane);
+        }
+        colsum_add(red, N0 + (N2 ? N1 : 0) + c, z0 + z2, z1 + z3, g);
+      }
+    }
 
     uint32_t a1h[N1 / 16][4], a1l[N1 / 16][4];
     if constexpr (N2 == 0) {
@@ -269,28 +440,36 @@
       for (int j = 0; j < N1 / 8; ++j) acc[j][0] = acc[j][1] = acc[j][2] = acc[j][3] = 0.f;
 #pragma unroll
       for (int kc = 0; kc < N2 / 16; ++kc) mma_k16<N1 / 8, P2>(acc, alh[kc], all[kc], w2h, w2l, kc * 16, g, t);
-      const bf16* y1h = p.p1;
-      bf16* dz1l = p.dz1 + p.rows_pad * CP1;
+      Split2 pa, pb;
+      uint32_t ma[4], mb[4];
 #pragma unroll
       for (int j = 0; j < N1 / 8; ++j) {
         const int c = j * 8 + 2 * t;
-        uint32_t ma, mb;
-        asm volatile("ld.global.nc.u32 %0, [%1];" : "=r"(ma) : "l"(y1h + ra * CP1 + c));
-        asm volatile("ld.global.nc.u32 %0, [%1];" : "=r"(mb) : "l"(y1h + rb * CP1 + c));
-        const float z0 = acc[j][0] * ((ma & 0xffffu) ? 1.f : 0.f), z1 = acc[j][1] * ((ma >> 16) ? 1.f : 0.f);
-        const float z2 = acc[j][2] * ((mb & 0xffffu) ? 1.f : 0.f), z3 = acc[j][3] * ((mb >> 16) ? 1.f : 0.f);
+        if (j % 4 == 0) {
+          const unsigned char* sm1 = ring_wait(sm.ring, pos);
+#pragma unroll
+          for (int i = 0; i < 4; ++i) {
+            ma[i] = *reinterpret_cast<const uint32_t*>(sm1 + sw64(ra_s, i * 16 + 4 * t));
+            mb[i] = *reinterpret_cast<const uint32_t*>(sm1 + sw64(rb_s, i * 16 + 4 * t));
+          }
+          ring_release(sm.ring, pos, lane);
+        }
+        const uint32_t m0 = ma[j % 4], m1 = mb[j % 4];
+        const float z0 = acc[j][0] * ((m0 & 0xffffu) ? 1.f : 0.f), z1 = acc[j][1] * ((m0 >> 16) ? 1.f : 0.f);
+        const float z2 = acc[j][2] * ((m1 & 0xffffu) ? 1.f : 0.f), z3 = acc[j][3] * ((m1 >> 16) ? 1.f : 0.f);
         const Split2 sa = split2(z0, z1), sb = split2(z2, z3);
         a1h[j / 2][(j & 1) * 2] = sa.hi; a1h[j / 2][(j & 1) * 2 + 1] = sb.hi;
         a1l[j / 2][(j & 1) * 2] = sa.lo; a1l[j / 2][(j & 1) * 2 + 1] = sb.lo;
         if (j & 1) {
-          st_chunk(p.dz1, CP1, ra, (j / 2) * 16, pa.hi, pb.hi, sa.hi, sb.hi, t);
-          st_chunk(dz1l, CP1, ra, (j / 2) * 16, pa.lo, pb.lo, sa.lo, sb.lo, t);
+          const int h = (j / 2) & 1;
+          if (h == 0) staging_reclaim(lane);
+          stage_split(stg, h, pa, pb, sa, sb, g, t);
+          if (h == 1) staging_store(&p.dz1, stg, (j / 4) * 32, r0, p.rows_pad, lane);
         } else {
           pa = sa, pb = sb;
         }
         colsum_add(red, N0 + c, z0 + z2, z1 + z3, g);
       }
-      zero_pad_cols<N1>(p.dz1, dz1l, r0, lane);
     }
 
 #pragma unroll 1
@@ -301,27 +480,34 @@
 #pragma unroll
       for (int kc = 0; kc < N1 / 16; ++kc)
         mma_k16<NC / 8, P1>(acc, a1h[kc], a1l[kc], w1h + n0 * P1, w1l + n0 * P1, kc * 16, g, t);
+      float2 y[8];
+#pragma unroll
+      for (int half = 0; half < 2; ++half) {
+        const unsigned char* sy = ring_wait(sm.ring, pos);
+#pragma unroll
+        for (int i = 0; i < 4; ++i) y[half * 4 + i] = lds2(sy, i & 1 ? rb_s : ra_s, (i >> 1) * 32 + 8 * t);
+        ring_release(sm.ring, pos, lane);
+      }
+      staging_reclaim(lane);
+      Split2 pa, pb;
 #pragma unroll
       for (int j = 0; j < NC / 8; ++j) {
         const int c = n0 + j * 8 + 2 * t;
-        const float2 ya = ld2(p.y0 + ra * N0 + c, va), yb = ld2(p.y0 + rb * N0 + c, vb);
+        const float2 ya = y[2 * j], yb = y[2 * j + 1];
         const float z0 = acc[j][0] * (ya.x > 0.f ? 1.f : 0.f), z1 = acc[j][1] * (ya.y > 0.f ? 1.f : 0.f);
         const float z2 = acc[j][2] * (yb.x > 0.f ? 1.f : 0.f), z3 = acc[j][3] * (yb.y > 0.f ? 1.f : 0.f);
         const Split2 sa = split2(z0, z1), sb = split2(z2, z3);
-        if (j & 1) {
-          st_chunk(p.dz0, CP0, ra, n0 + (j / 2) * 16, pa.hi, pb.hi, sa.hi, sb.hi, t);
-          st_chunk(dz0l, CP0, ra, n0 + (j / 2) * 16, pa.lo, pb.lo, sa.lo, sb.lo, t);
-        } else {
-          pa = sa, pb = sb;
-        }
+        if (j & 1) stage_split(stg, j / 2, pa, pb, sa, sb, g, t);
+        else pa = sa, pb = sb;
         colsum_add(red, c, z0 + z2, z1 + z3, g);
       }
-    }
-    zero_pad_cols<N0>(p.dz0, dz0l, r0, lane);
-  }
-
-  __syncthreads();
-  for (int c = threadIdx.x; c < NT; c += kTowerThreads) {
+      staging_store(&p.dz0, stg, n0, r0, p.rows_pad, lane);
+    }
+  }
+  if (lane == 0) bulk_wait_read();
+
+  consumers_sync();
+  for (int c = threadIdx.x; c < NT; c += kConsumerThreads) {
     float s = 0.f;
 #pragma unroll
     for (int w = 0; w < kTowerWarps; ++w) s += red_all[w * NT + c];
@@ -341,8 +527,32 @@
   else db2[c - n0 - n1] = s;
 }
 
+constexpr int64_t kMaxRowsPad = int64_t(1) << 30;
+
+bool tower_map(CUtensorMap* m, const void* base, bool bf, int64_t cols, int64_t rows, int box_rows) {
+  EncodeTiledFn enc = tma_encoder();
+  const int esz = bf ? 2 : 4;
+  if (!enc || ((uintptr_t)base & 15) || (cols * esz) % 16) return false;
+  cuuint64_t dims[2] = {(cuuint64_t)cols, (cuuint64_t)rows};
+  cuuint64_t strides[1] = {(cuuint64_t)(cols * esz)};
+  cuuint32_t box[2] = {(cuuint32_t)(64 / esz), (cuuint32_t)box_rows};
+  cuuint32_t estr[2] = {1, 1};
+  return enc(m, bf ? CU_TENSOR_MAP_DATA_TYPE_BFLOAT16 : CU_TENSOR_MAP_DATA_TYPE_FLOAT32, 2, const_cast<void*>(base),
+             dims, strides, box, estr, CU_TENSOR_MAP_INTERLEAVE_NONE, CU_TENSOR_MAP_SWIZZLE_64B,
+             CU_TENSOR_MAP_L2_PROMOTION_L2_256B, CU_TENSOR_MAP_FLOAT_OOB_FILL_NONE) == CUDA_SUCCESS;
+}
+bool plane_map(CUtensorMap* m, void* planes, int64_t cols, int64_t rows_pad) {
+  return tower_map(m, planes, true, cols, 2 * rows_pad, 16);
+}
+
+bool weights_aligned(const float* const* w, int n) {
+  for (int i = 0; i < n; ++i)
+    if ((uintptr_t)w[i] & 15) return false;
+  return true;
+}
+
 int tower_grid(int64_t rows_pad) {
-  const int64_t need = ceil_div(rows_pad / 16, kTowerWarps);
+  const int64_t need = rows_pad / kBlockRows;
   return (int)(need < kNumSMs ? need : kNumSMs);
 }
 
@@ -394,8 +604,20 @@
   B2_REQUIRE(tower_widths(widths, nlayers, n), "mlp_relu_fwd: unsupported tower widths");
   B2_REQUIRE(y0 && w && b && planes && y_last && batch > 0, "mlp_relu_fwd: bad arguments");
   B2_REQUIRE(w[0] && b[0] && planes[0] && (n[2] == 0 || (w[1] && b[1] && planes[1])), "mlp_relu_fwd: NULL operand");
-  TowerFwd p{y0, w[0], b[0], n[2] ? w[1] : nullptr, n[2] ? b[1] : nullptr, (bf16*)planes[0],
-             n[2] ? (bf16*)planes[1] : nullptr, y_last, batch, planes_rows_pad(batch)};
+  TowerFwd p{};
+  p.w1 = w[0], p.b1 = b[0], p.w2 = n[2] ? w[1] : nullptr, p.b2 = n[2] ? b[1] : nullptr;
+  p.ylast = y_last, p.batch = batch, p.rows_pad = planes_rows_pad(batch);
+  B2_REQUIRE(p.rows_pad <= kMaxRowsPad, "mlp_relu_fwd: batch too large");
+  if (!weights_aligned(w, n[2] ? 2 : 1)) {
+    set_error("mlp_relu_fwd: the weights must be 16-byte aligned");
+    return B2CTR_ERR_UNSUPPORTED;
+  }
+  if (!tower_map(&p.y0, y0, false, n[0], batch, kBlockRows) || !plane_map(&p.p0, planes[0], n[0], p.rows_pad) ||
+      (n[2] && !plane_map(&p.p1, planes[1], n[1], p.rows_pad))) {
+    set_error("mlp_relu_fwd: cannot encode the TMA maps (cuTensorMapEncodeTiled unavailable, or an operand is not "
+              "16-byte aligned)");
+    return B2CTR_ERR_UNSUPPORTED;
+  }
   const int grid = tower_grid(p.rows_pad);
 #define B2_FWD(a, b_, c)                                                                                     \
   if (n[0] == a && n[1] == b_ && n[2] == c)                                                                  \
@@ -427,9 +649,25 @@
     set_error("mlp_relu_bwd: needs %zu workspace bytes, got %zu", need, workspace_bytes);
     return B2CTR_ERR_WORKSPACE;
   }
-  TowerBwd p{dy_last, y_last, y0, n[2] ? (const bf16*)planes[1] : nullptr, w[0], n[2] ? w[1] : nullptr,
-             (bf16*)dz_planes[0], (bf16*)dz_planes[1], n[2] ? (bf16*)dz_planes[2] : nullptr, (float*)workspace,
-             batch, planes_rows_pad(batch)};
+  const int nl = n[2] ? n[2] : n[1];
+  TowerBwd p{};
+  p.w1 = w[0], p.w2 = n[2] ? w[1] : nullptr, p.partial = (float*)workspace;
+  p.batch = batch, p.rows_pad = planes_rows_pad(batch);
+  B2_REQUIRE(p.rows_pad <= kMaxRowsPad, "mlp_relu_bwd: batch too large");
+  if (!weights_aligned(w, n[2] ? 2 : 1)) {
+    set_error("mlp_relu_bwd: the weights must be 16-byte aligned");
+    return B2CTR_ERR_UNSUPPORTED;
+  }
+  if (!tower_map(&p.dy, dy_last, false, nl, batch, kBlockRows) ||
+      !tower_map(&p.ylast, y_last, false, nl, batch, kBlockRows) ||
+      !tower_map(&p.y0, y0, false, n[0], batch, kBlockRows) ||
+      (n[2] && !tower_map(&p.y1h, planes[1], true, n[1], p.rows_pad, kBlockRows)) ||
+      !plane_map(&p.dz0, dz_planes[0], n[0], p.rows_pad) || !plane_map(&p.dz1, dz_planes[1], n[1], p.rows_pad) ||
+      (n[2] && !plane_map(&p.dz2, dz_planes[2], n[2], p.rows_pad))) {
+    set_error("mlp_relu_bwd: cannot encode the TMA maps (cuTensorMapEncodeTiled unavailable, or an operand is not "
+              "16-byte aligned)");
+    return B2CTR_ERR_UNSUPPORTED;
+  }
   const int grid = tower_grid(p.rows_pad);
   b2ctr_status_t s = B2CTR_ERR_INVALID_ARG;
 #define B2_BWD(a, b_, c)                                                                                     \
diff --git a/deepctr_b200/kernels.py b/deepctr_b200/kernels.py
--- a/deepctr_b200/kernels.py
+++ b/deepctr_b200/kernels.py
@@ -329,6 +329,11 @@
     return torch.empty((L.lib().b2ctr_planes_bytes(rows, cols),), dtype=torch.uint8, device=device)
 
 
+def _tma_operand(t):
+    t = t.contiguous()
+    return t if t.data_ptr() % 16 == 0 else t.clone()
+
+
 @_timed
 def mlp_relu_fwd(y0, ws, bs):
     _require_cuda(y0, *ws, *bs)
@@ -336,7 +341,8 @@
     m = y0.shape[0]
     planes = [_planes(m, n, y0.device) for n in widths[:-1]]
     y = torch.empty((m, widths[-1]), dtype=torch.float32, device=y0.device)
-    L.check(L.lib().b2ctr_mlp_relu_fwd(ptr(y0.contiguous()), _ptrs(ws), _ptrs(bs), _ptrs(planes), ptr(y),
+    y0, ws = _tma_operand(y0), [_tma_operand(w) for w in ws]
+    L.check(L.lib().b2ctr_mlp_relu_fwd(ptr(y0), _ptrs(ws), _ptrs(bs), _ptrs(planes), ptr(y),
                                        *_widths(widths), m, stream()), "mlp_relu_fwd")
     return planes, y
 
@@ -351,7 +357,9 @@
     wid = _widths(widths)
     nbytes = L.lib().b2ctr_mlp_relu_bwd_workspace_bytes(*wid)
     wsp = workspace(nbytes, y0.device)
-    L.check(L.lib().b2ctr_mlp_relu_bwd(ptr(dy.contiguous()), ptr(y), ptr(y0), _ptrs(planes), _ptrs(ws), _ptrs(dzp),
+    dy, y, y0 = _tma_operand(dy), _tma_operand(y), _tma_operand(y0)
+    ws = [_tma_operand(w) for w in ws]
+    L.check(L.lib().b2ctr_mlp_relu_bwd(ptr(dy), ptr(y), ptr(y0), _ptrs(planes), _ptrs(ws), _ptrs(dzp),
                                        _ptrs(db), *wid, m, ptr(wsp), nbytes, stream()), "mlp_relu_bwd")
     return dzp, db
 
```

After: 39.04 million (median of 6 runs). +6.8%, better.
